# geloescht/mxnet-maintenance

Hardware: AMD Instinct MI355X
Metric: images/sec (whole node) ResNet-50 fp16 batch 256/GPU at 1/2/4/8 MI355X (higher is better)
Workload: dtype fp16; 1 GPU; model=ResNet-50 v1b, global_batch=256, per_gpu_batch=256, image_size=224, parallelism=dp1, layout=NHWC, optimizer=mp-SGD momentum 0.9, lr 0.1 (linear warm-up 40 steps), hip_graph=True, deterministic=True

## Files before the change

### mxnet_maintenance_amd/contrib/amp/lists.py

```python

LP16 = ['Convolution', 'Deconvolution', 'FullyConnected', 'RNN', 'dot', 'batch_dot', '_linalg_gemm', '_linalg_gemm2',
        'linalg_gemm', 'linalg_gemm2', '_contrib_interleaved_matmul_selfatt_qk',
        '_contrib_interleaved_matmul_selfatt_valatt', '_contrib_interleaved_matmul_encdec_qk',
        '_contrib_interleaved_matmul_encdec_valatt']

FP32 = ['exp', 'expm1', 'log', 'log10', 'log2', 'log1p', 'pow', '_power', 'power', 'broadcast_power', 'rsqrt',
        'rcbrt', 'reciprocal', 'square', 'sqrt', 'cbrt', 'arccos', 'arcsin', 'arctanh', 'arccosh', 'cosh', 'sinh',
        'tan', 'erfinv', 'gamma', 'gammaln', 'digamma',
        'softmax', 'log_softmax', 'softmin', 'SoftmaxActivation', 'softmax_cross_entropy', 'SoftmaxOutput',
        'LinearRegressionOutput', 'LogisticRegressionOutput', 'MAERegressionOutput', 'CTCLoss', 'ctc_loss',
        'MakeLoss', 'make_loss', 'SVMOutput',
        'norm', 'L2Normalization', 'LayerNorm', 'GroupNorm', 'InstanceNorm', 'LRN', 'moments',
        'sum', 'sum_axis', 'nansum', 'prod', 'nanprod', 'mean', 'topk', 'sort', 'argsort', 'cumsum',
        '_contrib_MultiBoxDetection', '_contrib_MultiBoxPrior', '_contrib_MultiBoxTarget', '_contrib_box_nms',
        '_contrib_ROIAlign', 'ROIPooling', 'Correlation', 'BilinearSampler', 'GridGenerator', 'SpatialTransformer']

WIDEST = ['elemwise_add', 'elemwise_sub', 'elemwise_mul', 'elemwise_div', '_plus', '_Plus', '_add', '_minus',
          '_Minus', '_sub', '_mul', '_Mul', '_div', '_Div', '_mod', '_Mod', '_maximum', '_minimum', '_hypot',
          '_equal', '_not_equal', '_greater', '_greater_equal', '_lesser', '_lesser_equal',
          'broadcast_add', 'broadcast_plus', 'broadcast_sub', 'broadcast_minus', 'broadcast_mul', 'broadcast_div',
          'broadcast_mod', 'broadcast_maximum', 'broadcast_minimum', 'broadcast_hypot', 'broadcast_equal',
          'broadcast_not_equal', 'broadcast_greater', 'broadcast_greater_equal', 'broadcast_lesser',
          'broadcast_lesser_equal', 'Concat', 'concat', 'stack', 'add_n', 'ElementWiseSum', 'where',
          '_contrib_BatchNormAddReLU', 'BatchNormAddReLU']

CONDITIONAL_FP32 = [('Activation', 'act_type', ['softrelu']), ('LeakyReLU', 'act_type', ['elu', 'selu'])]

LOSS_OUTPUT = ['SoftmaxOutput', 'LinearRegressionOutput', 'LogisticRegressionOutput', 'MAERegressionOutput']
```

### mxnet_maintenance_amd/gluon/model_zoo/vision/resnet.py

```python
from ... import nn
from ...block import HybridBlock
from ...nn.basic_layers import _BatchNorm
from ....context import cpu

__all__ = ['ResNetV1', 'ResNetV2', 'BasicBlockV1', 'BasicBlockV2', 'BottleneckV1', 'BottleneckV2',
           'BottleneckV1b', 'resnet18_v1', 'resnet34_v1', 'resnet50_v1', 'resnet101_v1', 'resnet152_v1',
           'resnet18_v2', 'resnet34_v2', 'resnet50_v2', 'resnet101_v2', 'resnet152_v2', 'resnet50_v1b',
           'resnet101_v1b', 'resnet152_v1b', 'resnet18_v1b', 'resnet34_v1b', 'get_resnet']


def _bn_axis(layout):
    return 3 if layout == 'NHWC' else 1


def _conv(channels, k, stride, pad, in_channels, layout, use_bias=False):
    return nn.Conv2D(channels, kernel_size=k, strides=stride, padding=pad, use_bias=use_bias,
                     in_channels=in_channels, layout=layout)


def _bn(layout, relu=False, fuse=False, **kw):
    if relu and fuse:
        return nn.BatchNormReLU(axis=_bn_axis(layout), **kw)
    return nn.BatchNorm(axis=_bn_axis(layout), **kw)


class _StemBNReLUPool(nn.BatchNormReLU):

    def hybrid_forward(self, F, x, gamma, beta, running_mean, running_var):
        return F.contrib.BatchNormReLUMaxPool(x, gamma, beta, running_mean, running_var, name='fwd',
                                              kernel=(3, 3), stride=(2, 2), pad=(1, 1), **self._kwargs)


def _stem_tail(features, layout, fuse):
    if fuse and layout == 'NHWC':
        features.add(_StemBNReLUPool(axis=_bn_axis(layout)))
        return
    features.add(_bn(layout, True, fuse))
    if not fuse:
        features.add(nn.Activation('relu'))
    features.add(nn.MaxPool2D(3, 2, 1, layout=layout))


class _ResidualTail(_BatchNorm):

    def __init__(self, layout, fuse, **kwargs):
        super().__init__(axis=_bn_axis(layout), **kwargs)
        self._fuse_add = fuse

    def _alias(self):
        return 'batchnorm'

    def hybrid_forward(self, F, x, shortcut, gamma, beta, running_mean, running_var):
        if self._fuse_add:
            return F.contrib.BatchNormAddReLU(x, shortcut, gamma, beta, running_mean, running_var, name='fwd',
                                              **self._kwargs)
        return F.BatchNorm(x, gamma, beta, running_mean, running_var, name='fwd', **self._kwargs)


def _finish(F, tail, out, shortcut):
    y = tail(out, shortcut)
    return y if tail._fuse_add else F.Activation(y + shortcut, act_type='relu')


class BasicBlockV1(HybridBlock):

    def __init__(self, channels, stride, downsample=False, in_channels=0, layout='NCHW', fuse=False, **kwargs):
        super().__init__(**kwargs)
        self.body = nn.HybridSequential(prefix='')
        self.body.add(_conv(channels, 3, stride, 1, in_channels, layout),
                      _bn(layout, True, fuse))
        if not fuse:
            self.body.add(nn.Activation('relu'))
        self.body.add(_conv(channels, 3, 1, 1, channels, layout))
        self.tail = _ResidualTail(layout, fuse)
        self.downsample = None
        if downsample:
            self.downsample = nn.HybridSequential(prefix='')
            self.downsample.add(_conv(channels, 1, stride, 0, in_channels, layout), _bn(layout))

    def hybrid_forward(self, F, x):
        shortcut = self.downsample(x) if self.downsample is not None else x
        return _finish(F, self.tail, self.body(x), shortcut)


class BottleneckV1(HybridBlock):

    def __init__(self, channels, stride, downsample=False, in_channels=0, layout='NCHW', fuse=False,
                 stride_on_3x3=False, **kwargs):
        super().__init__(**kwargs)
        mid = channels // 4
        s1, s3 = (1, stride) if stride_on_3x3 else (stride, 1)
        self.body = nn.HybridSequential(prefix='')
        self.body.add(_conv(mid, 1, s1, 0, in_channels, layout), _bn(layout, True, fuse))
        if not fuse:
            self.body.add(nn.Activation('relu'))
        self.body.add(_conv(mid, 3, s3, 1, mid, layout), _bn(layout, True, fuse))
        if not fuse:
            self.body.add(nn.Activation('relu'))
        self.body.add(_conv(channels, 1, 1, 0, mid, layout))
        self.tail = _ResidualTail(layout, fuse)
        self.downsample = None
        if downsample:
            self.downsample = nn.HybridSequential(prefix='')
            self.downsample.add(_conv(channels, 1, stride, 0, in_channels, layout), _bn(layout))
        self._tee = fuse and s1 == 1 and layout == 'NHWC'
        if self._tee:
            self.body[0]._tee = True

    def hybrid_forward(self, F, x):
        if self._tee:
            blocks = list(self.body._children.values())
            out, passthrough = blocks[0](x)
            for b in blocks[1:]:
                out = b(out)
            shortcut = self.downsample(passthrough) if self.downsample is not None else passthrough
            return _finish(F, self.tail, out, shortcut)
        shortcut = self.downsample(x) if self.downsample is not None else x
        return _finish(F, self.tail, self.body(x), shortcut)


class BottleneckV1b(BottleneckV1):
    def __init__(self, channels, stride, downsample=False, in_channels=0, layout='NCHW', fuse=False, **kwargs):
        super().__init__(channels, stride, downsample, in_channels, layout, fuse, stride_on_3x3=True, **kwargs)


class BasicBlockV2(HybridBlock):

    def __init__(self, channels, stride, downsample=False, in_channels=0, layout='NCHW', fuse=False, **kwargs):
        super().__init__(**kwargs)
        self.bn1 = _bn(layout, True, fuse)
        self.conv1 = _conv(channels, 3, stride, 1, in_channels, layout)
        self.bn2 = _bn(layout, True, fuse)
        self.conv2 = _conv(channels, 3, 1, 1, channels, layout)
        self._fused = fuse
        self.downsample = _conv(channels, 1, stride, 0, in_channels, layout) if downsample else None

    def _act(self, F, x, bn):
        x = bn(x)
        return x if self._fused else F.Activation(x, act_type='relu')

    def hybrid_forward(self, F, x):
        shortcut = x
        x = self._act(F, x, self.bn1)
        if self.downsample is not None:
            shortcut = self.downsample(x)
        x = self.conv1(x)
        x = self.conv2(self._act(F, x, self.bn2))
        return x + shortcut


class BottleneckV2(HybridBlock):

    def __init__(self, channels, stride, downsample=False, in_channels=0, layout='NCHW', fuse=False, **kwargs):
        super().__init__(**kwargs)
        mid = channels // 4
        self.bn1 = _bn(layout, True, fuse)
        self.conv1 = _conv(mid, 1, 1, 0, 0, layout)
        self.bn2 = _bn(layout, True, fuse)
        self.conv2 = _conv(mid, 3, stride, 1, mid, layout)
        self.bn3 = _bn(layout, True, fuse)
        self.conv3 = _conv(channels, 1, 1, 0, 0, layout)
        self._fused = fuse
        self.downsample = _conv(channels, 1, stride, 0, in_channels, layout) if downsample else None

    def _act(self, F, x, bn):
        x = bn(x)
        return x if self._fused else F.Activation(x, act_type='relu')

    def hybrid_forward(self, F, x):
        shortcut = x
        x = self._act(F, x, self.bn1)
        if self.downsample is not None:
            shortcut = self.downsample(x)
        x = self.conv1(x)
        x = self.conv2(self._act(F, x, self.bn2))
        x = self.conv3(self._act(F, x, self.bn3))
        return x + shortcut


class _ResNetBase(HybridBlock):
    def _stage(self, block, n, channels, stride, index, in_channels, layout, fuse):
        stage = nn.HybridSequential(prefix='stage%d_' % index)
        with stage.name_scope():
            stage.add(block(channels, stride, channels != in_channels, in_channels=in_channels, layout=layout,
                            fuse=fuse, prefix=''))
            for _ in range(n - 1):
                stage.add(block(channels, 1, False, in_channels=channels, layout=layout, fuse=fuse, prefix=''))
        return stage


class ResNetV1(_ResNetBase):

    def __init__(self, block, layers, channels, classes=1000, thumbnail=False, layout='NCHW', fuse=False,
                 **kwargs):
        super().__init__(**kwargs)
        assert len(layers) == len(channels) - 1
        self._layout = layout
        with self.name_scope():
            self.features = nn.HybridSequential(prefix='')
            if thumbnail:
                self.features.add(_conv(channels[0], 3, 1, 1, 0, layout))
            else:
                self.features.add(_conv(channels[0], 7, 2, 3, 0, layout))
                _stem_tail(self.features, layout, fuse)
            for i, n in enumerate(layers):
                self.features.add(self._stage(block, n, channels[i + 1], 1 if i == 0 else 2, i + 1,
                                              channels[i], layout, fuse))
            self.features.add(nn.GlobalAvgPool2D(layout=layout))
            self.output = nn.Dense(classes, in_units=channels[-1])

    def hybrid_forward(self, F, x):
        return self.output(self.features(x))


class ResNetV2(_ResNetBase):

    def __init__(self, block, layers, channels, classes=1000, thumbnail=False, layout='NCHW', fuse=False,
                 **kwargs):
        super().__init__(**kwargs)
        assert len(layers) == len(channels) - 1
        with self.name_scope():
            self.features = nn.HybridSequential(prefix='')
            self.features.add(nn.BatchNorm(scale=False, center=False, axis=_bn_axis(layout)))
            if thumbnail:
                self.features.add(_conv(channels[0], 3, 1, 1, 0, layout))
            else:
                self.features.add(_conv(channels[0], 7, 2, 3, 0, layout))
                _stem_tail(self.features, layout, fuse)
            in_channels = channels[0]
            for i, n in enumerate(layers):
                self.features.add(self._stage(block, n, channels[i + 1], 1 if i == 0 else 2, i + 1,
                                              in_channels, layout, fuse))
                in_channels = channels[i + 1]
            self.features.add(_bn(layout, True, fuse))
            if not fuse:
                self.features.add(nn.Activation('relu'))
            self.features.add(nn.GlobalAvgPool2D(layout=layout))
            self.features.add(nn.Flatten())
            self.output = nn.Dense(classes, in_units=in_channels)

    def hybrid_forward(self, F, x):
        return self.output(self.features(x))


resnet_spec = {18: ('basic_block', [2, 2, 2, 2], [64, 64, 128, 256, 512]),
               34: ('basic_block', [3, 4, 6, 3], [64, 64, 128, 256, 512]),
               50: ('bottle_neck', [3, 4, 6, 3], [64, 256, 512, 1024, 2048]),
               101: ('bottle_neck', [3, 4, 23, 3], [64, 256, 512, 1024, 2048]),
               152: ('bottle_neck', [3, 8, 36, 3], [64, 256, 512, 1024, 2048])}
resnet_net_versions = [ResNetV1, ResNetV2]
resnet_block_versions = [{'basic_block': BasicBlockV1, 'bottle_neck': BottleneckV1},
                         {'basic_block': BasicBlockV2, 'bottle_neck': BottleneckV2}]


def get_resnet(version, num_layers, pretrained=False, ctx=cpu(), root='~/.mxnet/models', v1b=False, **kwargs):
    assert num_layers in resnet_spec, 'Invalid number of layers: %d. Options are %s' % (
        num_layers, str(resnet_spec.keys()))
    block_type, layers, channels = resnet_spec[num_layers]
    assert 1 <= version <= 2, 'Invalid resnet version: %d. Options are 1 and 2.' % version
    resnet_class = resnet_net_versions[version - 1]
    block_class = resnet_block_versions[version - 1][block_type]
    if v1b and block_type == 'bottle_neck':
        block_class = BottleneckV1b
    net = resnet_class(block_class, layers, channels, **kwargs)
    if pretrained:
        from ..model_store import get_model_file
        net.load_parameters(get_model_file('resnet%d_v%d' % (num_layers, version), root=root), ctx=ctx)
    return net


# ... 59 lines not shown
```

### mxnet_maintenance_amd/ops/hip_ops.py

```python
import os

import torch
import torch.nn.functional as F

from ..base import MXNetError
from . import kernels as _K

_ALLOW_FALLBACK = os.environ.get('MXAMD_ALLOW_TORCH_FALLBACK', '0') == '1'


def _acc(t):
    return t if t.dtype == torch.float64 else t.float()


def _use_hip(t):
    if not t.is_cuda:
        return False
    if _K.available():
        return _K.enabled()
    if _ALLOW_FALLBACK:
        return False
    raise MXNetError('HIP kernel extension not loaded on a GPU device: %s' % _K.load_error())


def _nd_to_ncx(x):
    nd = x.dim()
    return x.permute(0, nd - 1, *range(1, nd - 1))


def _ncx_to_nd(x):
    nd = x.dim()
    return x.permute(0, *range(2, nd), 1)



def linear(data, weight, bias):
    if _use_hip(data) and _K.gemm_ok(data, weight):
        return _K.Linear.apply(data, weight, bias)
    if data.dim() == 2:
        return F.linear(data, weight, bias)
    return F.linear(data, weight, bias)


def embedding(data, weight):
    if _use_hip(weight) and _K.embedding_ok(data, weight):
        return _K.Embedding.apply(data, weight)
    return None


def _as_nhwc_view(t):
    v = t.permute(0, 2, 3, 1)
    return v if v.is_contiguous() else v.contiguous()


def _nchw_on_hip(data):
    return (data.dim() == 4 and data.dtype in (torch.float16, torch.bfloat16) and _use_hip(data)
            and _NCHW_VIA_NHWC)


_NCHW_VIA_NHWC = os.environ.get('MXAMD_NCHW_VIA_NHWC', '1') == '1'


def _nhwc_weight(w):
    if w.shape[2] == 1 and w.shape[3] == 1 and w.is_contiguous():
        return w.view(w.shape[0], 1, 1, w.shape[1])
    return w.permute(0, 2, 3, 1).contiguous()


def conv(data, weight, bias, stride, pad, dilate, groups, channel_last):
    nsp = data.dim() - 2
    if groups > 1 and nsp == 2 and _use_hip(data):
        from .conv_dw import dw_ok, ConvDwNHWC
        xl = data if channel_last else (_as_nhwc_view(data) if _nchw_on_hip(data) else None)
        if xl is not None and dw_ok(xl, weight, groups, dilate):
            rs = tuple(weight.shape[1:3]) if channel_last else tuple(weight.shape[2:4])
            y = ConvDwNHWC.apply(xl, weight, bias, rs, tuple(stride), tuple(pad), tuple(dilate))
            return y if channel_last else y.permute(0, 3, 1, 2)
    if not channel_last and nsp == 2 and _nchw_on_hip(data):
        xl = _as_nhwc_view(data)
        wl = _nhwc_weight(weight)
        if _K.conv_ok(xl, wl, stride, pad, dilate, groups):
            if _K.kpad_ok(xl, wl):
                return _K.conv_kpad(xl, wl, bias, stride, pad, dilate).permute(0, 3, 1, 2)
            return _K.ConvNHWC.apply(xl, wl, bias, tuple(stride), tuple(pad), tuple(dilate)).permute(0, 3, 1, 2)
    if channel_last and _use_hip(data) and _K.conv_ok(data, weight, stride, pad, dilate, groups):
        if _K.kpad_ok(data, weight):
            return _K.conv_kpad(data, weight, bias, stride, pad, dilate)
        return _K.ConvNHWC.apply(data, weight, bias, tuple(stride), tuple(pad), tuple(dilate))
    if nsp == 2 and groups == 1 and _use_hip(data) and tuple(dilate) != (1, 1):
        xl = data if channel_last else (_as_nhwc_view(data) if _nchw_on_hip(data) else None)
        if xl is not None:
            wl = weight if channel_last else _nhwc_weight(weight)
            if _K.dil_ok(xl, wl, dilate):
                y = _K.ConvDilNHWC.apply(xl, wl, bias, tuple(stride), tuple(pad), tuple(dilate))
                return y if channel_last else y.permute(0, 3, 1, 2)
    if _use_hip(data):
        from . import conv_gen
        y = conv_gen.conv(data, weight, bias, tuple(stride), tuple(pad), tuple(dilate), groups, channel_last)
        if y is not None:
            return y
    if channel_last:
        x = _nd_to_ncx(data)
        w = _nd_to_ncx(weight)
    else:
        x, w = data, weight
    fn = {1: F.conv1d, 2: F.conv2d, 3: F.conv3d}[nsp]
    y = fn(x, w, bias, stride=stride, padding=pad, dilation=dilate, groups=groups)
    return _ncx_to_nd(y) if channel_last else y


def conv_tee(data, weight, inplace_grad=False):
    if _use_hip(data) and hasattr(_K, 'ConvTeeNHWC') and _K.conv_tee_ok(data, weight):
        return _K.ConvTeeNHWC.apply(data, weight, bool(inplace_grad))
    return conv(data, weight, None, (1, 1), (0, 0), (1, 1), 1, True), data



def batch_norm_relu_maxpool(data, gamma, beta, moving_mean, moving_var, eps, momentum, fix_gamma, training,
                            axis, kernel, stride, pad, invstd_out=False):
    nd = data.dim()
    if (nd == 4 and axis % nd == 3 and _use_hip(data) and _K.bnrelu_pool_ok(data, kernel, stride, pad)):
        g = torch.ones_like(gamma) if fix_gamma else gamma
        return _K.BatchNormNHWC.apply(data, g, beta, None, eps, training, True, moving_mean, moving_var, momentum,
                                      invstd_out, (tuple(kernel), tuple(stride), tuple(pad)))
    out, m, v = batch_norm(data, gamma, beta, moving_mean, moving_var, eps, momentum, fix_gamma, training, axis,
                           'relu', invstd_out=invstd_out)
    return pool(out, 'max', tuple(kernel), tuple(stride), tuple(pad), 'valid', True, axis % nd == nd - 1), m, v


def batch_norm(data, gamma, beta, moving_mean, moving_var, eps, momentum, fix_gamma, training,
               axis, act_type, addend=None, invstd_out=False):
    nd = data.dim()
    axis = axis % nd
    channel_last = (axis == nd - 1) and nd > 2
    g = torch.ones_like(gamma) if fix_gamma else gamma
    if axis == 1 and _nchw_on_hip(data) and data.permute(0, 2, 3, 1).is_contiguous():
        xl = data.permute(0, 2, 3, 1)
        al = _as_nhwc_view(addend) if addend is not None else None
        if _K.bn_ok(xl):
            out, m, v = _K.BatchNormNHWC.apply(xl, g, beta, al, eps, training, act_type == 'relu',
                                                moving_mean, moving_var, momentum, invstd_out)
            return out.permute(0, 3, 1, 2), m, v
    if channel_last and _use_hip(data) and _K.bn_ok(data):
        return _K.BatchNormNHWC.apply(data, g, beta, addend, eps, training, act_type == 'relu',
                                      moving_mean, moving_var, momentum, invstd_out)
    if channel_last:
        x = _nd_to_ncx(data)
    elif axis != 1:
        others = [i for i in range(nd) if i != axis]
        perm = [others[0], axis] + others[1:]
        x = data.permute(*perm)
    else:
        x = data
    if training:
        out, smean, sinvstd = torch.ops.aten.native_batch_norm(x, g, beta, None, None, True, 0.0, eps)
        with torch.no_grad():
            var = (1.0 / (sinvstd.float() ** 2) - eps).clamp_(min=0.0) if sinvstd.numel() else sinvstd
            moving_mean.mul_(momentum).add_(smean.detach().to(moving_mean.dtype), alpha=1 - momentum)
            moving_var.mul_(momentum).add_(var.to(moving_var.dtype), alpha=1 - momentum)
        mean_out, var_out = smean, (sinvstd if invstd_out else var)
    else:
        out = F.batch_norm(x, moving_mean, moving_var, g, beta, False, 0.0, eps)
        mean_out, var_out = moving_mean, moving_var
    if channel_last:
        out = _ncx_to_nd(out)
    elif axis != 1:
        inv = [0] * nd
        others = [i for i in range(nd) if i != axis]
        perm = [others[0], axis] + others[1:]
        for i, p in enumerate(perm):
            inv[p] = i
        out = out.permute(*inv)
    if addend is not None:
        out = out + addend
    if act_type == 'relu':
        out = torch.relu(out)
    return out, mean_out, var_out



def global_pool(data, pool_type, channel_last):
    nsp = data.dim() - 2
    if not channel_last and pool_type == 'avg' and _nchw_on_hip(data) and data.permute(0, 2, 3, 1).is_contiguous():
        xl = data.permute(0, 2, 3, 1)
        if _K.gap_ok(xl):
            return _K.GlobalAvgPoolNHWC.apply(xl).permute(0, 3, 1, 2)
    if channel_last:
        if _use_hip(data) and nsp == 2 and pool_type == 'avg' and _K.gap_ok(data):
            return _K.GlobalAvgPoolNHWC.apply(data)
        dims = tuple(range(1, 1 + nsp))
    else:
        dims = tuple(range(2, 2 + nsp))
    if pool_type == 'max':
        return torch.amax(data, dim=dims, keepdim=True)
    if pool_type == 'sum':
        return torch.sum(data, dim=dims, keepdim=True)
    if pool_type == 'lp':
        return torch.sqrt(torch.sum(data * data, dim=dims, keepdim=True))
    return torch.mean(data, dim=dims, keepdim=True)


def _pool_out(n, k, s, p, conv):
    if conv == 'full':
        return int(-(-(n + 2 * p - k) // s)) + 1
    return (n + 2 * p - k) // s + 1


def pool(data, pool_type, kernel, stride, pad, convention, count_include_pad, channel_last, p_value=None):
    nsp = data.dim() - 2
    if not channel_last and nsp == 2 and pool_type in ('max', 'avg') and convention != 'same' \
            and _nchw_on_hip(data) and data.permute(0, 2, 3, 1).is_contiguous():
        xl = data.permute(0, 2, 3, 1)
        if _K.pool_ok(xl, kernel, stride, pad):
            return _K.PoolNHWC.apply(xl, pool_type, tuple(kernel), tuple(stride), tuple(pad),
                                     convention == 'full', bool(count_include_pad)).permute(0, 3, 1, 2)
    if channel_last and _use_hip(data) and nsp == 2 and pool_type in ('max', 'avg') \
            and _K.pool_ok(data, kernel, stride, pad):
        return _K.PoolNHWC.apply(data, pool_type, tuple(kernel), tuple(stride), tuple(pad),
                                 convention == 'full', bool(count_include_pad))
    x = _nd_to_ncx(data) if channel_last else data
    if channel_last and x.is_cuda and pool_type != 'max':
        x = x.contiguous()
    ceil = convention == 'full'
    pad_r = list(pad)
    if convention == 'same':
        ceil = False
        for i in range(nsp):
            n = x.shape[2 + i]
            out = -(-n // stride[i])
            tot = max((out - 1) * stride[i] + kernel[i] - n, 0)
            pad_r[i] = tot // 2
    if pool_type == 'max':
        fn = {1: F.max_pool1d, 2: F.max_pool2d, 3: F.max_pool3d}[nsp]
        y = fn(x, kernel, stride, pad_r, ceil_mode=ceil)
    elif pool_type == 'avg':
        fn = {1: F.avg_pool1d, 2: F.avg_pool2d, 3: F.avg_pool3d}[nsp]
        y = fn(x, kernel, stride, pad_r, ceil_mode=ceil, count_include_pad=count_include_pad)
    elif pool_type == 'sum':
        fn = {1: F.avg_pool1d, 2: F.avg_pool2d, 3: F.avg_pool3d}[nsp]
        y = fn(x, kernel, stride, pad_r, ceil_mode=ceil, count_include_pad=True) * float(torch.tensor(kernel).prod())
    elif pool_type == 'lp':
        pv = p_value or 2
        fn = {1: F.lp_pool1d, 2: F.lp_pool2d, 3: F.lp_pool3d}[nsp]
        if any(pad_r):
            x = F.pad(x, [q for pp in reversed(pad_r) for q in (pp, pp)])
        y = fn(x, pv, kernel, stride, ceil_mode=ceil)
    else:
        raise MXNetError('unknown pool_type %s' % pool_type)
    return _ncx_to_nd(y) if channel_last else y



_HIP_ELEMWISE = os.environ.get('MXAMD_HIP_ELEMWISE', '1') == '1'


def relu(x):
    if _HIP_ELEMWISE and _use_hip(x) and _K.relu_ok(x):
        return _K.ReluHip.apply(x)
    return torch.relu(x)


def binary(op, a, b):
    if (_HIP_ELEMWISE and isinstance(a, torch.Tensor) and isinstance(b, torch.Tensor) and _use_hip(a)
            and _K.binary_ok(a, b)):
        return _K.BinaryHip.apply(a, b, op)
    return None


def gelu(x):
    if _use_hip(x) and _K.ew_ok(x):
        return _K.GELU.apply(x)
    return F.gelu(x)


def layer_norm(data, gamma, beta, eps, want_stats=True):
    if _use_hip(data) and _K.ln_ok(data):
        return _K.LayerNorm.apply(data, gamma, beta, eps, bool(want_stats))
    x = _acc(data)
    mean = x.mean(-1, keepdim=True)
    var = x.var(-1, keepdim=True, unbiased=False)
    std = torch.sqrt(var + eps)
    y = (x - mean) / std * _acc(gamma) + _acc(beta)
    return y.to(data.dtype), mean.to(data.dtype), std.to(data.dtype)


def add_dropout_layer_norm(x, h, gamma, beta, eps, p, handoff=False):
    if (_use_hip(x) and x.dtype in (torch.float16, torch.bfloat16) and _K.ln_ok(x) and h.shape == x.shape
            and h.dtype == x.dtype and h.is_contiguous()
            and h.data_ptr() % 16 == 0 and 0.0 <= p < 1.0):
        return _K.AddDropoutLN.apply(x, h, gamma, beta, eps, p, bool(handoff))
    if p > 0:
        h = h * (torch.rand_like(h, dtype=torch.float32) >= p).to(h.dtype) / (1 - p)
    return layer_norm(x + h, gamma, beta, eps, False)[0]


def softmax(x, axis=-1, scale=1.0, log=False):
    if _use_hip(x) and hasattr(_K, 'Softmax') and _K.softmax_ok(x, axis):
        return _K.Softmax.apply(x, scale, log)
    return None


def dropout(x, p):
    if _use_hip(x) and hasattr(_K, 'Dropout') and _K.ew_ok(x) and 0.0 < p < 1.0:
        return _K.Dropout.apply(x, p)
    return None


def softmax_ce(logits, label, reduction='none'):
    if label.dim() > 1 and label.numel() == logits.shape[0]:
        label = label.reshape(-1)
    if _use_hip(logits) and _K.ce_ok(logits):
        loss = _K.SoftmaxCE.apply(logits, label)
    else:
        lg = logits.float() if logits.dtype in (torch.float16, torch.bfloat16) else logits
        loss = F.cross_entropy(lg, label.to(torch.int64), reduction='none')
    if reduction == 'sum':
        return loss.sum()
    if reduction == 'mean':
        return loss.mean()
    return loss
```

### mxnet_maintenance_amd/ops/kernel_fns.py

```python
import os

import torch

from . import kernels as _K
from .. import _state
from ..utils import env as _env

__all__ = ['BatchNormNHWC', 'SoftmaxCE', 'GlobalAvgPoolNHWC', 'flat_sgd']

_DT = {torch.float32: 0, torch.float16: 1, torch.bfloat16: 2}


def _stream():
    return torch.cuda.current_stream().cuda_stream


def _p(t):
    return 0 if t is None else t.data_ptr()


def _f32(t):
    if t.dtype == torch.float32 and t.is_contiguous():
        return t
    m = getattr(t, '_mxamd_master', None)
    if m is not None and m[1] == t._version and m[0].shape == t.shape:
        return m[0]
    return t.float().contiguous()



def bn_ok(x):
    C = x.shape[-1] if x.dim() else 0
    return (x.dtype in _DT and x.dim() >= 2 and x.is_contiguous() and C % 8 == 0
            and x.numel() > 0 and x.data_ptr() % 16 == 0)


def ce_ok(x):
    return x.dim() == 2 and x.dtype in _DT and x.is_contiguous()




def _leaf_grad(t, numel=None, dtype=torch.float32):
    if t is None or _state.DIRECT_GRAD[0] <= 0 or torch.is_grad_enabled() or not t.is_leaf or not t.requires_grad:
        return None
    gb = t.grad
    if gb is None or gb.dtype != dtype or not gb.is_contiguous() or gb.shape != t.shape:
        return None
    if numel is not None and gb.numel() != numel:
        return None
    return gb


_RELU_FROM_X = [True]
_BN_BWD_FUSE = [os.environ.get('MXAMD_BN_BWD_FUSE', '1') != '0']
_BN_TAIL_DS = [os.environ.get('MXAMD_BN_TAIL_DS', '1') != '0']
_BN_POOL_BWD = [True]
_ZEROS = {}


def _zeros_f32(n, dev):
    z = _ZEROS.get((n, dev))
    if z is None:
        z = _ZEROS[(n, dev)] = torch.zeros(n, dtype=torch.float32, device=dev)
    return z


class _BnToken:
    __slots__ = ('lazy',)

    def __init__(self):
        self.lazy = None


class BatchNormNHWC(torch.autograd.Function):

    @staticmethod
    def forward(ctx, x, gamma, beta, addend, eps, training, relu, moving_mean, moving_var, momentum=None,
                invstd_out=False, pool=None):
        lib = _K.lib()
        C = x.shape[-1]
        R = x.numel() // C
        dev = x.device
        g = _f32(gamma)
        b = _f32(beta)
        mm = _f32(moving_mean)
        assert pool is None or (relu and addend is None)
        y = torch.empty_like(x) if pool is None else None
        if addend is not None:
            assert addend.shape == x.shape and addend.dtype == x.dtype
            addend = addend.contiguous()
        ext_nblk = 0
        center = mm
        if training:
            ext = getattr(x, '_mxamd_bn_part', None)
            if ext is not None and ext[0].numel() == 2 * C * ext[1] and ext[0].device == dev:
                part, ext_nblk = ext
                center = _zeros_f32(C, dev)
            else:
                nblk = lib.bn_partials_rows(R, C)
                part = torch.empty(2 * nblk * C, dtype=torch.float32, device=dev)
            stats = torch.empty(5, C, dtype=torch.float32, device=dev)
            mean, invstd, var, scale, shift = stats.unbind(0)
        else:
            part = None
            mean = mm
            invstd = torch.rsqrt(_f32(moving_var) + eps)
            var = _f32(moving_var)
            scale = g * invstd
            shift = b - mean * scale
        upd = (training and momentum is not None and mm is moving_mean and moving_var.dtype == torch.float32
               and moving_var.is_contiguous())
        mask = (torch.empty(x.numel() // 8, dtype=torch.uint8, device=dev)
                if (addend is not None and relu and _RELU_FROM_X[0]) else None)
        lib.bn_nhwc_forward(_DT[x.dtype], x.data_ptr(), _p(addend), _p(y), _p(mask), g.data_ptr(),
                            b.data_ptr(),
                            center.data_ptr(), _p(part), mean.data_ptr(), invstd.data_ptr(), var.data_ptr(),
                            scale.data_ptr(), shift.data_ptr(), R, C, float(eps), int(bool(training)),
                            int(bool(relu)), 0, float(momentum or 0.0), moving_mean.data_ptr() if upd else 0,
                            moving_var.data_ptr() if upd else 0, int(ext_nblk), _stream())
        if training and momentum is not None and not upd:
            with torch.no_grad():
                moving_mean.mul_(momentum).add_(mean.to(moving_mean.dtype), alpha=1 - momentum)
                moving_var.mul_(momentum).add_(var.to(moving_var.dtype), alpha=1 - momentum)
        ctx.pool = None
        if pool is not None:
            (kh, kw), (sh, sw), (ph, pw) = pool
            N, H, W = x.shape[:3]
            Ho, Wo = _pool_out(H, kh, sh, ph, False), _pool_out(W, kw, sw, pw, False)
            y = torch.empty((N, Ho, Wo, C), dtype=x.dtype, device=dev)
            arg = torch.empty((N, Ho, Wo, C), dtype=torch.uint8, device=dev)
            ctx.pool = (N, H, W, C, Ho, Wo, kh, kw, sh, sw, ph, pw, 1)
            lib.pool_nhwc_forward_bnrelu(_DT[x.dtype], x.data_ptr(), y.data_ptr(), arg.data_ptr(), *ctx.pool,
                                         _stream(), scale.data_ptr(), shift.data_ptr())
            mask = arg
        relu_mode = 0 if not relu else (1 if not _RELU_FROM_X[0] else (3 if addend is not None else 2))
        if pool is not None:
            relu_mode = 2
        ctx.save_for_backward(x, y if relu_mode == 1 else mask, g, mean, invstd,
                              scale if relu_mode == 2 else None, shift if relu_mode == 2 else None)
        ctx.cfg = (relu_mode, bool(training), addend is not None, gamma.dtype, beta.dtype)
        ctx.tee_key = getattr(addend, '_mxamd_tee_key', None) if (addend is not None and relu_mode == 3) else None
        ctx.bn_token = None
        if training and relu_mode in (0, 2, 3) and _BN_BWD_FUSE[0] and pool is None:
            ctx.bn_token = _BnToken()
            y._mxamd_bn_src = (x, mean, scale if relu_mode == 2 else None, shift if relu_mode == 2 else None,
                               mask if relu_mode == 3 else None, relu_mode, ctx.bn_token)
        ctx.refs = (gamma, beta)
        ctx.add_src = None
        if relu_mode == 3 and training and _BN_BWD_FUSE[0] and _BN_TAIL_DS[0]:
            src = getattr(addend, '_mxamd_bn_src', None)
            if (src is not None and src[5] == 0 and tuple(src[0].shape) == tuple(x.shape)
                    and src[0].dtype == x.dtype and src[0].is_contiguous()):
                ctx.add_src = src
        third = invstd if (invstd_out and training) else var
        ctx.mark_non_differentiable(mean, third)
        ctx.set_materialize_grads(False)
        return y, mean, third

    @staticmethod
    def backward(ctx, gy, _gm, _gv):
        lib = _K.lib()
        x, y, g, mean, invstd, fscale, fshift = ctx.saved_tensors
        relu_mode, training, has_add, gdt, bdt = ctx.cfg
        gamma_ref, beta_ref = ctx.refs
        if gy is None:
            return (None,) * 12
        gy = gy.contiguous()
        C = x.shape[-1]
        R = x.numel() // C
        dev = x.device
        fused_pool = False
        if ctx.pool is not None:
            fused_pool = (x.dtype in (torch.float16, torch.bfloat16) and 256 % (C // 8) == 0
                          and hasattr(lib, 'bn_pool_backward') and _BN_POOL_BWD[0])
            if not fused_pool:
                gyd = torch.empty_like(x)
                lib.pool_nhwc_backward(_DT[x.dtype], 1, gy.data_ptr(), y.data_ptr(), gyd.data_ptr(), *ctx.pool,
                                       _stream())
                gy, y = gyd, None
        lazy_mask = None
        tok = ctx.bn_token
        if tok is not None and tok.lazy is not None:
            dy_l, mask_l, ver_l = tok.lazy
            tok.lazy = None
            if gy is dy_l and gy._version == ver_l and relu_mode == 0 and not has_add and ctx.pool is None:
                lazy_mask = mask_l
            else:
                gy = (gy - dy_l + _materialize_dz(dy_l, mask_l)).contiguous()
        dx = torch.empty_like(x)
        dz = torch.empty_like(x) if has_add else None
        ext = getattr(gy, '_mxamd_bn_bwd', None)
        ext_nblk = 0
        if (ext is not None and ctx.bn_token is not None and ext[2] is ctx.bn_token
                and ext[3] == gy._version):
            part, ext_nblk = ext[0], ext[1]
        else:
            nblk = lib.bn_partials_rows(R, C)
            part = torch.empty(2 * nblk * C, dtype=torch.float32, device=dev)
        out = torch.empty(5, C, dtype=torch.float32, device=dev)
        need_g, need_b = ctx.needs_input_grad[1], ctx.needs_input_grad[2]
        tg = _leaf_grad(gamma_ref, C) if need_g else None
        tb = _leaf_grad(beta_ref, C) if need_b else None
        direct = tb is not None and (tg is not None or not need_g) and (tg is not None or tb is not None)
        if direct:
            dg_buf = tg if tg is not None else torch.zeros(C, dtype=torch.float32, device=dev)
            dg_ptr, db_ptr, accum = dg_buf.data_ptr(), tb.data_ptr(), 1
        else:
            dg_ptr, db_ptr, accum = out[0].data_ptr(), out[1].data_ptr(), 0
        if fused_pool:
            N_, H_, W_, C_, Ho_, Wo_, kh, kw, sh, sw, ph, pw, _ = ctx.pool
            ppart = torch.empty(2 * lib.bn_pool_bwd_blocks() * C, dtype=torch.float32, device=dev)
            lib.bn_pool_backward(_DT[x.dtype], x.data_ptr(), gy.data_ptr(), y.data_ptr(), dx.data_ptr(), g.data_ptr(),
                                 mean.data_ptr(), invstd.data_ptr(), fscale.data_ptr(), fshift.data_ptr(),
                                 ppart.data_ptr(), dg_ptr, db_ptr, out[2].data_ptr(), N_, H_, W_, C_, Ho_, Wo_, kh, kw,
                                 sh, sw, ph, pw, 0, int(training), accum, _stream())
            if direct:
                return dx, None, None, None, None, None, None, None, None, None, None, None
            return (dx, out[0].to(gdt) if need_g else None, out[1].to(bdt) if need_b else None,
                    None, None, None, None, None, None, None, None, None)
        ymask = y if relu_mode == 3 else None
        y = y if relu_mode == 1 else None
        ds = ctx.add_src if dz is not None else None
        lazy = (dz is not None and ds is None and ymask is not None and ctx.tee_key is not None
                and lazy_shortcut_ok(ctx.tee_key))
        lazy_ds = (dz is not None and ds is not None and ymask is not None and _LAZY_DZ[0]
                   and isinstance(ds[6], _BnToken))
        if lazy or lazy_ds:
            dz = None
        kmode = relu_mode
        if lazy_mask is not None:
            kmode, ymask = 3, lazy_mask
        dkw = {}
        if ds is not None:
            ds_nblk = lib.bn_tail_ds_rows(R, C)
            ds_part = torch.empty(2 * ds_nblk * C, dtype=torch.float32, device=dev)
            dkw = dict(ds_z=ds[0].data_ptr(), ds_mean=ds[1].data_ptr(), ds_part=ds_part.data_ptr())
        lib.bn_nhwc_backward(_DT[x.dtype], x.data_ptr(), gy.data_ptr(), _p(y), _p(ymask), dx.data_ptr(), _p(dz),
                             g.data_ptr(),
                             mean.data_ptr(), invstd.data_ptr(), _p(fscale), _p(fshift), part.data_ptr(), dg_ptr,
                             db_ptr, out[2].data_ptr(), R, C, kmode, 0, int(training), accum, _stream(),
                             ext_nblk, **dkw)
        if ds is not None:
            if lazy_ds:
                gy._mxamd_bn_bwd = (ds_part, ds_nblk, ds[6], gy._version)
                ds[6].lazy = (gy, ymask, gy._version)
                dz = gy
            else:
                dz._mxamd_bn_bwd = (ds_part, ds_nblk, ds[6], dz._version)
        if lazy:
            gy._mxamd_lazy_mask = (ymask, gy._version)
            dz = gy
        if direct:
            dgamma = None
            dbeta = None
        else:
            dgamma = out[0].to(gdt) if need_g else None
            dbeta = out[1].to(bdt) if need_b else None
        return dx, dgamma, dbeta, dz, None, None, None, None, None, None, None, None


def bnrelu_pool_ok(x, kernel, stride, pad):
    return (bn_ok(x) and tuple(kernel) == (3, 3) and pool_ok(x, kernel, stride, pad)
            and x.numel() + 256 * 32 * 256 * 8 < 2 ** 31 and hasattr(_K.lib(), 'pool_nhwc_forward_bnrelu'))


class SoftmaxCE(torch.autograd.Function):

    @staticmethod
    def forward(ctx, logits, label):
        lib = _K.lib()
        N, K = logits.shape
        lab = label.reshape(-1)
        is_int = not lab.is_floating_point()
        lab = lab.to(torch.int64).contiguous() if is_int else lab.float().contiguous()
        loss = torch.empty(N, dtype=torch.float32, device=logits.device)
        lse = torch.empty(N, dtype=torch.float32, device=logits.device)
        lib.softmax_ce_forward(_DT[logits.dtype], int(is_int), logits.data_ptr(), lab.data_ptr(), loss.data_ptr(),
                               lse.data_ptr(), N, K, _stream())
        ctx.save_for_backward(logits, lab, lse)
        ctx.is_int = is_int
        return loss

    @staticmethod
    def backward(ctx, gout):
        lib = _K.lib()
        logits, lab, lse = ctx.saved_tensors
        N, K = logits.shape
        g = gout.float().contiguous()
        dl = torch.empty_like(logits)
        lib.softmax_ce_backward(_DT[logits.dtype], int(ctx.is_int), logits.data_ptr(), lab.data_ptr(),
                                lse.data_ptr(), g.data_ptr(), dl.data_ptr(), N, K, _stream())
        return dl, None


class GlobalAvgPoolNHWC(torch.autograd.Function):
    @staticmethod
    def forward(ctx, x):
        lib = _K.lib()
        x = x.contiguous()
        N, C = x.shape[0], x.shape[-1]
        HW = x.numel() // (N * C)
        y = torch.empty((N,) + (1,) * (x.dim() - 2) + (C,), dtype=x.dtype, device=x.device)
        lib.gap_nhwc_forward(_DT[x.dtype], x.data_ptr(), y.data_ptr(), N, HW, C, _stream())
        ctx.shape = x.shape
        return y

    @staticmethod
    def backward(ctx, gy):
        lib = _K.lib()
        shape = ctx.shape
        N, C = shape[0], shape[-1]
        HW = int(torch.tensor(shape[1:-1]).prod())
        gy = gy.contiguous()
        dx = torch.empty(shape, dtype=gy.dtype, device=gy.device)
        lib.gap_nhwc_backward(_DT[gy.dtype], gy.data_ptr(), dx.data_ptr(), N, HW, C, _stream())
        return dx


def gap_ok(x):
    return x.dtype in _DT and x.is_contiguous() and x.shape[-1] % 8 == 0


class ReluHip(torch.autograd.Function):

    @staticmethod
    def forward(ctx, x):
        x = x.contiguous()
        y = torch.empty_like(x)
        _K.lib().relu_forward(_DT[x.dtype], x.data_ptr(), y.data_ptr(), x.numel(), _stream())
        ctx.save_for_backward(y)
        return y

    @staticmethod
    def backward(ctx, gy):
        y, = ctx.saved_tensors
        gy = gy.contiguous()
        dx = torch.empty_like(y)
        _K.lib().relu_backward(_DT[y.dtype], y.data_ptr(), gy.data_ptr(), dx.data_ptr(), y.numel(), _stream())
        return dx


def relu_ok(x):
    return x.dtype in _DT and x.is_cuda and x.numel() > 0 and x.data_ptr() % 16 == 0 and x.is_contiguous()


_PW_OPS = {'add': 0, 'sub': 1, 'mul': 2, 'div': 3, 'maximum': 4, 'minimum': 5}


def _bcast_strides(t, shape):
    lead = len(shape) - t.dim()
    st = [0] * lead + list(t.stride())
    sz = [1] * lead + list(t.shape)
    return [0 if sz[d] == 1 and shape[d] != 1 else st[d] for d in range(len(shape))]


def _collapse(shape, sa, sb):
    dims = [(n, a, b) for n, a, b in zip(shape, sa, sb) if n != 1] or [(1, 0, 0)]
    out = [list(dims[-1])]
    for n, a, b in reversed(dims[:-1]):
        pn, pa, pb = out[0]
        if a == pa * pn and b == pb * pn:
            out[0] = [n * pn, pa, pb]
        else:
            out.insert(0, [n, a, b])
    return [d[0] for d in out], [d[1] for d in out], [d[2] for d in out]


def _is_row(t, full):
    ts = tuple(t.shape)
    while ts and ts[0] == 1:
        ts = ts[1:]
    return len(ts) <= len(full) and ts == full[len(full) - len(ts):]


def binary_hip(op, a, b):
    shape = torch.broadcast_shapes(a.shape, b.shape)
    out = torch.empty(shape, dtype=a.dtype, device=a.device)
    n = out.numel()
    if n == 0:
        return out
    vec = 4 if a.dtype == torch.float32 else 8
    aligned = a.data_ptr() % 16 == 0 and b.data_ptr() % 16 == 0
    mode, row = 3, 0
    full = tuple(shape)
    if aligned and a.is_contiguous() and b.is_contiguous():
        if tuple(a.shape) == full and tuple(b.shape) == full:
            mode = 0
        elif tuple(a.shape) == full and _is_row(b, full) and b.numel() % vec == 0:
            mode, row = 1, b.numel()
        elif tuple(b.shape) == full and _is_row(a, full) and a.numel() % vec == 0:
            mode, row = 2, a.numel()
    if mode == 3:
        shp, sa, sb = _collapse(list(shape), _bcast_strides(a, shape), _bcast_strides(b, shape))
        if len(shp) > 6:
            return {'add': torch.add, 'sub': torch.sub, 'mul': torch.mul, 'div': torch.div,
                    'maximum': torch.maximum, 'minimum': torch.minimum}[op](a, b)
    else:
        shp, sa, sb = [], [], []
    _K.lib().pointwise_binary(_DT[a.dtype], _PW_OPS[op], a.data_ptr(), b.data_ptr(), out.data_ptr(), n, mode, row,
                              shp, sa, sb, _stream())
    return out


def _sum_to(g, shape):
    if tuple(g.shape) == tuple(shape):
        return g
    return g.sum_to_size(shape) if len(shape) else g.sum()


class BinaryHip(torch.autograd.Function):

    @staticmethod
    def forward(ctx, a, b, op):
# ... 1279 lines not shown
```

### mxnet_maintenance_amd/ops/nn.py

```python
import math
import os

import torch
import torch.nn.functional as F

from .. import _state
from ..base import torch_dtype, MXNetError
from .registry import register
from . import hip_ops



def _acc(t):
    return t if t.dtype == torch.float64 else t.float()


def _is_channel_last(layout):
    return layout is not None and layout.endswith('C') and len(layout) > 2


def _to_ncx(x, layout):
    if _is_channel_last(layout):
        nd = x.dim()
        return x.permute(0, nd - 1, *range(1, nd - 1))
# ... 71 lines not shown

_CONV_PARAMS = {'kernel': ('shape', ()), 'stride': ('shape', ()), 'dilate': ('shape', ()),
                'pad': ('shape', ()), 'num_filter': ('int', 0), 'num_group': ('int', 1),
                'workspace': ('int', 1024), 'no_bias': ('bool', False), 'cudnn_tune': ('str?', None),
                'cudnn_off': ('bool', False), 'layout': ('str?', None)}


@register('Convolution', aliases=('Convolution_v1',), arg_names=_conv_args, infer_params=_conv_infer,
          params=_CONV_PARAMS)
def convolution(data, weight, bias=None, kernel=(), stride=(), dilate=(), pad=(), num_filter=0,
                num_group=1, workspace=1024, no_bias=False, cudnn_tune=None, cudnn_off=False, layout=None):
    nsp = len(kernel)
    stride = _tup(stride, nsp, 1)
    dilate = _tup(dilate, nsp, 1)
    pad = _tup(pad, nsp, 0)
    return hip_ops.conv(data, weight, bias, stride, pad, dilate, num_group,
                        _is_channel_last(layout))


@register('_contrib_ConvolutionTee', aliases=('ConvolutionTee',), arg_names=('data', 'weight'),
          infer_params=_conv_infer, num_outputs=2,
          params=dict(_CONV_PARAMS, no_bias=('bool', True), inplace_shortcut_grad=('bool', False)))
def convolution_tee(data, weight, kernel=(1, 1), stride=(), dilate=(), pad=(), num_filter=0, num_group=1,
                    workspace=1024, no_bias=True, cudnn_tune=None, cudnn_off=False, layout=None,
                    inplace_shortcut_grad=False):
    if tuple(kernel) != (1, 1) or tuple(stride or (1, 1)) != (1, 1) or tuple(pad or (0, 0)) != (0, 0) \
            or not _is_channel_last(layout) or num_group != 1:
        raise ValueError('ConvolutionTee: only channel-last 1x1 stride-1 convolutions')
    return hip_ops.conv_tee(data, weight, inplace_shortcut_grad)


def _deconv_infer(in_shapes, a):
    d = in_shapes[0]
    if d is None:
        return {}
    k = tuple(a['kernel'])
    layout = a.get('layout') or {1: 'NCW', 2: 'NCHW', 3: 'NCDHW'}[len(k)]
    g = a.get('num_group', 1) or 1
    c = d[-1] if _is_channel_last(layout) else d[1]
    if _is_channel_last(layout):
        w = (c,) + k + (a['num_filter'] // g,)
    else:
        w = (c, a['num_filter'] // g) + k
    res = {1: w}
    if not a.get('no_bias', True):
        res[2] = (a['num_filter'],)
    return res


def _deconv_args(a):
    nb = a.get('no_bias', True)
    nb = nb if isinstance(nb, bool) else str(nb) in ('True', 'true', '1')
    return ['data', 'weight'] if nb else ['data', 'weight', 'bias']


@register('Deconvolution', arg_names=_deconv_args, infer_params=_deconv_infer,
          params=dict(_CONV_PARAMS, adj=('shape', ()), target_shape=('shape', ()), no_bias=('bool', True)))
def deconvolution(data, weight, bias=None, kernel=(), stride=(), dilate=(), pad=(), adj=(), target_shape=(),
                  num_filter=0, num_group=1, workspace=1024, no_bias=True, cudnn_tune=None,
                  cudnn_off=False, layout=None):
    nsp = len(kernel)
    stride = _tup(stride, nsp, 1)
    dilate = _tup(dilate, nsp, 1)
    pad = list(_tup(pad, nsp, 0))
    adj = list(_tup(adj, nsp, 0))
    x = _to_ncx(data, layout)
    w = _to_ncx(weight, layout)
    if target_shape:
        for i in range(nsp):
            full = (x.shape[2 + i] - 1) * stride[i] + dilate[i] * (kernel[i] - 1) + 1
            tot = full - target_shape[i]
            pad[i] = (tot + 1) // 2
            adj[i] = tot % 2
    if data.is_cuda and hip_ops._use_hip(data):
        from . import conv_gen
        y = conv_gen.deconv(data, weight, bias, stride, pad, dilate, adj, num_group, _is_channel_last(layout))
        if y is not None:
            return y
    fn = {1: F.conv_transpose1d, 2: F.conv_transpose2d, 3: F.conv_transpose3d}[nsp]
    y = fn(x, w, bias, stride=stride, padding=pad, output_padding=adj, groups=num_group, dilation=dilate)
    return _from_ncx(y, layout)



def _bn_infer(in_shapes, a):
    d = in_shapes[0]
    if d is None:
        return {}
    c = d[a.get('axis', 1) % len(d)]
    return {1: (c,), 2: (c,), 3: (c,), 4: (c,)}


_BN_PARAMS = {'eps': ('float', 1e-3), 'momentum': ('float', 0.9), 'fix_gamma': ('bool', True),
              'use_global_stats': ('bool', False), 'output_mean_var': ('bool', False),
              'axis': ('int', 1), 'cudnn_off': ('bool', False), 'act_type': ('str?', None),
              'min_calib_range': ('float?', None), 'max_calib_range': ('float?', None)}


def _bn_nvis(a):
    o = a.get('output_mean_var', False)
    o = o if isinstance(o, bool) else str(o) in ('True', 'true', '1')
    return 3 if o else 1


@register('BatchNorm', aliases=('BatchNorm_v1', 'CuDNNBatchNorm'),
          arg_names=('data', 'gamma', 'beta'), aux_names=('moving_mean', 'moving_var'),
          num_outputs=3, num_visible_outputs=_bn_nvis, infer_params=_bn_infer, params=_BN_PARAMS,
          output_names=('output', 'mean', 'var'))
def batch_norm(data, gamma, beta, moving_mean, moving_var, eps=1e-3, momentum=0.9, fix_gamma=True,
               use_global_stats=False, output_mean_var=False, axis=1, cudnn_off=False, act_type=None,
               min_calib_range=None, max_calib_range=None):
    training = _state.STATE.training and not use_global_stats
    return hip_ops.batch_norm(data, gamma, beta, moving_mean, moving_var, eps, momentum, fix_gamma,
                              training, axis, act_type, invstd_out=True)


@register('_contrib_BatchNormWithReLU', aliases=('BatchNormWithReLU',),
          arg_names=('data', 'gamma', 'beta'), aux_names=('moving_mean', 'moving_var'),
          num_outputs=3, num_visible_outputs=_bn_nvis, infer_params=_bn_infer, params=_BN_PARAMS)
def batch_norm_relu(data, gamma, beta, moving_mean, moving_var, eps=1e-3, momentum=0.9, fix_gamma=True,
                    use_global_stats=False, output_mean_var=False, axis=1, cudnn_off=False, act_type=None,
                    min_calib_range=None, max_calib_range=None):
    training = _state.STATE.training and not use_global_stats
    return hip_ops.batch_norm(data, gamma, beta, moving_mean, moving_var, eps, momentum, fix_gamma,
                              training, axis, 'relu', invstd_out=True)


_BNPOOL_PARAMS = dict(_BN_PARAMS, kernel=('shape', (3, 3)), stride=('shape', (2, 2)), pad=('shape', (1, 1)))


@register('_contrib_BatchNormReLUMaxPool', aliases=('BatchNormReLUMaxPool',),
          arg_names=('data', 'gamma', 'beta'), aux_names=('moving_mean', 'moving_var'),
          num_outputs=3, num_visible_outputs=_bn_nvis, infer_params=_bn_infer, params=_BNPOOL_PARAMS)
def batch_norm_relu_maxpool(data, gamma, beta, moving_mean, moving_var, eps=1e-3, momentum=0.9, fix_gamma=True,
                            use_global_stats=False, output_mean_var=False, axis=1, cudnn_off=False, act_type=None,
                            min_calib_range=None, max_calib_range=None, kernel=(3, 3), stride=(2, 2), pad=(1, 1)):
    training = _state.STATE.training and not use_global_stats
    return hip_ops.batch_norm_relu_maxpool(data, gamma, beta, moving_mean, moving_var, eps, momentum, fix_gamma,
                                           training, axis, _tup(kernel, 2, 1), _tup(stride, 2, 1), _tup(pad, 2, 0),
                                           invstd_out=True)


@register('_contrib_BatchNormAddReLU', aliases=('BatchNormAddReLU',),
          arg_names=('data', 'addend', 'gamma', 'beta'), aux_names=('moving_mean', 'moving_var'),
          num_outputs=3, num_visible_outputs=_bn_nvis,
          infer_params=lambda s, a: {k + 1: v for k, v in _bn_infer(s, a).items() if k + 1 <= 5 and k > 0},
          params=_BN_PARAMS)
def batch_norm_add_relu(data, addend, gamma, beta, moving_mean, moving_var, eps=1e-3, momentum=0.9,
                        fix_gamma=True, use_global_stats=False, output_mean_var=False, axis=1,
                        cudnn_off=False, act_type=None, min_calib_range=None, max_calib_range=None):
    training = _state.STATE.training and not use_global_stats
    return hip_ops.batch_norm(data, gamma, beta, moving_mean, moving_var, eps, momentum, fix_gamma,
                              training, axis, 'relu', addend=addend)



_POOL_PARAMS = {'kernel': ('shape', ()), 'pool_type': ('str', 'max'), 'global_pool': ('bool', False),
                'cudnn_off': ('bool', False), 'pooling_convention': ('str', 'valid'),
                'stride': ('shape', ()), 'pad': ('shape', ()), 'p_value': ('int?', None),
                'count_include_pad': ('bool?', None), 'layout': ('str?', None)}


@register('Pooling', aliases=('Pooling_v1',), params=_POOL_PARAMS)
def pooling(data, kernel=(), pool_type='max', global_pool=False, cudnn_off=False,
            pooling_convention='valid', stride=(), pad=(), p_value=None, count_include_pad=None,
            layout=None):
    nsp = data.dim() - 2
    if count_include_pad is None:
        count_include_pad = True
    if global_pool:
        return hip_ops.global_pool(data, pool_type, _is_channel_last(layout))
    kernel = _tup(kernel, nsp, 1)
    stride = _tup(stride, nsp, 1)
    if pooling_convention == 'same':
        if any(int(p) != 0 for p in (pad or ())):
            raise MXNetError('Pooling: pad must be 0 with pooling_convention=same, got %s' % (tuple(pad),))
        pad = (0,) * nsp
    pad = _tup(pad, nsp, 0)
    return hip_ops.pool(data, pool_type, kernel, stride, pad, pooling_convention,
                        count_include_pad, _is_channel_last(layout), p_value)


@register('_contrib_AdaptiveAvgPooling2D', aliases=('AdaptiveAvgPooling2D',), params={'output_size': ('shape', ())})
def adaptive_avg_pool2d(data, output_size=()):
    os_ = tuple(output_size) if output_size else (1, 1)
    if len(os_) == 1:
        os_ = os_ * 2
    return F.adaptive_avg_pool2d(data, os_)


@register('_contrib_BilinearResize2D', aliases=('BilinearResize2D',), arg_names=lambda a: ['data'] if a.get('mode', 'size') != 'like' else ['data', 'like'],
          params={'height': ('int', 1), 'width': ('int', 1), 'scale_height': ('float?', None),
                  'scale_width': ('float?', None), 'mode': ('str', 'size'), 'align_corners': ('bool', True)})
def bilinear_resize2d(data, like=None, height=1, width=1, scale_height=None, scale_width=None, mode='size',
                      align_corners=True):
    if mode == 'like' and like is not None:
        height, width = like.shape[2], like.shape[3]
    elif scale_height is not None:
        height, width = int(data.shape[2] * scale_height), int(data.shape[3] * (scale_width or scale_height))
    elif mode == 'odd_scale':
        pass
    return F.interpolate(data, size=(height, width), mode='bilinear', align_corners=align_corners)



_ACTS = {
    'relu': torch.relu, 'sigmoid': torch.sigmoid, 'tanh': torch.tanh,
    'softrelu': F.softplus, 'softsign': F.softsign, 'log_sigmoid': F.logsigmoid,
    'mish': F.mish,
}


@register('Activation', params={'act_type': ('str', 'relu')})
def activation(data, act_type='relu'):
    if act_type == 'relu':
        return hip_ops.relu(data)
    return _ACTS[act_type](data)


def _lrelu_args(a):
    return ['data', 'gamma'] if a.get('act_type', 'leaky') == 'prelu' else ['data']


def _lrelu_infer(in_shapes, a):
    if a.get('act_type') != 'prelu' or in_shapes[0] is None:
        return {}
    d = in_shapes[0]
    return {1: (d[1] if len(d) > 1 else 1,)}


@register('LeakyReLU', arg_names=_lrelu_args, infer_params=_lrelu_infer, num_outputs=1,
          params={'act_type': ('str', 'leaky'), 'slope': ('float', 0.25), 'lower_bound': ('float', 0.125),
                  'upper_bound': ('float', 0.334)})
def leaky_relu(data, gamma=None, act_type='leaky', slope=0.25, lower_bound=0.125, upper_bound=0.334):
    if act_type == 'leaky':
        return F.leaky_relu(data, slope)
    if act_type == 'prelu':
        if gamma.dim() > 1:
            g = gamma.reshape(tuple(gamma.shape) + (1,) * (data.dim() - gamma.dim()))
        else:
            g = gamma.reshape((1, -1) + (1,) * (data.dim() - 2)) if data.dim() > 1 else gamma
        return torch.where(data >= 0, data, data * g)
    if act_type == 'elu':
        return F.elu(data, slope)
    if act_type == 'selu':
        return F.selu(data)
    if act_type == 'gelu':
        return hip_ops.gelu(data)
    if act_type == 'rrelu':
        if _state.STATE.training:
            a = torch.empty_like(data).uniform_(lower_bound, upper_bound)
            return torch.where(data >= 0, data, data * a)
        return F.leaky_relu(data, (lower_bound + upper_bound) / 2)
    raise MXNetError('unknown act_type %s' % act_type)



def _softmax_args(a):
    ul = a.get('use_length', False)
    ul = ul if isinstance(ul, bool) else str(ul) in ('True', 'true', '1')
    return ['data', 'length'] if ul else ['data']


def _length_mask(data, length, axis):
    n = data.shape[axis]
    ar = torch.arange(n, device=data.device)
    shape = [1] * data.dim()
    shape[axis] = n
    ar = ar.reshape(shape)
    lshape = list(data.shape)
    lshape[axis] = 1
    return ar < length.reshape(lshape).to(ar.dtype)


_SM_PARAMS = {'axis': ('int', -1), 'temperature': ('float?', None), 'dtype': ('str?', None),
              'use_length': ('bool', False)}


@register('softmax', arg_names=_softmax_args, params=_SM_PARAMS)
def softmax(data, length=None, axis=-1, temperature=None, dtype=None, use_length=False):
    if not (length is not None and use_length) and (dtype is None or torch_dtype(dtype) == data.dtype):
        r = hip_ops.softmax(data, axis, 1.0 / temperature if temperature else 1.0)
        if r is not None:
            return r
    x = data if temperature is None or temperature == 1.0 else data / temperature
    if length is not None and use_length:
        m = _length_mask(x, length, axis % x.dim())
        x = x.masked_fill(~m, float('-inf'))
        r = torch.softmax(_acc(x), dim=axis)
        r = torch.nan_to_num(r, nan=0.0).masked_fill(~m, 0.0)
    else:
        r = torch.softmax(x, dim=axis, dtype=torch.float32) if x.dtype in (torch.float16, torch.bfloat16) else torch.softmax(x, dim=axis)
    return r.to(torch_dtype(dtype) if dtype else data.dtype)


@register('log_softmax', arg_names=_softmax_args, params=_SM_PARAMS)
def log_softmax(data, length=None, axis=-1, temperature=None, dtype=None, use_length=False):
    if dtype is None or torch_dtype(dtype) == data.dtype:
        r = hip_ops.softmax(data, axis, 1.0 / temperature if temperature else 1.0, log=True)
        if r is not None:
            return r
    x = data if temperature is None or temperature == 1.0 else data / temperature
    r = torch.log_softmax(x.float() if x.dtype in (torch.float16, torch.bfloat16) else x, dim=axis)
    return r.to(torch_dtype(dtype) if dtype else data.dtype)


# ... 777 lines not shown
```

### src/kernels/bindings.cc

```cpp
#include <hip/hip_runtime.h>
#include <pybind11/pybind11.h>
#include <pybind11/stl.h>

#include <cstdint>
#include <stdexcept>
#include <vector>

namespace py = pybind11;

namespace mxamd {
void bn_nhwc_forward(int dtype, const void* x, const void* addend, void* y, uint8_t* mask, const float* gamma,
                     const float* beta,
                     const float* center, float* part, float* mean, float* invstd, float* var, float* scale,
                     float* shift, int64_t R, int C, float eps, int training, int relu, int fix_gamma,
                     float momentum, float* mm_upd, float* mv_upd, int ext_nblk, hipStream_t s);
void bn_nhwc_backward(int dtype, const void* x, const void* dy, const void* y, const uint8_t* mask, void* dx,
                      void* dz,
                      const float* gamma, const float* mean, const float* invstd, const float* fscale,
                      const float* fshift, float* part, float* dgamma, float* dbeta, float* coef, int64_t R, int C,
                      int relu_mode, int fix_gamma, int training, int accum, hipStream_t s, int ext_nblk, const void* ds_z, const float* ds_mean, float* ds_part);
int bn_partials_rows(int64_t R, int C);
int bn_tail_ds_rows(int64_t R, int C);
void gemm_nt(int dtype, const void* a, const void* b, const void* bias, const void* addend, void* c, int out_f32,
             int M, int N, int K, int lda, int ldb, int ldc, int act, int cfg, int splits, float* ws, hipStream_t s,
             int bias_lowp);
int gemm_nt_tile_n(int cfg);
int gemm_nt_tile_m(int cfg);
void int8_gemm(const int8_t* A, const int8_t* B, int32_t* C, int M, int N, int K, hipStream_t s);
void csr_dot_dense(int dtype, const int64_t* indptr, const int64_t* indices, const void* vals, const void* rhs,
                   void* out, int64_t M, int64_t K, int N, hipStream_t s);
void csrT_dot_dense(int dtype, const int64_t* indptr, const int64_t* indices, const void* vals, const void* rhs,
                    const int64_t* slot, float* out32, int64_t M, int64_t K, int N, hipStream_t s);
void embedding_forward(int dtype, int itype, const void* idx, const void* w, void* y, int64_t n, int V, int C,
                       hipStream_t s);
void embedding_backward(int dtype, int itype, const void* idx, const void* dy, float* acc, uint8_t* touched,
                        int out_dtype, void* grad, int accum, int64_t n, int V, int C, hipStream_t s);
int bn_nhwc_stats(int dtype, const void* x, const float* center, float* part, int64_t R, int C, hipStream_t s,
                  int total_blocks);
int64_t colsum_partials(int64_t R, int C);
void colsum_rows(int dtype, const void* x, const float* zeros, float* part, int64_t R, int C, int out_dtype,
                 void* out, int accum, hipStream_t s);
void softmax_ce_forward(int dtype, int label_is_int, const void* logits, const void* label, float* loss, float* lse,
                        int N, int K, hipStream_t s);
void softmax_ce_backward(int dtype, int label_is_int, const void* logits, const void* label, const float* lse,
                         const float* gout, void* dlogits, int N, int K, hipStream_t s);
void gap_nhwc_forward(int dtype, const void* x, void* y, int N, int HW, int C, hipStream_t s);
void relu_forward(int dtype, const void* x, void* y, int64_t n, hipStream_t s);
void relu_backward(int dtype, const void* y, const void* dy, void* dx, int64_t n, hipStream_t s);
void pointwise_binary(int dtype, int op, const void* a, const void* b, void* out, int64_t n, int mode, int64_t row,
                      int ndim, const int64_t* shape, const int64_t* astride, const int64_t* bstride, hipStream_t s);
void gap_nhwc_backward(int dtype, const void* dy, void* dx, int N, int HW, int C, hipStream_t s);
void flat_sgd(int dtype, void* w, const void* g, float* mom, float* w32, int64_t n, float lr, float wd,
              float momentum, float rescale, float clip, const float* hp, hipStream_t s);
void conv_nhwc_fwd(int dtype, const void* x, const void* w, const float* bias, void* y, int N, int H, int W, int C,
                   int K, int R, int S, int sh, int sw, int ph, int pw, int variant, hipStream_t s);
int conv_nhwc_fwd_big_nparts(int N, int H, int W, int R, int S, int sh, int sw, int ph, int pw, int variant);
void conv_nhwc_fwd_big(int dtype, const void* x, const void* w, const float* bias, void* y, const void* zero, int N,
                       int H, int W, int C, int K, int R, int S, int sh, int sw, int ph, int pw, int variant,
                       float* part, int nparts, const void* addend, hipStream_t s, const void* bn_z,
                       const float* bn_mean, const float* bn_scale, const float* bn_shift, const uint8_t* bn_mask,
                       int bn_mode, float* bn_part, int bn_nparts, int up, int dh, int dw);
int conv_nhwc_fwd_big_bwd_nparts(int N, int H, int W, int R, int S, int sh, int sw, int ph, int pw, int variant);
void conv_nhwc_fwd_glds(int dtype, const void* x, const void* w, const float* bias, void* y, const void* zero, int N,
                        int H, int W, int C, int K, int R, int S, int sh, int sw, int ph, int pw, int bco,
                        hipStream_t s, const void* bn_z, const float* bn_mean, const float* bn_scale,
                        const float* bn_shift, float* bn_part, int bn_nparts);
int conv_glds_bwd_nparts(int M, int bco);
void conv_nhwc_dgrad_phases_glds(int dtype, const void* dy, const void* w, void* dx, const void* zero, int N, int Hi,
                                 int Wi, int Cin, int Cout, int Ho, int Wo, int stride, int nph, const int* ph,
                                 const int* pw, const int* R, const int* S, const int* pad_h, const int* pad_w,
                                 const int64_t* w_off, int nzero, const int* zph, const int* zpw, int bco,
                                 hipStream_t s, const void* bn_z, const float* bn_mean, const float* bn_scale,
                                 const float* bn_shift, float* bn_part, int bn_nparts);
int conv_nhwc_fwd_ring_nparts(int N, int H, int W, int R, int S, int sh, int sw, int ph, int pw, int variant);
void conv_nhwc_fwd_ring(int dtype, const void* x, const void* w, void* y, const void* zero, int N, int H, int W, int C,
                        int K, int R, int S, int sh, int sw, int ph, int pw, int variant, float* part, int nparts,
                        hipStream_t s);
bool conv3x3_halo_ok(int C, int K, int R, int S, int sh, int sw, int ph, int pw, int W);
int conv3x3_halo_nparts(int N, int H);
void conv3x3_halo(int dtype, const void* x, const void* w, void* y, const void* zero, int N, int H, int W, int C, int K,
                  float* part, int nparts, const void* bn_z, const float* bn_mean, const float* bn_scale,
                  const float* bn_shift, int bn_mode, float* bn_part, hipStream_t s);
int conv_nhwc_wgrad_ring_ok(int C, int K, int R, int S, int variant);
int64_t conv_nhwc_wgrad_ring_workspace(int N, int H, int W, int C, int K, int R, int S, int sh, int sw, int ph, int pw,
                                       int variant, int dh, int dw);
void conv_nhwc_wgrad_ring(int dtype, const void* x, const void* dy, float* slab, int out_dtype, void* out, int accum,
                          int N, int H, int W, int C, int K, int R, int S, int sh, int sw, int ph, int pw,
                          const void* zero, int variant, hipStream_t s, int dh, int dw);
int64_t conv_nhwc_wgrad_workspace(int N, int H, int W, int C, int K, int R, int S, int sh, int sw, int ph, int pw,
                                  int dh, int dw);
void conv_nhwc_wgrad(int dtype, const void* x, const void* dy, float* slab, int out_dtype, void* out, int accum, int N,
                     int H, int W, int C, int K, int R, int S, int sh, int sw, int ph, int pw, const void* zero,
                     hipStream_t s, int dh, int dw);
int conv_stem_grid(int N, int H, int W, int R, int S, int ph, int pw);
void conv_stem_fwd(int dtype, const void* x, const void* w, void* y, int N, int H, int W, int C, int K, int R, int S,
                   int sh, int sw, int ph, int pw, float* part, int nparts, hipStream_t s);
int64_t conv_stem_wgrad_workspace(int N, int H, int W, int R, int S, int ph, int pw);
void conv_stem_wgrad(int dtype, const void* x, const void* dy, float* slab, int out_dtype, void* out, int accum, int N,
                     int H, int W, int C, int K, int R, int S, int sh, int sw, int ph, int pw, hipStream_t s);
int layernorm_bwd_partials(int M);
void layernorm_forward(int dtype, const void* x, const void* gamma, const void* beta, int pt, void* y, float* mean,
                       float* rstd, int M, int D, float eps, hipStream_t s);
void layernorm_backward(int dtype, const void* x, const void* dy, const void* gamma, int pt, const float* mean,
                        const float* rstd, void* dx, float* part, void* dgamma, void* dbeta, int gdtype, int accum,
                        int M, int D, hipStream_t s);
void add_dropout_ln_forward(int dtype, const void* x, const void* h, const void* gamma, const void* beta, int pt,
                            void* y, void* s_out, uint8_t* mask, float* mean, float* rstd, int M, int D, float eps,
                            float p, uint64_t seed, const uint64_t* seed_base, hipStream_t s);
void add_dropout_ln_backward(int dtype, const void* s_in, const void* dy, const void* gamma, int pt, const float* mean,
                             const float* rstd, const uint8_t* mask, float p, void* ds, void* dh, float* part,
                             float* hpart, void* dgamma, void* dbeta, int gdtype, int accum, int M, int D,
                             hipStream_t s);
void column_sum_partials(int gdtype, const float* part, int nb, int ncol, void* out, int accum, hipStream_t s);
void gelu_forward(int dtype, const void* x, void* y, int64_t n, hipStream_t s);
void gelu_backward(int dtype, const void* x, const void* dy, void* dx, int64_t n, hipStream_t s);
void gelu_backward_colpart(int dtype, const void* x, const void* dy, void* dx, float* part, int M, int N,
                           hipStream_t s);
int gelu_colpart_blocks(int M, int N);
void softmax_forward(int dtype, int log, const void* x, void* y, int M, int L, float scale, hipStream_t s);
void softmax_backward(int dtype, int log, const void* y, const void* dy, void* dx, int M, int L, float scale,
                      hipStream_t s);
void dropout_forward(int dtype, const void* x, void* y, uint8_t* mask, int64_t n, float p, uint64_t seed,
                     const uint64_t* seed_base, hipStream_t s);
void dropout_backward(int dtype, const void* dy, const uint8_t* mask, void* dx, int64_t n, float p, hipStream_t s);
int attention_max_seq();
void attention_forward(int dtype, const void* qkv, const float* kmask, void* out, float* lse, int S, int B, int H,
                       int D, float scale, float p, uint64_t seed, const uint64_t* seed_base, hipStream_t s);
void attention_backward(int dtype, const void* qkv, const float* kmask, const void* out, const void* dout,
                        const float* lse, float* delta, void* dqkv, int S, int B, int H, int D, float scale, float p,
                        uint64_t seed, const uint64_t* seed_base, hipStream_t s);
void flat_adam(int dtype, int mode, void* w, const void* g, float* mean, float* var, float* w32, int64_t n, float lr,
               float beta1, float beta2, float eps, float wd, float eta, float rescale, float clip, const float* hp,
               hipStream_t s);
void lamb_update(int dtype, void* w, const void* g, float* mean, float* var, float* w32, float* upd,
                 const void* chunks, int nchunks, float* nrm, int nseg, float lr, float beta1, float beta2, float eps,
                 float bc1, float bc2, float wd, float rescale, float clip, float lb, float ub, const float* hp,
                 hipStream_t s);
void seg_sumsq(int dtype, const void* x, const void* chunks, int nchunks, float* out, int nseg, hipStream_t s);
void all_finite(int dtype, const void* x, int64_t n, float scale, int* flag, int init, hipStream_t s);
void pool_nhwc_forward(int dtype, int is_max, const void* x, void* y, uint8_t* arg, int N, int H, int W, int C,
                       int Ho, int Wo, int kh, int kw, int sh, int sw, int ph, int pw, int cip, hipStream_t s,
                       const float* scale, const float* shift);
int bn_pool_bwd_blocks();
void bn_pool_backward(int dtype, const void* x, const void* dy, const uint8_t* arg, void* dx, const float* gamma,
                      const float* mean, const float* invstd, const float* fscale, const float* fshift, float* part,
                      float* dgamma, float* dbeta, float* coef, int N, int H, int W, int C, int Ho, int Wo, int kh,
                      int kw, int sh, int sw, int ph, int pw, int fix_gamma, int training, int accum,
                      hipStream_t s);
void pool_nhwc_backward(int dtype, int is_max, const void* dy, const uint8_t* arg, void* dx, int N, int H, int W,
                        int C, int Ho, int Wo, int kh, int kw, int sh, int sw, int ph, int pw, int cip,
                        hipStream_t s);
void deform_im2col(int dtype, const void* x, const void* off, const void* msk, void* cols, int N, int C, int H, int W,
                   int Ho, int Wo, int kh, int kw, int sh, int sw, int ph, int pw, int dh, int dw, int dg,
                   int rows, hipStream_t s);
void deform_col2im(int dtype, const void* off, const void* msk, const void* gcols, float* gx, int N, int C, int H,
                   int W, int Ho, int Wo, int kh, int kw, int sh, int sw, int ph, int pw, int dh, int dw, int dg,
                   int rows, hipStream_t s);
void deform_col2im_coord(int dtype, const void* x, const void* off, const void* msk, const void* gcols, void* goff,
                         void* gmsk, int N, int C, int H, int W, int Ho, int Wo, int kh, int kw, int sh, int sw,
                         int ph, int pw, int dh, int dw, int dg, int rows, hipStream_t s);
void deform_im2col_nhwc(int dtype, const void* x, const void* off, const void* msk, void* cols, const int* g,
                        int ld_off, int ld_msk, hipStream_t s);
void deform_bwd_nhwc(int dtype, const void* x, const void* off, const void* msk, const void* gcols, float* gx,
                     void* goff, void* gmsk, const int* g, int ld_off, int ld_msk, hipStream_t s);
void conv_dw_fwd(int dtype, const void* x, const void* wt, const float* bias, void* y, const int* gm, hipStream_t s);
void conv_dw_dgrad(int dtype, const void* dy, const void* wt, void* dx, const int* gm, hipStream_t s);
void conv_dw_wgrad(int dtype, const void* x, const void* dy, float* slab, int nslice, int out_dtype, void* out,
                   int accum, const int* gm, hipStream_t s);
// ... 99 lines not shown
                                    uintptr_t out, uintptr_t s) {
    twobit_dequantize_sum(P<void>(packed), row_bytes, nrows, n, thr, P<float>(out), S(s));
    check_launch("twobit_dequantize_sum");
  });
  m.def("gemm_nt", [](int dt, uintptr_t a, uintptr_t b, uintptr_t bias, uintptr_t addend, uintptr_t c, int out_f32,
                      int M, int N, int K, int lda, int ldb, int ldc, int act, int cfg, int splits, uintptr_t ws,
                      uintptr_t s, int bias_lowp) {
    gemm_nt(dt, P<void>(a), P<void>(b), P<void>(bias), P<void>(addend), P<void>(c), out_f32, M, N, K, lda, ldb, ldc,
            act, cfg, splits, P<float>(ws), S(s), bias_lowp);
    check_launch("gemm_nt");
  }, py::arg("dt"), py::arg("a"), py::arg("b"), py::arg("bias"), py::arg("addend"), py::arg("c"), py::arg("out_f32"),
     py::arg("M"), py::arg("N"), py::arg("K"), py::arg("lda"), py::arg("ldb"), py::arg("ldc"), py::arg("act"),
     py::arg("cfg"), py::arg("splits"), py::arg("ws"), py::arg("s"), py::arg("bias_lowp") = 0);
  m.def("weight_taps_t", [](int eb, uintptr_t w, uintptr_t out, int K, int RS, int C, std::vector<int> src,
                            std::vector<int64_t> base, std::vector<int64_t> rstride, uintptr_t s) {
    if (src.size() != base.size() || src.size() != rstride.size()) throw std::runtime_error("weight_taps_t: table sizes");
    weight_taps_t(eb, P<const void>(w), P<void>(out), K, RS, C, static_cast<int>(src.size()), src.data(), base.data(),
                  rstride.data(), S(s));
    check_launch("weight_taps_t");
  });
  m.def("conv_pw_stream_ok", &conv_pw_stream_ok);
  m.def("conv_pw_stream_slices", &conv_pw_stream_slices);
  m.def("conv_pw_stream_grid", [](int M, int kin, int nout, int ncu, int add) {
    return conv_pw_stream_grid(M, kin, nout, ncu, add);
  }, pybind11::arg("M"), pybind11::arg("kin"), pybind11::arg("nout"), pybind11::arg("ncu"), pybind11::arg("add") = 0);
  m.def("conv_pw_stream", [](int dt, uintptr_t x, uintptr_t w, uintptr_t y, uintptr_t zero, int M, int kin, int nout,
                             uintptr_t part, int grid, uintptr_t s, uintptr_t addend, int wt, uintptr_t bn_z,
                             uintptr_t bn_mask, uintptr_t bn_mean, uintptr_t bn_scale, uintptr_t bn_shift, int bn_mode,
                             uintptr_t addend_mask) {
    conv_pw_stream(dt, P<const void>(x), P<const void>(w), P<void>(y), P<const void>(zero), M, kin, nout,
                   P<float>(part), grid, S(s), P<const void>(addend), wt, P<const void>(bn_z), P<const uint8_t>(bn_mask),
                   P<const float>(bn_mean), P<const float>(bn_scale), P<const float>(bn_shift), bn_mode,
                   P<const uint8_t>(addend_mask));
    check_launch("conv_pw_stream");
  }, pybind11::arg("dt"), pybind11::arg("x"), pybind11::arg("w"), pybind11::arg("y"), pybind11::arg("zero"),
     pybind11::arg("M"), pybind11::arg("kin"), pybind11::arg("nout"), pybind11::arg("part"), pybind11::arg("grid"),
     pybind11::arg("s"), pybind11::arg("addend"), pybind11::arg("wt") = 0, pybind11::arg("bn_z") = 0,
     pybind11::arg("bn_mask") = 0, pybind11::arg("bn_mean") = 0, pybind11::arg("bn_scale") = 0,
     pybind11::arg("bn_shift") = 0, pybind11::arg("bn_mode") = 0, pybind11::arg("addend_mask") = 0);
  m.def("conv_pw_stream_bnb_ok", &conv_pw_stream_bnb_ok);
  m.def("conv_gen", [](int dt, int mode, uintptr_t src, uintptr_t wsrc, uintptr_t bias, uintptr_t dst,
                       std::vector<int> geom, int splits, uintptr_t s) {
    if (geom.size() != 22) throw std::runtime_error("conv_gen: geometry needs 22 ints");
    conv_gen(dt, mode, P<const void>(src), P<const void>(wsrc), P<const float>(bias), P<void>(dst), geom.data(),
             splits, S(s));
    check_launch("conv_gen");
  });
  m.def("rnn_fwd_seq", [](int dt, int mode, uintptr_t gx, uintptr_t h0, uintptr_t c0, uintptr_t whh, uintptr_t bhh,
                          uintptr_t out, int ldo, uintptr_t cseq, uintptr_t save, int T, int N, int H, int reverse,
                          uintptr_t s) {
    rnn_fwd_seq(dt, mode, P<const float>(gx), P<const void>(h0), P<const float>(c0), P<const void>(whh),
                P<const float>(bhh), P<void>(out), ldo, P<float>(cseq), P<float>(save), T, N, H, reverse, S(s));
    check_launch("rnn_fwd_seq");
  });
  m.def("rnn_bwd_seq", [](int dt, int mode, uintptr_t whhT, uintptr_t dy, int ldy, uintptr_t dhT, uintptr_t save,
                          uintptr_t cseq, uintptr_t c0, uintptr_t h0, uintptr_t out, int ldo, uintptr_t dgh,
                          uintptr_t dgx, uintptr_t dc, uintptr_t dhd, uintptr_t dh0, int T, int N, int H, int reverse,
                          uintptr_t s) {
    rnn_bwd_seq(dt, mode, P<const void>(whhT), P<const void>(dy), ldy, P<const float>(dhT), P<const float>(save),
                P<const float>(cseq), P<const float>(c0), P<const void>(h0), P<const void>(out), ldo, P<void>(dgh),
                P<void>(dgx), P<float>(dc), P<float>(dhd), P<float>(dh0), T, N, H, reverse, S(s));
    check_launch("rnn_bwd_seq");
  });
  m.def("gemm_nt_tile_n", &gemm_nt_tile_n);
  m.def("gemm_nt_tile_m", &gemm_nt_tile_m);
  m.def("slab_reduce", [](int odt, uintptr_t slab, int splits, int64_t n, uintptr_t out, int accum, uintptr_t s) {
    slab_reduce(odt, P<float>(slab), splits, n, P<void>(out), accum, S(s));
    check_launch("slab_reduce");
  });
  m.def("deform_im2col", [](int dt, uintptr_t x, uintptr_t off, uintptr_t msk, uintptr_t cols, std::vector<int> g,
                            uintptr_t s) {
    if (g.size() != 15 && g.size() != 16) throw std::runtime_error("deform_im2col: geometry needs 15 or 16 ints");
    const int rows = g.size() == 16 ? g[15] : 0;
    deform_im2col(dt, P<void>(x), P<void>(off), P<void>(msk), P<void>(cols), g[0], g[1], g[2], g[3], g[4], g[5], g[6],
                  g[7], g[8], g[9], g[10], g[11], g[12], g[13], g[14], rows, S(s));
    check_launch("deform_im2col");
  });
  m.def("deform_col2im", [](int dt, uintptr_t off, uintptr_t msk, uintptr_t gcols, uintptr_t gx, std::vector<int> g,
                            uintptr_t s) {
    if (g.size() != 15 && g.size() != 16) throw std::runtime_error("deform_col2im: geometry needs 15 or 16 ints");
    const int rows = g.size() == 16 ? g[15] : 0;
    deform_col2im(dt, P<void>(off), P<void>(msk), P<void>(gcols), P<float>(gx), g[0], g[1], g[2], g[3], g[4], g[5],
                  g[6], g[7], g[8], g[9], g[10], g[11], g[12], g[13], g[14], rows, S(s));
    check_launch("deform_col2im");
  });
  m.def("deform_col2im_coord", [](int dt, uintptr_t x, uintptr_t off, uintptr_t msk, uintptr_t gcols, uintptr_t goff,
                                  uintptr_t gmsk, std::vector<int> g, uintptr_t s) {
    if (g.size() != 15 && g.size() != 16) throw std::runtime_error("deform_col2im_coord: geometry needs 15 or 16 ints");
    const int rows = g.size() == 16 ? g[15] : 0;
    deform_col2im_coord(dt, P<void>(x), P<void>(off), P<void>(msk), P<void>(gcols), P<void>(goff), P<void>(gmsk),
                        g[0], g[1], g[2], g[3], g[4], g[5], g[6], g[7], g[8], g[9], g[10], g[11], g[12], g[13], g[14],
                        rows, S(s));
    check_launch("deform_col2im_coord");
  });
  m.def("deform_im2col_nhwc", [](int dt, uintptr_t x, uintptr_t off, uintptr_t msk, uintptr_t cols, std::vector<int> g,
                                 int ld_off, int ld_msk, uintptr_t s) {
    if (g.size() != 15) throw std::runtime_error("deform_im2col_nhwc: geometry needs 15 ints");
    deform_im2col_nhwc(dt, P<void>(x), P<void>(off), P<void>(msk), P<void>(cols), g.data(), ld_off, ld_msk, S(s));
    check_launch("deform_im2col_nhwc");
  });
  m.def("deform_bwd_nhwc", [](int dt, uintptr_t x, uintptr_t off, uintptr_t msk, uintptr_t gcols, uintptr_t gx,
                              uintptr_t goff, uintptr_t gmsk, std::vector<int> g, int ld_off, int ld_msk, uintptr_t s) {
    if (g.size() != 15) throw std::runtime_error("deform_bwd_nhwc: geometry needs 15 ints");
    deform_bwd_nhwc(dt, P<void>(x), P<void>(off), P<void>(msk), P<void>(gcols), P<float>(gx), P<void>(goff),
                    P<void>(gmsk), g.data(), ld_off, ld_msk, S(s));
    check_launch("deform_bwd_nhwc");
  });
  m.def("conv_dw_fwd", [](int dt, uintptr_t x, uintptr_t wt, uintptr_t bias, uintptr_t y, std::vector<int> g,
                          uintptr_t s) {
    if (g.size() != 14) throw std::runtime_error("conv_dw_fwd: geometry needs 14 ints");
    conv_dw_fwd(dt, P<void>(x), P<void>(wt), P<float>(bias), P<void>(y), g.data(), S(s));
    check_launch("conv_dw_fwd");
  });
  m.def("conv_dw_dgrad", [](int dt, uintptr_t dy, uintptr_t wt, uintptr_t dx, std::vector<int> g, uintptr_t s) {
    if (g.size() != 14) throw std::runtime_error("conv_dw_dgrad: geometry needs 14 ints");
    conv_dw_dgrad(dt, P<void>(dy), P<void>(wt), P<void>(dx), g.data(), S(s));
    check_launch("conv_dw_dgrad");
  });
  m.def("conv_dw_wgrad", [](int dt, uintptr_t x, uintptr_t dy, uintptr_t slab, int nslice, int out_dt, uintptr_t out,
                            int accum, std::vector<int> g, uintptr_t s) {
    if (g.size() != 14) throw std::runtime_error("conv_dw_wgrad: geometry needs 14 ints");
    conv_dw_wgrad(dt, P<void>(x), P<void>(dy), P<float>(slab), nslice, out_dt, P<void>(out), accum, g.data(), S(s));
    check_launch("conv_dw_wgrad");
  });
  m.def("ssd_loss_blocks", &ssd_loss_blocks);
  m.def("ssd_loss_fwd", [](int dt, uintptr_t cls, uintptr_t loc, uintptr_t ct, uintptr_t lt, uintptr_t lm, int rows,
                           int C1, float lambd, uintptr_t part, uintptr_t out, uintptr_t s) {
    ssd_loss_fwd(dt, P<void>(cls), P<void>(loc), P<float>(ct), P<float>(lt), P<float>(lm), rows, C1, lambd,
                 P<float>(part), P<float>(out), S(s));
    check_launch("ssd_loss_fwd");
  });
  m.def("ssd_loss_bwd", [](int dt, uintptr_t cls, uintptr_t loc, uintptr_t ct, uintptr_t lt, uintptr_t lm,
                           uintptr_t stats, uintptr_t gout, int rows, int C1, float lambd, uintptr_t dcls, uintptr_t dloc,
                           uintptr_t s) {
    ssd_loss_bwd(dt, P<void>(cls), P<void>(loc), P<float>(ct), P<float>(lt), P<float>(lm), P<float>(stats),
                 P<float>(gout), rows, C1, lambd, P<void>(dcls), P<void>(dloc), S(s));
    check_launch("ssd_loss_bwd");
  });
  m.def("multibox_target", [](int dt, uintptr_t anchors, uintptr_t labels, uintptr_t cls_pred, uintptr_t loc_target,
                              uintptr_t loc_mask, uintptr_t cls_target, uintptr_t match_iou, uintptr_t match_gt,
                              uintptr_t key, int B, int A, int L, int W, int C, float thr, float ignore_label,
                              float neg_ratio, float neg_thresh, int min_neg, float v0, float v1, float v2, float v3,
                              uintptr_t s) {
    multibox_target(dt, P<float>(anchors), P<float>(labels), P<void>(cls_pred), P<float>(loc_target),
                    P<float>(loc_mask), P<float>(cls_target), P<float>(match_iou), P<int>(match_gt),
                    P<uint32_t>(key), B, A, L, W, C, thr, ignore_label, neg_ratio, neg_thresh, min_neg, v0, v1, v2,
                    v3, S(s));
    check_launch("multibox_target");
  });
  m.def("bn_nhwc_forward", [](int dt, uintptr_t x, uintptr_t add, uintptr_t y, uintptr_t mask, uintptr_t g, uintptr_t b,
                              uintptr_t center, uintptr_t part, uintptr_t mean, uintptr_t inv, uintptr_t var,
                              uintptr_t scale, uintptr_t shift, int64_t R, int C, float eps, int training, int relu,
                              int fix_gamma, float momentum, uintptr_t mm_upd, uintptr_t mv_upd, int ext_nblk,
                              uintptr_t s) {
    bn_nhwc_forward(dt, P<void>(x), P<void>(add), P<void>(y), P<uint8_t>(mask), P<float>(g), P<float>(b), P<float>(center),
                    P<float>(part), P<float>(mean), P<float>(inv), P<float>(var), P<float>(scale), P<float>(shift), R,
                    C, eps, training, relu, fix_gamma, momentum, P<float>(mm_upd), P<float>(mv_upd), ext_nblk, S(s));
    check_launch("bn_nhwc_forward");
  });
  m.def("bn_nhwc_backward", [](int dt, uintptr_t x, uintptr_t dy, uintptr_t y, uintptr_t mask, uintptr_t dx,
                               uintptr_t dz,
                               uintptr_t g, uintptr_t mean, uintptr_t inv, uintptr_t fscale, uintptr_t fshift,
                               uintptr_t part, uintptr_t dgamma, uintptr_t dbeta, uintptr_t coef, int64_t R, int C,
                               int relu_mode, int fix_gamma, int training, int accum, uintptr_t s, int ext_nblk,
                               uintptr_t ds_z, uintptr_t ds_mean, uintptr_t ds_part) {
    bn_nhwc_backward(dt, P<void>(x), P<void>(dy), P<void>(y), P<uint8_t>(mask), P<void>(dx), P<void>(dz), P<float>(g), P<float>(mean),
                     P<float>(inv), P<float>(fscale), P<float>(fshift), P<float>(part), P<float>(dgamma),
                     P<float>(dbeta), P<float>(coef), R, C, relu_mode, fix_gamma, training, accum, S(s), ext_nblk,
                     P<const void>(ds_z), P<const float>(ds_mean), P<float>(ds_part));
    check_launch("bn_nhwc_backward");
  }, py::arg("dt"), py::arg("x"), py::arg("dy"), py::arg("y"), py::arg("mask"), py::arg("dx"), py::arg("dz"),
     py::arg("g"), py::arg("mean"), py::arg("inv"), py::arg("fscale"), py::arg("fshift"), py::arg("part"),
     py::arg("dgamma"), py::arg("dbeta"), py::arg("coef"), py::arg("R"), py::arg("C"), py::arg("relu_mode"),
     py::arg("fix_gamma"), py::arg("training"), py::arg("accum"), py::arg("stream"), py::arg("ext_nblk") = 0,
     py::arg("ds_z") = 0, py::arg("ds_mean") = 0, py::arg("ds_part") = 0);
  m.def("softmax_ce_forward", [](int dt, int li, uintptr_t logits, uintptr_t label, uintptr_t loss, uintptr_t lse,
                                 int N, int K, uintptr_t s) {
    softmax_ce_forward(dt, li, P<void>(logits), P<void>(label), P<float>(loss), P<float>(lse), N, K, S(s));
    check_launch("softmax_ce_forward");
  });
  m.def("softmax_ce_backward", [](int dt, int li, uintptr_t logits, uintptr_t label, uintptr_t lse, uintptr_t gout,
                                  uintptr_t dlogits, int N, int K, uintptr_t s) {
    softmax_ce_backward(dt, li, P<void>(logits), P<void>(label), P<float>(lse), P<float>(gout), P<void>(dlogits), N,
                        K, S(s));
    check_launch("softmax_ce_backward");
  });
  m.def("relu_forward", [](int dt, uintptr_t x, uintptr_t y, int64_t n, uintptr_t s) {
    relu_forward(dt, P<void>(x), P<void>(y), n, S(s));
    check_launch("relu_forward");
  });
  m.def("relu_backward", [](int dt, uintptr_t y, uintptr_t dy, uintptr_t dx, int64_t n, uintptr_t s) {
    relu_backward(dt, P<void>(y), P<void>(dy), P<void>(dx), n, S(s));
    check_launch("relu_backward");
  });
  m.def("pointwise_binary", [](int dt, int op, uintptr_t a, uintptr_t b, uintptr_t out, int64_t n, int mode,
                               int64_t row, std::vector<int64_t> shape, std::vector<int64_t> sa,
                               std::vector<int64_t> sb, uintptr_t s) {
    if (shape.size() != sa.size() || shape.size() != sb.size()) throw std::runtime_error("pointwise_binary: rank");
    pointwise_binary(dt, op, P<void>(a), P<void>(b), P<void>(out), n, mode, row, static_cast<int>(shape.size()),
                     shape.data(), sa.data(), sb.data(), S(s));
    check_launch("pointwise_binary");
  });
  m.def("gap_nhwc_forward", [](int dt, uintptr_t x, uintptr_t y, int N, int HW, int C, uintptr_t s) {
    gap_nhwc_forward(dt, P<void>(x), P<void>(y), N, HW, C, S(s));
    check_launch("gap_nhwc_forward");
  });
  m.def("gap_nhwc_backward", [](int dt, uintptr_t dy, uintptr_t dx, int N, int HW, int C, uintptr_t s) {
    gap_nhwc_backward(dt, P<void>(dy), P<void>(dx), N, HW, C, S(s));
    check_launch("gap_nhwc_backward");
  });
  m.def("flat_sgd", [](int dt, uintptr_t w, uintptr_t g, uintptr_t mom, uintptr_t w32, int64_t n, float lr,
                       float wd, float momentum, float rescale, float clip, uintptr_t s) {
    flat_sgd(dt, P<void>(w), P<void>(g), P<float>(mom), P<float>(w32), n, lr, wd, momentum, rescale, clip, nullptr,
             S(s));
    check_launch("flat_sgd");
  });
  m.def("flat_sgd", [](int dt, uintptr_t w, uintptr_t g, uintptr_t mom, uintptr_t w32, int64_t n, float lr,
                       float wd, float momentum, float rescale, float clip, uintptr_t s, uintptr_t hp) {
    flat_sgd(dt, P<void>(w), P<void>(g), P<float>(mom), P<float>(w32), n, lr, wd, momentum, rescale, clip,
             P<float>(hp), S(s));
    check_launch("flat_sgd");
  });
  m.def("conv_nhwc_fwd", [](int dt, uintptr_t x, uintptr_t w, uintptr_t bias, uintptr_t y, int N, int H, int W,
                            int C, int K, int R, int Sf, int sh, int sw, int ph, int pw, int variant, uintptr_t s) {
    conv_nhwc_fwd(dt, P<void>(x), P<void>(w), P<float>(bias), P<void>(y), N, H, W, C, K, R, Sf, sh, sw, ph, pw,
                  variant, S(s));
    check_launch("conv_nhwc_fwd");
  });
  m.def("conv_nhwc_fwd_glds", [](int dt, uintptr_t x, uintptr_t w, uintptr_t bias, uintptr_t y, uintptr_t zero, int N,
                                 int H, int W, int C, int K, int R, int Sf, int sh, int sw, int ph, int pw, int bco,
                                 uintptr_t s, uintptr_t bn_z, uintptr_t bn_mean, uintptr_t bn_scale,
                                 uintptr_t bn_shift, uintptr_t bn_part, int bn_nparts) {
    conv_nhwc_fwd_glds(dt, P<void>(x), P<void>(w), P<float>(bias), P<void>(y), P<void>(zero), N, H, W, C, K, R, Sf,
                       sh, sw, ph, pw, bco, S(s), P<void>(bn_z), P<float>(bn_mean), P<float>(bn_scale),
                       P<float>(bn_shift), P<float>(bn_part), bn_nparts);
    check_launch("conv_nhwc_fwd_glds");
  }, py::arg("dtype"), py::arg("x"), py::arg("w"), py::arg("bias"), py::arg("y"), py::arg("zero"), py::arg("N"),
     py::arg("H"), py::arg("W"), py::arg("C"), py::arg("K"), py::arg("R"), py::arg("S"), py::arg("sh"),
     py::arg("sw"), py::arg("ph"), py::arg("pw"), py::arg("bco"), py::arg("stream"), py::arg("bn_z") = 0,
     py::arg("bn_mean") = 0, py::arg("bn_scale") = 0, py::arg("bn_shift") = 0, py::arg("bn_part") = 0,
     py::arg("bn_nparts") = 0);
  m.def("conv_glds_bwd_nparts", &conv_glds_bwd_nparts);
  m.def("conv_nhwc_dgrad_phases_glds",
        [](int dt, uintptr_t dy, uintptr_t w, uintptr_t dx, uintptr_t zero, int N, int Hi, int Wi, int Cin, int Cout,
           int Ho, int Wo, int stride, std::vector<int> ph, std::vector<int> pw, std::vector<int> R,
           std::vector<int> Sf, std::vector<int> pad_h, std::vector<int> pad_w, std::vector<int64_t> w_off,
           std::vector<int> zph, std::vector<int> zpw, int bco, uintptr_t s, uintptr_t bn_z, uintptr_t bn_mean,
           uintptr_t bn_scale, uintptr_t bn_shift, uintptr_t bn_part, int bn_nparts) {
          const size_t n = ph.size();
          if (pw.size() != n || R.size() != n || Sf.size() != n || pad_h.size() != n || pad_w.size() != n ||
              w_off.size() != n || zph.size() != zpw.size())
            throw std::runtime_error("conv_nhwc_dgrad_phases_glds: per-phase lists differ in length");
          conv_nhwc_dgrad_phases_glds(dt, P<void>(dy), P<void>(w), P<void>(dx), P<void>(zero), N, Hi, Wi, Cin, Cout,
                                      Ho, Wo, stride, (int)n, ph.data(), pw.data(), R.data(), Sf.data(),
                                      pad_h.data(), pad_w.data(), w_off.data(), (int)zph.size(), zph.data(),
                                      zpw.data(), bco, S(s), P<void>(bn_z), P<float>(bn_mean), P<float>(bn_scale),
                                      P<float>(bn_shift), P<float>(bn_part), bn_nparts);
          check_launch("conv_nhwc_dgrad_phases_glds");
        },
        py::arg("dtype"), py::arg("dy"), py::arg("w"), py::arg("dx"), py::arg("zero"), py::arg("N"), py::arg("Hi"),
        py::arg("Wi"), py::arg("Cin"), py::arg("Cout"), py::arg("Ho"), py::arg("Wo"), py::arg("stride"),
        py::arg("ph"), py::arg("pw"), py::arg("R"), py::arg("S"), py::arg("pad_h"), py::arg("pad_w"),
        py::arg("w_off"), py::arg("zph"), py::arg("zpw"), py::arg("bco"), py::arg("stream"), py::arg("bn_z") = 0,
        py::arg("bn_mean") = 0, py::arg("bn_scale") = 0, py::arg("bn_shift") = 0, py::arg("bn_part") = 0,
        py::arg("bn_nparts") = 0);
  m.def("conv_stem_grid", &conv_stem_grid);
  m.def("conv_stem_wgrad_workspace", &conv_stem_wgrad_workspace);
  m.def("conv_stem_fwd", [](int dt, uintptr_t x, uintptr_t w, uintptr_t y, int N, int H, int W, int C, int K, int R,
                            int Sf, int sh, int sw, int ph, int pw, uintptr_t part, int nparts, uintptr_t s) {
    conv_stem_fwd(dt, P<void>(x), P<void>(w), P<void>(y), N, H, W, C, K, R, Sf, sh, sw, ph, pw, P<float>(part),
                  nparts, S(s));
    check_launch("conv_stem_fwd");
  });
  m.def("conv_stem_wgrad", [](int dt, uintptr_t x, uintptr_t dy, uintptr_t slab, int odt, uintptr_t out, int accum,
                              int N, int H, int W, int C, int K, int R, int Sf, int sh, int sw, int ph, int pw,
                              uintptr_t s) {
    conv_stem_wgrad(dt, P<void>(x), P<void>(dy), P<float>(slab), odt, P<void>(out), accum, N, H, W, C, K, R, Sf, sh,
                    sw, ph, pw, S(s));
    check_launch("conv_stem_wgrad");
  });
  m.def("conv_nhwc_fwd_big_nparts", &conv_nhwc_fwd_big_nparts);
  m.def("conv_nhwc_fwd_big_bwd_nparts", &conv_nhwc_fwd_big_bwd_nparts);
  m.def("conv_nhwc_fwd_big", [](int dt, uintptr_t x, uintptr_t w, uintptr_t bias, uintptr_t y, uintptr_t zero, int N,
                                int H, int W, int C, int K, int R, int Sf, int sh, int sw, int ph, int pw, int variant,
                                uintptr_t part, int nparts, uintptr_t addend, uintptr_t s, uintptr_t bz,
                                uintptr_t bmean, uintptr_t bscale, uintptr_t bshift, uintptr_t bmask, int bmode,
                                uintptr_t bpart, int bnparts, int up, int dh, int dw) {
    conv_nhwc_fwd_big(dt, P<void>(x), P<void>(w), P<float>(bias), P<void>(y), P<void>(zero), N, H, W, C, K, R, Sf, sh,
                      sw, ph, pw, variant, P<float>(part), nparts, P<void>(addend), S(s), P<void>(bz), P<float>(bmean),
                      P<float>(bscale), P<float>(bshift), P<uint8_t>(bmask), bmode, P<float>(bpart), bnparts, up, dh,
                      dw);
    check_launch("conv_nhwc_fwd_big");
  }, py::arg("dt"), py::arg("x"), py::arg("w"), py::arg("bias"), py::arg("y"), py::arg("zero"), py::arg("N"),
     py::arg("H"), py::arg("W"), py::arg("C"), py::arg("K"), py::arg("R"), py::arg("S"), py::arg("sh"),
     py::arg("sw"), py::arg("ph"), py::arg("pw"), py::arg("variant"), py::arg("part"), py::arg("nparts"),
     py::arg("addend"), py::arg("stream"), py::arg("bn_z") = 0, py::arg("bn_mean") = 0, py::arg("bn_scale") = 0,
     py::arg("bn_shift") = 0, py::arg("bn_mask") = 0, py::arg("bn_mode") = 0, py::arg("bn_part") = 0,
     py::arg("bn_nparts") = 0, py::arg("up") = 0, py::arg("dh") = 1, py::arg("dw") = 1);
  m.def("conv_nhwc_fwd_ring_nparts", &conv_nhwc_fwd_ring_nparts);
  m.def("conv_nhwc_fwd_ring", [](int dt, uintptr_t x, uintptr_t w, uintptr_t y, uintptr_t zero, int N, int H, int W,
                                 int C, int K, int R, int Sf, int sh, int sw, int ph, int pw, int variant, uintptr_t part,
                                 int nparts, uintptr_t s) {
    conv_nhwc_fwd_ring(dt, P<void>(x), P<void>(w), P<void>(y), P<void>(zero), N, H, W, C, K, R, Sf, sh, sw, ph, pw,
                       variant, P<float>(part), nparts, S(s));
    check_launch("conv_nhwc_fwd_ring");
  });
  m.def("conv3x3_halo_ok", &conv3x3_halo_ok);
  m.def("conv3x3_halo_nparts", &conv3x3_halo_nparts);
  m.def("conv3x3_halo", [](int dt, uintptr_t x, uintptr_t w, uintptr_t y, uintptr_t zero, int N, int H, int W, int C,
                           int K, uintptr_t part, int nparts, uintptr_t bn_z, uintptr_t bn_mean, uintptr_t bn_scale,
                           uintptr_t bn_shift, int bn_mode, uintptr_t bn_part, uintptr_t s) {
    conv3x3_halo(dt, P<void>(x), P<void>(w), P<void>(y), P<void>(zero), N, H, W, C, K, P<float>(part), nparts,
// ... 199 lines not shown
```

### src/kernels/bn_nhwc.hip

```cpp
#include <cstdlib>
#include <stdexcept>

#include <algorithm>

#include "common.h"

namespace mxamd {

constexpr int kBnThreads = 256;

struct BnGeom {
  int tpr;
  int cb;
  int rpi;
};

static inline BnGeom bn_geom(int C) {
  BnGeom g;
  int v = C / 8;
  g.tpr = v;
  if (v > kBnThreads)
    for (g.tpr = kBnThreads; v % g.tpr != 0; --g.tpr) {
    }
  g.cb = g.tpr * 8;
// ... 49 lines not shown
        s1[i] += dz;
        s2[i] += dz * (xi - k[i]);
      }
    }
  };
  int64_t r = r0 + lane_r;
  for (; r + (UNR - 1) * rpi < r1; r += UNR * rpi) {
    Vec8<T> vx[UNR], vdy[UNR], vy[UNR];
    uint32_t vm[UNR];
#pragma unroll
    for (int u = 0; u < UNR; ++u) {
      const int64_t off = (r + u * rpi) * C + cbase;
      vx[u].load(x + off);
      if (MODE == 1) vdy[u].load(dy + off);
      if (MODE == 1 && RELU == kReluFromY) vy[u].load(y + off);
      vm[u] = (MODE == 1 && RELU == kReluFromMask) ? mask[off >> 3] : 0u;
    }
#pragma unroll
    for (int u = 0; u < UNR; ++u) accum(vx[u], vdy[u], vy[u], vm[u]);
  }
  for (; r < r1; r += rpi) {
    const int64_t off = r * C + cbase;
    Vec8<T> vx, vdy, vy;
    vx.load(x + off);
    if (MODE == 1) vdy.load(dy + off);
    if (MODE == 1 && RELU == kReluFromY) vy.load(y + off);
    accum(vx, vdy, vy, (MODE == 1 && RELU == kReluFromMask) ? mask[off >> 3] : 0u);
  }
  __shared__ float sh1[kBnThreads * 8];
  __shared__ float sh2[kBnThreads * 8];
  const int cb = tpr * 8;
  if (!spare) {
#pragma unroll
    for (int i = 0; i < 8; ++i) {
      sh1[lane_r * cb + lane_c * 8 + i] = s1[i];
      sh2[lane_r * cb + lane_c * 8 + i] = s2[i];
    }
  }
  __syncthreads();
  for (int c = tid; c < cb; c += kBnThreads) {
    float a = 0.f, b = 0.f;
    for (int rr = 0; rr < rpi; ++rr) {
      a += sh1[rr * cb + c];
      b += sh2[rr * cb + c];
    }
    const int64_t o = static_cast<int64_t>(blockIdx.y * cb + c) * gridDim.x + blockIdx.x;
    part1[o] = a;
    part2[o] = b;
  }
}

constexpr int kFinThreads = 256;
constexpr int kFinPerBlock = kFinThreads / 64;
template <int MODE>
__global__ void __launch_bounds__(kFinThreads) bn_finalize_kernel(
    const float* __restrict__ part1, const float* __restrict__ part2, int nblk, int C, int64_t R,
    const float* __restrict__ center, const float* __restrict__ gamma, const float* __restrict__ beta,
    const float* __restrict__ invstd_in, float eps, float* __restrict__ o0, float* __restrict__ o1,
    float* __restrict__ o2, float* __restrict__ o3, float* __restrict__ o4, float* __restrict__ o5,
    int fix_gamma, int training, float momentum, float* __restrict__ mm_upd, float* __restrict__ mv_upd,
    int accum) {
  const int lane = threadIdx.x & 63;
  const int c = blockIdx.x * kFinPerBlock + (threadIdx.x >> 6);
  if (c >= C) return;
  const float* p1 = part1 + static_cast<int64_t>(c) * nblk;
  const float* p2 = part2 + static_cast<int64_t>(c) * nblk;
  double a = 0.0, b = 0.0;
  const int nv = ((reinterpret_cast<uintptr_t>(p1) | reinterpret_cast<uintptr_t>(p2)) & 15) == 0 ? nblk / 4 : 0;
  for (int i = lane; i < nv; i += 64) {
    const float4 x = reinterpret_cast<const float4*>(p1)[i];
    const float4 y = reinterpret_cast<const float4*>(p2)[i];
    a += static_cast<double>(x.x) + static_cast<double>(x.y) + static_cast<double>(x.z) + static_cast<double>(x.w);
    b += static_cast<double>(y.x) + static_cast<double>(y.y) + static_cast<double>(y.z) + static_cast<double>(y.w);
  }
  for (int i = nv * 4 + lane; i < nblk; i += 64) {
    a += p1[i];
    b += p2[i];
  }
#pragma unroll
  for (int o = 32; o > 0; o >>= 1) {
    a += __shfl_xor(a, o, 64);
    b += __shfl_xor(b, o, 64);
  }
  if (lane != 0) return;
  const double n = static_cast<double>(R);
  const float g = fix_gamma ? 1.f : gamma[c];
  if (MODE == 0) {
    double m1 = a / n;
    double var = b / n - m1 * m1;
    if (var < 0) var = 0;
    double mean = center[c] + m1;
    float inv = static_cast<float>(1.0 / sqrt(var + eps));
    o0[c] = static_cast<float>(mean);
    o1[c] = inv;
    o2[c] = static_cast<float>(var);
    float sc = g * inv;
    o3[c] = sc;
    o4[c] = beta[c] - static_cast<float>(mean) * sc;
    if (mm_upd) mm_upd[c] = mm_upd[c] * momentum + static_cast<float>(mean) * (1.f - momentum);
    if (mv_upd) mv_upd[c] = mv_upd[c] * momentum + static_cast<float>(var) * (1.f - momentum);
  } else {
    const float inv = invstd_in[c];
    const double dbeta = a;
    const double dgamma = b * inv;
    if (accum) {
      o0[c] += static_cast<float>(dgamma);
      o1[c] += static_cast<float>(dbeta);
    } else {
      o0[c] = static_cast<float>(dgamma);
      o1[c] = static_cast<float>(dbeta);
    }
    const double A = static_cast<double>(g) * inv;
    const double B = training ? -A * inv * dgamma / n : 0.0;
    const double Cc = training ? A * (static_cast<double>(center[c]) * inv * dgamma / n - dbeta / n) : 0.0;
    o2[c] = static_cast<float>(A);
    o3[c] = static_cast<float>(B);
    o4[c] = static_cast<float>(Cc);
  }
}

typedef unsigned int bn_u32x4 __attribute__((ext_vector_type(4)));

template <typename T>
__device__ __forceinline__ void vload(Vec8<T>& v, const T* p, int nt) {
  if constexpr (sizeof(T) == 2) {
    if (nt) {
      const bn_u32x4 r = __builtin_nontemporal_load(reinterpret_cast<const bn_u32x4*>(p));
      v.raw = make_uint4(r.x, r.y, r.z, r.w);
      return;
    }
  }
  v.load(p);
}

template <typename T>
__device__ __forceinline__ void vstore(const Vec8<T>& v, T* p, int nt) {
  if constexpr (sizeof(T) == 2) {
    if (nt > 1) {
      const bn_u32x4 r = {v.raw.x, v.raw.y, v.raw.z, v.raw.w};
      __builtin_nontemporal_store(r, reinterpret_cast<bn_u32x4*>(p));
      return;
    }
  }
  v.store(p);
}

__device__ __forceinline__ void load8f(const float* __restrict__ p, float* o) {
  const float4 a = *reinterpret_cast<const float4*>(p);
  const float4 b = *reinterpret_cast<const float4*>(p + 4);
  o[0] = a.x; o[1] = a.y; o[2] = a.z; o[3] = a.w; o[4] = b.x; o[5] = b.y; o[6] = b.z; o[7] = b.w;
}


template <typename T, bool ADD, bool RELU, bool MASK>
__global__ void __launch_bounds__(kBnThreads) bn_apply_kernel(
    const T* __restrict__ x, const T* __restrict__ addend, const float* __restrict__ scale,
    const float* __restrict__ shift, T* __restrict__ y, uint8_t* __restrict__ mask, int64_t nvec, int C, int nt) {
  const int64_t stride = static_cast<int64_t>(gridDim.x) * blockDim.x;
  int64_t v = static_cast<int64_t>(blockIdx.x) * blockDim.x + threadIdx.x;
  int c = static_cast<int>((v * 8) % C);
  const int cstep = static_cast<int>((stride * 8) % C);
  float sc[8], sh[8];
  auto compute = [&](const Vec8<T>& vx, const Vec8<T>& va, int64_t vv) {
    Vec8<T> out;
    uint32_t bits = 0;
#pragma unroll
    for (int i = 0; i < 8; ++i) {
      float r = vx.get(i) * sc[i] + sh[i];
      if (ADD) r += va.get(i);
      if (MASK) bits |= (r > 0.f ? 1u : 0u) << i;
      if (RELU) r = r > 0.f ? r : 0.f;
      out.set(i, r);
    }
    vstore(out, y + vv * 8, nt == 2 ? 2 : 0);
    if (MASK) mask[vv] = static_cast<uint8_t>(bits);
  };
  if (cstep == 0) {
    load8f(scale + c, sc);
    load8f(shift + c, sh);
    for (; v + stride < nvec; v += 2 * stride) {
      Vec8<T> vx0, vx1, va0, va1;
      vload(vx0, x + v * 8, nt);
      vload(vx1, x + (v + stride) * 8, nt);
      if (ADD) {
        vload(va0, addend + v * 8, nt);
        vload(va1, addend + (v + stride) * 8, nt);
      }
      compute(vx0, va0, v);
      compute(vx1, va1, v + stride);
    }
    if (v < nvec) {
      Vec8<T> vx, va;
      vload(vx, x + v * 8, nt);
      if (ADD) vload(va, addend + v * 8, nt);
      compute(vx, va, v);
    }
    return;
  }
  for (; v < nvec; v += stride, c = (c + cstep >= C) ? c + cstep - C : c + cstep) {
    Vec8<T> vx, va;
    vload(vx, x + v * 8, nt);
    if (ADD) vload(va, addend + v * 8, nt);
    load8f(scale + c, sc);
    load8f(shift + c, sh);
    compute(vx, va, v);
  }
}

template <typename T, int RELU, bool WRITE_DZ>
__global__ void __launch_bounds__(kBnThreads) bn_bwd_apply_kernel(
    const T* __restrict__ x, const T* __restrict__ dy, const T* __restrict__ y, const uint8_t* __restrict__ mask,
    const float* __restrict__ A, const float* __restrict__ B, const float* __restrict__ Cc,
    const float* __restrict__ fscale, const float* __restrict__ fshift,
    T* __restrict__ dx, T* __restrict__ dz_out, int64_t nvec, int C, int nt) {
  const int64_t stride = static_cast<int64_t>(gridDim.x) * blockDim.x;
  int64_t v = static_cast<int64_t>(blockIdx.x) * blockDim.x + threadIdx.x;
  int c = static_cast<int>((v * 8) % C);
  const int cstep = static_cast<int>((stride * 8) % C);
  float fs[8], fh[8], ka[8], kb[8], kc[8];
  auto coef = [&](int cc) {
    if (RELU == kReluFromX) {
      load8f(fscale + cc, fs);
      load8f(fshift + cc, fh);
    }
    load8f(A + cc, ka);
    load8f(B + cc, kb);
    load8f(Cc + cc, kc);
  };
  struct In {
    Vec8<T> x, dy, y;
    uint32_t mb;
  };
  auto load = [&](In& in, int64_t vv) {
    vload(in.x, x + vv * 8, nt);
    vload(in.dy, dy + vv * 8, nt);
    if (RELU == kReluFromY) vload(in.y, y + vv * 8, nt);
    in.mb = RELU == kReluFromMask ? mask[vv] : 0u;
  };
  auto compute = [&](const In& in, int64_t vv) {
    Vec8<T> out, dz;
#pragma unroll
    for (int i = 0; i < 8; ++i) {
      float d = in.dy.get(i);
      if (RELU == kReluFromY) d = in.y.get(i) > 0.f ? d : 0.f;
      if (RELU == kReluFromX) d = fmaf(in.x.get(i), fs[i], fh[i]) > 0.f ? d : 0.f;
      if (RELU == kReluFromMask) d = ((in.mb >> i) & 1u) ? d : 0.f;
      if (WRITE_DZ) dz.set(i, d);
      out.set(i, ka[i] * d + kb[i] * in.x.get(i) + kc[i]);
    }
    vstore(out, dx + vv * 8, nt == 2 ? 2 : 0);
    if (WRITE_DZ) vstore(dz, dz_out + vv * 8, nt >= 2 ? 2 : 0);
  };
  if (cstep == 0) {
    coef(c);
    for (; v + stride < nvec; v += 2 * stride) {
      In i0, i1;
      load(i0, v);
      load(i1, v + stride);
      compute(i0, v);
      compute(i1, v + stride);
    }
    if (v < nvec) {
      In i0;
      load(i0, v);
      compute(i0, v);
    }
    return;
  }
  for (; v < nvec; v += stride, c = (c + cstep >= C) ? c + cstep - C : c + cstep) {
    In i0;
    load(i0, v);
    coef(c);
    compute(i0, v);
  }
}

template <typename T>
__global__ void __launch_bounds__(kBnThreads) bn_tail_bwd_ds_kernel(
    const T* __restrict__ x, const T* __restrict__ dy, const uint8_t* __restrict__ mask,
    const float* __restrict__ A, const float* __restrict__ B, const float* __restrict__ Cc, T* __restrict__ dx,
    T* __restrict__ dz_out, const T* __restrict__ zds, const float* __restrict__ mean_ds, float* __restrict__ part1,
    float* __restrict__ part2, int64_t R, int C, int tpr, int rpi, int64_t rows_per_block, int nt) {
  const int tid = threadIdx.x;
  const int lane_c = tid % tpr;
  const int lane_r = tid / tpr;
  const int cbase = blockIdx.y * tpr * 8 + lane_c * 8;
  float s1[8], s2[8], ka[8], kb[8], kc[8], km[8];
#pragma unroll
  for (int i = 0; i < 8; ++i) {
    s1[i] = 0.f;
    s2[i] = 0.f;
    ka[i] = A[cbase + i];
    kb[i] = B[cbase + i];
    kc[i] = Cc[cbase + i];
    km[i] = mean_ds[cbase + i];
  }
  const int64_t r0 = static_cast<int64_t>(blockIdx.x) * rows_per_block;
  int64_t r1 = r0 + rows_per_block;
  if (r1 > R) r1 = R;
  const bool spare = lane_r >= rpi;
  if (spare) r1 = r0;
  constexpr int UNR = 2;
  auto body = [&](const Vec8<T>& vx, const Vec8<T>& vdy, const Vec8<T>& vz, uint32_t mb, int64_t off) {
    Vec8<T> out, dz;
#pragma unroll
    for (int i = 0; i < 8; ++i) {
      const float d = ((mb >> i) & 1u) ? vdy.get(i) : 0.f;
      dz.set(i, d);
      out.set(i, ka[i] * d + kb[i] * vx.get(i) + kc[i]);
      s1[i] += d;
      s2[i] += d * (vz.get(i) - km[i]);
    }
    out.store(dx + off);
    if (dz_out != nullptr) vstore(dz, dz_out + off, nt >= 2 ? 2 : 0);
  };
  int64_t r = r0 + lane_r;
  for (; r + (UNR - 1) * rpi < r1; r += UNR * rpi) {
    Vec8<T> vx[UNR], vdy[UNR], vz[UNR];
    uint32_t vm[UNR];
#pragma unroll
    for (int u = 0; u < UNR; ++u) {
      const int64_t off = (r + u * rpi) * C + cbase;
      vload(vx[u], x + off, nt);
      vload(vdy[u], dy + off, nt);
      vload(vz[u], zds + off, nt);
      vm[u] = mask[off >> 3];
    }
#pragma unroll
    for (int u = 0; u < UNR; ++u) body(vx[u], vdy[u], vz[u], vm[u], (r + u * rpi) * C + cbase);
  }
  for (; r < r1; r += rpi) {
    const int64_t off = r * C + cbase;
    Vec8<T> vx, vdy, vz;
    vload(vx, x + off, nt);
    vload(vdy, dy + off, nt);
    vload(vz, zds + off, nt);
    body(vx, vdy, vz, mask[off >> 3], off);
  }
  __shared__ float sh1[kBnThreads * 8];
  __shared__ float sh2[kBnThreads * 8];
  const int cb = tpr * 8;
  if (!spare) {
#pragma unroll
    for (int i = 0; i < 8; ++i) {
      sh1[lane_r * cb + lane_c * 8 + i] = s1[i];
      sh2[lane_r * cb + lane_c * 8 + i] = s2[i];
    }
  }
  __syncthreads();
  for (int c = tid; c < cb; c += kBnThreads) {
    float a = 0.f, b = 0.f;
    for (int rr = 0; rr < rpi; ++rr) {
      a += sh1[rr * cb + c];
      b += sh2[rr * cb + c];
    }
    const int64_t o = static_cast<int64_t>(blockIdx.y * cb + c) * gridDim.x + blockIdx.x;
    part1[o] = a;
    part2[o] = b;
  }
}


static int bn_nt() { return 1; }

static int bn_total_blocks() { return 512; }

static inline int64_t bn_rows_per_block(int64_t R, int C, const BnGeom& g, int* nblk,
                                        int total_blocks = bn_total_blocks(), int min_rows = 0) {
  const int cblocks = C / g.cb;
  int64_t target = total_blocks / cblocks;
  if (target < 8) target = 8;
  int64_t rpb = (R + target - 1) / target;
  rpb = (rpb + g.rpi - 1) / g.rpi * g.rpi;
  if (rpb < g.rpi * 4) rpb = g.rpi * 4;
  if (rpb < min_rows) rpb = (min_rows + g.rpi - 1) / g.rpi * g.rpi;
  *nblk = static_cast<int>((R + rpb - 1) / rpb);
  return rpb;
}

static int bn_tail_blocks() { return 1024; }

int bn_tail_ds_rows(int64_t R, int C) {
  BnGeom g = bn_geom(C);
  int nblk;
  bn_rows_per_block(R, C, g, &nblk, bn_tail_blocks(), 64);
  return nblk;
}

int bn_partials_rows(int64_t R, int C) {
  BnGeom g = bn_geom(C);
  int nblk;
  bn_rows_per_block(R, C, g, &nblk);
  return nblk;
}

template <typename T>
static void bn_forward_impl(const void* x, const void* addend, void* y, uint8_t* mask, const float* gamma,
                            const float* beta, const float* center, float* part, float* mean, float* invstd,
                            float* var, float* scale, float* shift, int64_t R, int C, float eps, int training,
                            int relu, int fix_gamma, float momentum, float* mm_upd, float* mv_upd, int ext_nblk,
                            hipStream_t s) {
  MXAMD_HOST_CHECK(C % 8 == 0, "bn_nhwc: channels must be a multiple of 8");
  BnGeom g = bn_geom(C);
  MXAMD_HOST_CHECK(C % g.cb == 0, "bn_nhwc: unsupported channel count");
  if (training) {
    int nblk;
    float* p1 = part;
    if (ext_nblk > 0) {
      nblk = ext_nblk;
    } else {
      int64_t rpb = bn_rows_per_block(R, C, g, &nblk);
      dim3 grid(nblk, C / g.cb);
      float* p2r = part + static_cast<int64_t>(nblk) * C;
      hipLaunchKernelGGL((bn_reduce_kernel<T, 0, kReluNone>), grid, dim3(kBnThreads), 0, s,
                         static_cast<const T*>(x), nullptr, nullptr, nullptr, center, nullptr, nullptr, p1, p2r, R, C,
                         g.tpr, g.rpi, rpb);
    }
    float* p2 = part + static_cast<int64_t>(nblk) * C;
    hipLaunchKernelGGL((bn_finalize_kernel<0>), dim3((C + kFinPerBlock - 1) / kFinPerBlock), dim3(kFinThreads), 0, s, p1, p2, nblk, C, R, center, gamma,
                       beta, nullptr, eps, mean, invstd, var, scale, shift, nullptr, fix_gamma, 1, momentum, mm_upd,
                       mv_upd, 0);
  }
  if (y == nullptr) return;
  const int64_t nvec = R * C / 8;
  int blocks = static_cast<int>((nvec + kBnThreads - 1) / kBnThreads);
  if (blocks > 256 * 16) blocks = 256 * 16;
  const T* xa = static_cast<const T*>(x);
  const T* aa = static_cast<const T*>(addend);
  T* ya = static_cast<T*>(y);
#define APPLY(ADD, RELU, MASK)                                                                              \
  hipLaunchKernelGGL((bn_apply_kernel<T, ADD, RELU, MASK>), dim3(blocks), dim3(kBnThreads), 0, s, xa, aa, scale, \
                     shift, ya, mask, nvec, C, bn_nt())
  MXAMD_HOST_CHECK(mask == nullptr || (addend && relu), "bn_nhwc_forward: mask output only for add+relu");
  if (addend) {
    if (relu) {
      if (mask) APPLY(true, true, true); else APPLY(true, true, false);
    } else {
      APPLY(true, false, false);
    }
  } else {
    if (relu) APPLY(false, true, false); else APPLY(false, false, false);
  }
#undef APPLY
}

template <typename T>
static void bn_backward_impl(const void* x, const void* dy, const void* y, const uint8_t* mask, void* dx, void* dz,
                             const float* gamma, const float* mean, const float* invstd, const float* fscale,
                             const float* fshift, float* part, float* dgamma, float* dbeta, float* coef, int64_t R,
                             int C, int relu_mode, int fix_gamma, int training, int accum, hipStream_t s,
                             int ext_nblk, const void* ds_z, const float* ds_mean, float* ds_part) {
  BnGeom g = bn_geom(C);
  int nblk;
  int64_t rpb = bn_rows_per_block(R, C, g, &nblk);
  if (ext_nblk > 0) nblk = ext_nblk;
  dim3 grid(nblk, C / g.cb);
  float* p1 = part;
  float* p2 = part + static_cast<int64_t>(nblk) * C;
  const T* xa = static_cast<const T*>(x);
  const T* dya = static_cast<const T*>(dy);
  const T* ya = static_cast<const T*>(y);
  MXAMD_HOST_CHECK(relu_mode != kReluFromY || y != nullptr, "bn_nhwc_backward: relu mask from y needs y");
  MXAMD_HOST_CHECK(relu_mode != kReluFromX || (fscale && fshift), "bn_nhwc_backward: relu-from-x needs scale/shift");
  MXAMD_HOST_CHECK(relu_mode != kReluFromMask || mask != nullptr, "bn_nhwc_backward: relu-from-mask needs the mask");
#define RED(RL)                                                                                                \
  hipLaunchKernelGGL((bn_reduce_kernel<T, 1, RL>), grid, dim3(kBnThreads), 0, s, xa, dya, ya, mask, mean, fscale, \
                     fshift,                                                                                         \
                     p1, p2, R, C, g.tpr, g.rpi, rpb)
  if (ext_nblk > 0) {
  } else if (relu_mode == kReluFromY) RED(kReluFromY);
  else if (relu_mode == kReluFromX) RED(kReluFromX);
  else if (relu_mode == kReluFromMask) RED(kReluFromMask);
  else RED(kReluNone);
#undef RED
  float* A = coef;
  float* B = coef + C;
  float* Cc = coef + 2 * C;
  hipLaunchKernelGGL((bn_finalize_kernel<1>), dim3((C + kFinPerBlock - 1) / kFinPerBlock), dim3(kFinThreads), 0, s, p1, p2, nblk, C, R, mean, gamma, nullptr,
                     invstd, 0.f, dgamma, dbeta, A, B, Cc, nullptr, fix_gamma, training, 0.f, nullptr,
                     nullptr, accum);
  const int64_t nvec = R * C / 8;
  int blocks = static_cast<int>((nvec + kBnThreads - 1) / kBnThreads);
  if (blocks > 256 * 16) blocks = 256 * 16;
  T* dxa = static_cast<T*>(dx);
  T* dza = static_cast<T*>(dz);
  if (ds_z) {
    MXAMD_HOST_CHECK(relu_mode == kReluFromMask && ds_mean && ds_part,
                     "bn_nhwc_backward: shortcut statistics need the tail's mask mode and the BN's mean");
    int dnblk;
    const int64_t drpb = bn_rows_per_block(R, C, g, &dnblk, bn_tail_blocks(), 64);
    hipLaunchKernelGGL((bn_tail_bwd_ds_kernel<T>), dim3(dnblk, C / g.cb), dim3(kBnThreads), 0, s, xa, dya, mask, A, B,
                       Cc, dxa, dza, static_cast<const T*>(ds_z), ds_mean, ds_part,
                       ds_part + static_cast<int64_t>(dnblk) * C, R, C, g.tpr, g.rpi, drpb, bn_nt());
    return;
  }
#define BWD(RL, WD)                                                                                      \
  hipLaunchKernelGGL((bn_bwd_apply_kernel<T, RL, WD>), dim3(blocks), dim3(kBnThreads), 0, s, xa, dya, ya, mask, A, B, \
                     Cc, fscale, fshift, dxa, dza, nvec, C, bn_nt())
  if (relu_mode == kReluFromY) {
    if (dz) BWD(kReluFromY, true); else BWD(kReluFromY, false);
  } else if (relu_mode == kReluFromX) {
    if (dz) BWD(kReluFromX, true); else BWD(kReluFromX, false);
  } else if (relu_mode == kReluFromMask) {
    if (dz) BWD(kReluFromMask, true); else BWD(kReluFromMask, false);
  } else {
    if (dz) BWD(kReluNone, true); else BWD(kReluNone, false);
  }
#undef BWD
}

int bn_nhwc_stats(int dtype, const void* x, const float* center, float* part, int64_t R, int C, hipStream_t s,
                  int total_blocks) {
  MXAMD_HOST_CHECK(C % 8 == 0, "bn_nhwc: channels must be a multiple of 8");
  BnGeom g = bn_geom(C);
  MXAMD_HOST_CHECK(C % g.cb == 0, "bn_nhwc: unsupported channel count");
  int nblk;
  int64_t rpb = bn_rows_per_block(R, C, g, &nblk, total_blocks);
  dim3 grid(nblk, C / g.cb);
  float* p2 = part + static_cast<int64_t>(nblk) * C;
#define STATS(T)                                                                                              \
  hipLaunchKernelGGL((bn_reduce_kernel<T, 0, kReluNone>), grid, dim3(kBnThreads), 0, s, static_cast<const T*>(x), \
                     nullptr, nullptr, nullptr, center, nullptr, nullptr, part, p2, R, C, g.tpr, g.rpi, rpb)
  if (dtype == kF16) STATS(__half); else if (dtype == kBF16) STATS(__hip_bfloat16); else STATS(float);
#undef STATS
  return nblk;
}

namespace {
constexpr int kColsumTargetBlocks = 768;

inline void colsum_geom(int64_t R, int C, int* nchunk, int* rows_per) {
  const int strips = (C + 63) / 64;
  int64_t n = (kColsumTargetBlocks + strips - 1) / strips;
  n = std::max<int64_t>(1, std::min<int64_t>(n, (R + 31) / 32));
  int64_t rp = (R + n - 1) / n;
  rp = (rp + 31) / 32 * 32;
  *rows_per = static_cast<int>(rp);
  *nchunk = static_cast<int>((R + rp - 1) / rp);
}

template <typename T>
__global__ void __launch_bounds__(256) colsum_part_kernel(const T* __restrict__ x, int64_t R, int C, int rows_per,
                                                          float* __restrict__ part) {
  __shared__ float red[32][64 + 1];
  const int cv = threadIdx.x & 7, ty = threadIdx.x >> 3;
  const int c0 = (blockIdx.x * 8 + cv) * 8;
  const int64_t r0 = static_cast<int64_t>(blockIdx.y) * rows_per;
  const int64_t r1 = r0 + rows_per < R ? r0 + rows_per : R;
  float a[8] = {0.f, 0.f, 0.f, 0.f, 0.f, 0.f, 0.f, 0.f};
  if (c0 < C) {
    for (int64_t r = r0 + ty; r < r1; r += 32) {
      Vec8<T> v;
      v.load(x + r * C + c0);
#pragma unroll
      for (int i = 0; i < 8; ++i) a[i] += v.get(i);
    }
  }
#pragma unroll
  for (int i = 0; i < 8; ++i) red[ty][cv * 8 + i] = a[i];
  __syncthreads();
  if (threadIdx.x < 64) {
    const int col = threadIdx.x;
    float t = 0.f;
#pragma unroll 8
    for (int j = 0; j < 32; ++j) t += red[j][col];
    const int c = blockIdx.x * 64 + col;
    if (c < C) part[static_cast<int64_t>(blockIdx.y) * C + c] = t;
  }
}

template <typename TO>
__global__ void __launch_bounds__(256) colsum_fin_kernel(const float* __restrict__ part, int nchunk, int C,
                                                         TO* __restrict__ out, int accum) {
  __shared__ float red[16][17];
  const int col = threadIdx.x & 15, l16 = threadIdx.x >> 4;
  const int c = blockIdx.x * 16 + col;
  float t0 = 0.f, t1 = 0.f, t2 = 0.f, t3 = 0.f;
  if (c < C) {
    int i = l16;
    for (; i + 48 < nchunk; i += 64) {
      t0 += part[static_cast<int64_t>(i) * C + c];
      t1 += part[static_cast<int64_t>(i + 16) * C + c];
      t2 += part[static_cast<int64_t>(i + 32) * C + c];
      t3 += part[static_cast<int64_t>(i + 48) * C + c];
    }
    for (; i < nchunk; i += 16) t0 += part[static_cast<int64_t>(i) * C + c];
  }
  red[l16][col] = (t0 + t1) + (t2 + t3);
  __syncthreads();
  if (l16 == 0 && c < C) {
    float t = 0.f;
#pragma unroll
    for (int j = 0; j < 16; ++j) t += red[j][col];
    if (accum) t += static_cast<float>(out[c]);
    out[c] = static_cast<TO>(t);
  }
}
}

int64_t colsum_partials(int64_t R, int C) {
  int nchunk, rows_per;
  colsum_geom(R, C, &nchunk, &rows_per);
  return static_cast<int64_t>(nchunk) * C;
}

void colsum_rows(int dtype, const void* x, const float* zeros, float* part, int64_t R, int C, int out_dtype,
                 void* out, int accum, hipStream_t s) {
  (void)zeros;
  MXAMD_HOST_CHECK(C % 8 == 0, "colsum_rows: columns must be a multiple of 8");
  int nchunk, rows_per;
  colsum_geom(R, C, &nchunk, &rows_per);
  const dim3 grid((C + 63) / 64, nchunk);
  if (dtype == kF16)
    hipLaunchKernelGGL(colsum_part_kernel<__half>, grid, dim3(256), 0, s, static_cast<const __half*>(x), R, C,
                       rows_per, part);
  else if (dtype == kBF16)
    hipLaunchKernelGGL(colsum_part_kernel<__hip_bfloat16>, grid, dim3(256), 0, s,
                       static_cast<const __hip_bfloat16*>(x), R, C, rows_per, part);
  else
    hipLaunchKernelGGL(colsum_part_kernel<float>, grid, dim3(256), 0, s, static_cast<const float*>(x), R, C,
                       rows_per, part);
  const dim3 g2((C + 15) / 16);
  if (out_dtype == kF16)
    hipLaunchKernelGGL(colsum_fin_kernel<__half>, g2, dim3(256), 0, s, part, nchunk, C, static_cast<__half*>(out),
                       accum);
  else if (out_dtype == kBF16)
    hipLaunchKernelGGL(colsum_fin_kernel<__hip_bfloat16>, g2, dim3(256), 0, s, part, nchunk, C,
                       static_cast<__hip_bfloat16*>(out), accum);
  else
    hipLaunchKernelGGL(colsum_fin_kernel<float>, g2, dim3(256), 0, s, part, nchunk, C, static_cast<float*>(out),
                       accum);
}

void bn_nhwc_forward(int dtype, const void* x, const void* addend, void* y, uint8_t* mask, const float* gamma,
                     const float* beta,
                     const float* center, float* part, float* mean, float* invstd, float* var, float* scale,
                     float* shift, int64_t R, int C, float eps, int training, int relu, int fix_gamma,
                     float momentum, float* mm_upd, float* mv_upd, int ext_nblk, hipStream_t s) {
  switch (dtype) {
    case kF16:
      bn_forward_impl<__half>(x, addend, y, mask, gamma, beta, center, part, mean, invstd, var, scale, shift, R, C, eps,
                              training, relu, fix_gamma, momentum, mm_upd, mv_upd, ext_nblk, s);
      break;
    case kBF16:
      bn_forward_impl<__hip_bfloat16>(x, addend, y, mask, gamma, beta, center, part, mean, invstd, var, scale, shift, R,
                                      C, eps, training, relu, fix_gamma, momentum, mm_upd, mv_upd, ext_nblk, s);
      break;
    default:
      bn_forward_impl<float>(x, addend, y, mask, gamma, beta, center, part, mean, invstd, var, scale, shift, R, C, eps,
                             training, relu, fix_gamma, momentum, mm_upd, mv_upd, ext_nblk, s);
  }
}

void bn_finalize_backward(const float* part, int nblk, int C, int64_t R, const float* mean, const float* gamma,
                          const float* invstd, float* dgamma, float* dbeta, float* coef, int fix_gamma, int training,
                          int accum, hipStream_t s) {
  hipLaunchKernelGGL((bn_finalize_kernel<1>), dim3((C + kFinPerBlock - 1) / kFinPerBlock), dim3(kFinThreads), 0, s, part,
                     part + static_cast<int64_t>(nblk) * C, nblk, C, R, mean, gamma, nullptr, invstd, 0.f, dgamma,
                     dbeta, coef, coef + C, coef + 2 * C, nullptr, fix_gamma, training, 0.f, nullptr, nullptr, accum);
}

void bn_nhwc_backward(int dtype, const void* x, const void* dy, const void* y, const uint8_t* mask, void* dx,
                      void* dz,
                      const float* gamma, const float* mean, const float* invstd, const float* fscale,
                      const float* fshift, float* part, float* dgamma, float* dbeta, float* coef, int64_t R, int C,
                      int relu_mode, int fix_gamma, int training, int accum, hipStream_t s, int ext_nblk,
                      const void* ds_z, const float* ds_mean, float* ds_part) {
  switch (dtype) {
    case kF16:
      bn_backward_impl<__half>(x, dy, y, mask, dx, dz, gamma, mean, invstd, fscale, fshift, part, dgamma, dbeta, coef, R,
                               C, relu_mode, fix_gamma, training, accum, s, ext_nblk, ds_z, ds_mean, ds_part);
      break;
    case kBF16:
      bn_backward_impl<__hip_bfloat16>(x, dy, y, mask, dx, dz, gamma, mean, invstd, fscale, fshift, part, dgamma, dbeta,
                                       coef, R, C, relu_mode, fix_gamma, training, accum, s, ext_nblk, ds_z, ds_mean,
                                       ds_part);
      break;
    default:
      bn_backward_impl<float>(x, dy, y, mask, dx, dz, gamma, mean, invstd, fscale, fshift, part, dgamma, dbeta, coef, R,
                              C, relu_mode, fix_gamma, training, accum, s, ext_nblk, ds_z, ds_mean, ds_part);
  }
}

}
```

### src/kernels/conv_wgrad.hip

```cpp
#include <algorithm>
#include <stdexcept>

#include "common.h"
#include "mfma.h"

namespace mxamd {

namespace {

typedef short v4s __attribute__((ext_vector_type(4)));
typedef short v8s __attribute__((ext_vector_type(8)));
typedef _Float16 half8_t __attribute__((ext_vector_type(8)));
typedef __bf16 bf16x8_t __attribute__((ext_vector_type(8)));
typedef float f4_t __attribute__((ext_vector_type(4)));
typedef uint32_t u32x4 __attribute__((ext_vector_type(4)));
typedef __attribute__((address_space(3))) v4s lds_v4s;

struct FastDiv {
  uint32_t d, m, s;
};

inline FastDiv make_fastdiv(uint32_t d) {
  FastDiv f;
  f.d = d;
// ... 373 lines not shown
#pragma unroll
  for (int i = 0; i < IPW; ++i) {
    const int ins = wid + i * NW;
    d_on[i] = ins < NINS;
    lpt += d_on[i] ? 1 : 0;
    const int sub = d_on[i] ? ins >> 3 : 0;
    const int row = (ins & 7) * 8 + t;
    const int gch = (lane & 7) ^ swz(row);
    d_row[i] = row;
    d_lds[i] = sub * SUB * (int)sizeof(T) + (ins & 7) * 1024;
    d_isx[i] = sub < XSUB;
    if (d_isx[i]) {
      const int n = m0 + sub * 64;
      const int rs = n / g.C;
      d_col[i] = n - rs * g.C + gch * 8;
      d_r[i] = (rs / g.S) * g.dh;
      d_s[i] = (rs - (rs / g.S) * g.S) * g.dw;
    } else {
      d_col[i] = n0 + (sub - XSUB) * 64 + gch * 8;
      d_r[i] = d_s[i] = 0;
    }
  }
  const T* zsrc = zero + ((lane & 7) << 3);

  int i_kt = 0, i_stage = 0;
  auto issue = [&]() {
    char* sbase = wsm + i_stage * STAGE_B;
#pragma unroll
    for (int i = 0; i < IPW; ++i) {
      if (!d_on[i]) continue;
      const int p = pbeg + i_kt * 64 + d_row[i];
      bool ok = p < pend;
      const T* src;
      if (!d_isx[i]) {
        src = dy + (int64_t)p * g.K + d_col[i];
      } else if (IDENT) {
        src = x + (int64_t)p * g.C + d_col[i];
      } else {
        const int nimg = (int)fdiv((uint32_t)p, g.fHoWo);
        const int rem = p - nimg * (g.Ho * g.Wo);
        const int ho = (int)fdiv((uint32_t)rem, g.fWo);
        const int wo = rem - ho * g.Wo;
        const int hi = ho * g.sh - g.ph + d_r[i];
        const int wi = wo * g.sw - g.pw + d_s[i];
        ok = ok && (unsigned)hi < (unsigned)g.H && (unsigned)wi < (unsigned)g.W;
        src = x + ((int64_t)(nimg * g.H + hi) * g.W + wi) * g.C + d_col[i];
      }
      __builtin_amdgcn_global_load_lds((gbl_void_t*)(ok ? src : zsrc), (lds_void_t*)(sbase + d_lds[i]), 16, 0,
                                       0);
    }
    ++i_kt;
    i_stage = (i_stage + 1 == NST) ? 0 : i_stage + 1;
  };

  const int fg = lane >> 4, fq = (lane >> 2) & 3, fp = lane & 3;
  const int frow = 8 * fg + fq;
  int foff[4];
#pragma unroll
  for (int f = 0; f < 4; ++f) foff[f] = frow * 128 + ((((2 * f) + (fp >> 1)) ^ swz(frow)) << 4) + ((fp & 1) << 3);

  f4_t acc[FM][4];
#pragma unroll
  for (int i = 0; i < FM; ++i)
#pragma unroll
    for (int j = 0; j < 4; ++j) acc[i][j] = f4_t{0.f, 0.f, 0.f, 0.f};

  const int npro = KT < D ? KT : D;
  for (int p = 0; p < npro; ++p) issue();
  int c_stage = 0;
  for (int kt = 0; kt < KT; ++kt) {
    const int ahead = (KT - 1 - kt) < (D - 1) ? (KT - 1 - kt) : (D - 1);
    wg_vm_wait_le(ahead * lpt);
    asm volatile("s_waitcnt lgkmcnt(0)\n\ts_barrier" ::: "memory");
    if (kt + D < KT) issue();
    const T* sx = reinterpret_cast<const T*>(wsm + c_stage * STAGE_B) + wm * MS * SUB;
    const T* sd = reinterpret_cast<const T*>(wsm + c_stage * STAGE_B) + (XSUB + wn) * SUB;
#pragma unroll
    for (int kk = 0; kk < 64; kk += 32) {
      v8s a[FM], b[4];
#pragma unroll
      for (int f = 0; f < 4; ++f) b[f] = tr_frag(sd, kk * 128 + foff[f]);
#pragma unroll
      for (int f = 0; f < FM; ++f) a[f] = tr_frag(sx + (f >> 2) * SUB, kk * 128 + foff[f & 3]);
#pragma unroll
      for (int i = 0; i < FM; ++i)
#pragma unroll
        for (int j = 0; j < 4; ++j) acc[i][j] = Mfma16<T>::run(a[i], b[j], acc[i][j]);
    }
    c_stage = (c_stage + 1 == NST) ? 0 : c_stage + 1;
  }

  float* out = slab + (size_t)split * g.K * g.RSC;
  const int rsc_l = (lane >> 4) * 4;
  const int k_l = lane & 15;
#pragma unroll
  for (int i = 0; i < FM; ++i) {
    const int rsc = m0 + wm * MS * 64 + i * 16 + rsc_l;
#pragma unroll
    for (int j = 0; j < 4; ++j) {
      const int k = n0 + wn * 64 + j * 16 + k_l;
      *reinterpret_cast<f4_t*>(out + (size_t)k * g.RSC + rsc) = acc[i][j];
    }
  }
}

template <typename OutT>
__device__ __forceinline__ void store4(OutT* p, f4_t v);
template <>
__device__ __forceinline__ void store4<float>(float* p, f4_t v) {
  *reinterpret_cast<f4_t*>(p) = v;
}
template <>
__device__ __forceinline__ void store4<__half>(__half* p, f4_t v) {
  __half2 a = __floats2half2_rn(v[0], v[1]), b = __floats2half2_rn(v[2], v[3]);
  uint2 r;
  r.x = *reinterpret_cast<uint32_t*>(&a);
  r.y = *reinterpret_cast<uint32_t*>(&b);
  *reinterpret_cast<uint2*>(p) = r;
}
template <>
__device__ __forceinline__ void store4<__hip_bfloat16>(__hip_bfloat16* p, f4_t v) {
  uint32_t u[4];
#pragma unroll
  for (int i = 0; i < 4; ++i) {
    uint32_t b = __float_as_uint(v[i]);
    u[i] = (b + 0x7fffu + ((b >> 16) & 1u)) >> 16;
  }
  uint2 r;
  r.x = u[0] | (u[1] << 16);
  r.y = u[2] | (u[3] << 16);
  *reinterpret_cast<uint2*>(p) = r;
}

template <typename OutT>
__device__ __forceinline__ f4_t load4(const OutT* p);
template <>
__device__ __forceinline__ f4_t load4<float>(const float* p) {
  return *reinterpret_cast<const f4_t*>(p);
}
template <>
__device__ __forceinline__ f4_t load4<__half>(const __half* p) {
  uint2 r = *reinterpret_cast<const uint2*>(p);
  __half2 a = *reinterpret_cast<__half2*>(&r.x), b = *reinterpret_cast<__half2*>(&r.y);
  float2 fa = __half22float2(a), fb = __half22float2(b);
  return f4_t{fa.x, fa.y, fb.x, fb.y};
}
template <>
__device__ __forceinline__ f4_t load4<__hip_bfloat16>(const __hip_bfloat16* p) {
  uint2 r = *reinterpret_cast<const uint2*>(p);
  return f4_t{__uint_as_float(r.x << 16), __uint_as_float(r.x & 0xffff0000u), __uint_as_float(r.y << 16),
              __uint_as_float(r.y & 0xffff0000u)};
}

template <typename OutT, bool FINAL>
__global__ void __launch_bounds__(256) wgrad_reduce_kernel(float* __restrict__ slab, int nrows, int64_t row_stride,
                                                           int rows_per_group, int64_t n, OutT* __restrict__ out,
                                                           int accum) {
  const int64_t i4 = ((int64_t)blockIdx.x * 256 + threadIdx.x) * 4;
  if (i4 >= n) return;
  const int r0 = blockIdx.y * rows_per_group;
  const int r1 = min(nrows, r0 + rows_per_group);
  float* base = slab + i4;
  f4_t s0 = f4_t{0.f, 0.f, 0.f, 0.f}, s1 = s0, s2 = s0, s3 = s0;
  int r = r0;
  for (; r + 3 < r1; r += 4) {
    s0 += *reinterpret_cast<const f4_t*>(base + (int64_t)r * row_stride);
    s1 += *reinterpret_cast<const f4_t*>(base + (int64_t)(r + 1) * row_stride);
    s2 += *reinterpret_cast<const f4_t*>(base + (int64_t)(r + 2) * row_stride);
    s3 += *reinterpret_cast<const f4_t*>(base + (int64_t)(r + 3) * row_stride);
  }
  for (; r < r1; ++r) s0 += *reinterpret_cast<const f4_t*>(base + (int64_t)r * row_stride);
  s0 += s1 + s2 + s3;
  if (FINAL) {
    if (accum) s0 += load4<OutT>(out + i4);
    store4<OutT>(out + i4, s0);
  } else {
    *reinterpret_cast<f4_t*>(base + (int64_t)r0 * row_stride) = s0;
  }
}

template <typename OutT>
void launch_reduce(float* slab, int splits, int64_t n, OutT* out, int accum, hipStream_t s) {
  const int64_t cols4 = n / 4;
  const unsigned gx = (unsigned)((cols4 + 255) / 256);
  int groups = (int)std::min<int64_t>(splits, std::max<int64_t>(1, (256 * 256 * 2) / std::max<int64_t>(cols4, 1)));
  const int rpg = (splits + groups - 1) / groups;
  groups = (splits + rpg - 1) / rpg;
  if (groups > 1) {
    hipLaunchKernelGGL((wgrad_reduce_kernel<OutT, false>), dim3(gx, groups), dim3(256), 0, s, slab, splits, n, rpg, n,
                       out, accum);
    hipLaunchKernelGGL((wgrad_reduce_kernel<OutT, true>), dim3(gx, 1), dim3(256), 0, s, slab, groups,
                       (int64_t)rpg * n, groups, n, out, accum);
  } else {
    hipLaunchKernelGGL((wgrad_reduce_kernel<OutT, true>), dim3(gx, 1), dim3(256), 0, s, slab, splits, n, splits, n,
                       out, accum);
  }
}

struct WgradPlan {
  int wm, wn, fm, splits, plen;
};

WgradPlan plan_wgrad(int N, int H, int W, int C, int K, int R, int S, int sh, int sw, int ph, int pw, int dh = 1,
                     int dw = 1) {
  WgradPlan pl;
  const int Ho = (H + 2 * ph - dh * (R - 1) - 1) / sh + 1, Wo = (W + 2 * pw - dw * (S - 1) - 1) / sw + 1;
  const int RSC = R * S * C;
  const int64_t P = (int64_t)N * Ho * Wo;
  pl.fm = 4;
  if (RSC % 128 == 0 && K % 128 == 0) { pl.wm = 2; pl.wn = 2; }
  else if (RSC % 192 == 0) { pl.wm = 3; pl.wn = 1; }
  else if (RSC % 128 == 0) { pl.wm = 2; pl.wn = 1; }
  else if (K % 128 == 0) { pl.wm = 1; pl.wn = 2; }
  else { pl.wm = 1; pl.wn = 1; }
  const int64_t tiles = (int64_t)(RSC / (16 * pl.fm * pl.wm)) * (K / (64 * pl.wn));
  const int waves = pl.wm * pl.wn;
  int64_t splits = 4096 / (tiles * waves);
  const int64_t max_by_len = P / 512;
  const int64_t max_by_mem = (int64_t)(24 << 20) / ((int64_t)K * RSC);
  splits = std::min(splits, std::min(max_by_len, max_by_mem));
  if (splits < 1) splits = 1;
  int64_t plen = (P + splits - 1) / splits;
  plen = (plen + 63) / 64 * 64;
  pl.plen = (int)plen;
  pl.splits = (int)((P + plen - 1) / plen);
  return pl;
}

template <typename T, int WM, int WN, int FM>
void launch_wgrad(const void* x, const void* dy, float* slab, const WgradGeom& g, int splits, bool ident,
                  const void* zero, hipStream_t s) {
  dim3 grid(g.tiles * splits);
  if (zero && FM == 4) {
    if (ident)
      hipLaunchKernelGGL((conv_wgrad_glds_kernel<T, WM, WN, true>), grid, dim3(64 * WM * WN), 0, s,
                         static_cast<const T*>(x), static_cast<const T*>(dy), slab, static_cast<const T*>(zero), g);
    else
      hipLaunchKernelGGL((conv_wgrad_glds_kernel<T, WM, WN, false>), grid, dim3(64 * WM * WN), 0, s,
                         static_cast<const T*>(x), static_cast<const T*>(dy), slab, static_cast<const T*>(zero), g);
    return;
  }
  if (ident)
    hipLaunchKernelGGL((conv_wgrad_kernel<T, WM, WN, FM, true>), grid, dim3(64 * WM * WN), 0, s,
                       static_cast<const T*>(x), static_cast<const T*>(dy), slab, g);
  else
    hipLaunchKernelGGL((conv_wgrad_kernel<T, WM, WN, FM, false>), grid, dim3(64 * WM * WN), 0, s,
                       static_cast<const T*>(x), static_cast<const T*>(dy), slab, g);
}

template <typename T>
void dispatch_wgrad(const void* x, const void* dy, float* slab, const WgradGeom& g, const WgradPlan& pl, bool ident,
                    const void* zero, hipStream_t s) {
  if (pl.wm == 2 && pl.wn == 2 && pl.fm == 8) launch_wgrad<T, 2, 2, 8>(x, dy, slab, g, pl.splits, ident, zero, s);
  else if (pl.wm == 2 && pl.wn == 2) launch_wgrad<T, 2, 2, 4>(x, dy, slab, g, pl.splits, ident, zero, s);
  else if (pl.wm == 3) launch_wgrad<T, 3, 1, 4>(x, dy, slab, g, pl.splits, ident, zero, s);
  else if (pl.wm == 2) launch_wgrad<T, 2, 1, 4>(x, dy, slab, g, pl.splits, ident, zero, s);
  else if (pl.wn == 2) launch_wgrad<T, 1, 2, 4>(x, dy, slab, g, pl.splits, ident, zero, s);
  else launch_wgrad<T, 1, 1, 4>(x, dy, slab, g, pl.splits, ident, zero, s);
}

struct RingW {
  int wm, wn, nst, fm;
};
static bool ring_wgrad_cfg(int variant, RingW* c) {
  switch (variant) {
    case 1: *c = {4, 2, 3, 4}; return true;
    case 2: *c = {2, 4, 3, 4}; return true;
    case 3: *c = {3, 1, 4, 4}; return true;
    case 4: *c = {4, 1, 4, 4}; return true;
    case 5: *c = {2, 2, 4, 4}; return true;
    case 6: *c = {2, 4, 2, 8}; return true;
    case 7: *c = {4, 2, 2, 8}; return true;
    case 8: *c = {9, 1, 2, 4}; return true;
    case 9: *c = {1, 4, 4, 4}; return true;
    default: return false;
  }
}

static WgradPlan plan_wgrad_ring(const RingW& c, int N, int H, int W, int C, int K, int R, int S, int sh, int sw,
                                 int ph, int pw, int dh = 1, int dw = 1) {
  WgradPlan pl;
  const int Ho = (H + 2 * ph - dh * (R - 1) - 1) / sh + 1, Wo = (W + 2 * pw - dw * (S - 1) - 1) / sw + 1;
  const int RSC = R * S * C;
  const int64_t P = (int64_t)N * Ho * Wo;
  pl.fm = 4;
  pl.wm = c.wm;
  pl.wn = c.wn;
  const int64_t tiles = (int64_t)(RSC / (16 * c.fm * c.wm)) * (K / (64 * c.wn));
  int64_t splits = std::max<int64_t>(1, 256 / tiles);
  splits = std::min<int64_t>(splits, std::max<int64_t>(1, P / 256));
  int64_t plen = (P + splits - 1) / splits;
  plen = (plen + 63) / 64 * 64;
  pl.plen = (int)plen;
  pl.splits = (int)((P + plen - 1) / plen);
  return pl;
}

template <typename T, int WM, int WN, int NST, int FM = 4>
static void launch_wgrad_ring(const void* x, const void* dy, float* slab, const WgradGeom& g, int splits, bool ident,
                              const void* zero, hipStream_t s) {
  constexpr int SMEM = NST * (WM * FM / 4 + WN) * 64 * 64 * (int)sizeof(T);
  static_assert(SMEM <= 160 * 1024, "wgrad ring LDS budget");
  static bool attr[2] = {false, false};
  const void* fn = ident ? reinterpret_cast<const void*>(&conv_wgrad_ring_kernel<T, WM, WN, NST, FM, true>)
                         : reinterpret_cast<const void*>(&conv_wgrad_ring_kernel<T, WM, WN, NST, FM, false>);
  if (!attr[ident]) {
    hipFuncSetAttribute(fn, hipFuncAttributeMaxDynamicSharedMemorySize, SMEM);
    attr[ident] = true;
  }
  dim3 grid(g.tiles * splits);
  if (ident)
    hipLaunchKernelGGL((conv_wgrad_ring_kernel<T, WM, WN, NST, FM, true>), grid, dim3(64 * WM * WN), SMEM, s,
                       static_cast<const T*>(x), static_cast<const T*>(dy), slab, static_cast<const T*>(zero), g);
  else
    hipLaunchKernelGGL((conv_wgrad_ring_kernel<T, WM, WN, NST, FM, false>), grid, dim3(64 * WM * WN), SMEM, s,
                       static_cast<const T*>(x), static_cast<const T*>(dy), slab, static_cast<const T*>(zero), g);
}

template <typename T>
static void dispatch_wgrad_ring(int variant, const void* x, const void* dy, float* slab, const WgradGeom& g,
                                int splits, bool ident, const void* zero, hipStream_t s) {
  switch (variant) {
    case 1: launch_wgrad_ring<T, 4, 2, 3>(x, dy, slab, g, splits, ident, zero, s); break;
    case 2: launch_wgrad_ring<T, 2, 4, 3>(x, dy, slab, g, splits, ident, zero, s); break;
    case 3: launch_wgrad_ring<T, 3, 1, 4>(x, dy, slab, g, splits, ident, zero, s); break;
    case 4: launch_wgrad_ring<T, 4, 1, 4>(x, dy, slab, g, splits, ident, zero, s); break;
    case 5: launch_wgrad_ring<T, 2, 2, 4>(x, dy, slab, g, splits, ident, zero, s); break;
    case 6: launch_wgrad_ring<T, 2, 4, 2, 8>(x, dy, slab, g, splits, ident, zero, s); break;
    case 7: launch_wgrad_ring<T, 4, 2, 2, 8>(x, dy, slab, g, splits, ident, zero, s); break;
    case 8: launch_wgrad_ring<T, 9, 1, 2, 4>(x, dy, slab, g, splits, ident, zero, s); break;
    case 9: launch_wgrad_ring<T, 1, 4, 4, 4>(x, dy, slab, g, splits, ident, zero, s); break;
  }
}

}

int conv_nhwc_wgrad_ring_ok(int C, int K, int R, int S, int variant) {
  RingW c;
  if (!ring_wgrad_cfg(variant, &c)) return 0;
  return (C % 64 == 0 && K % (64 * c.wn) == 0 && (R * S * C) % (16 * c.fm * c.wm) == 0) ? 1 : 0;
}

int64_t conv_nhwc_wgrad_ring_workspace(int N, int H, int W, int C, int K, int R, int S, int sh, int sw, int ph, int pw,
                                       int variant, int dh, int dw) {
  RingW c;
  MXAMD_HOST_CHECK(ring_wgrad_cfg(variant, &c), "conv_nhwc_wgrad_ring: unknown variant");
  WgradPlan pl = plan_wgrad_ring(c, N, H, W, C, K, R, S, sh, sw, ph, pw, dh, dw);
  return (int64_t)pl.splits * K * R * S * C;
// ... 85 lines not shown
```

Measured before the change: 12360 images/sec.

## Fold projection-shortcut BN into dual BN-add-ReLU tail; single-pass LDS wgrad reduce

The projection shortcut's BatchNorm is folded into the residual tail. A new dual BN+add+ReLU op computes the shortcut BN statistics, then applies both affine transforms, the add and the ReLU in one apply kernel, so the shortcut BN output is never written and read back. Separately, the split-K wgrad reduction goes from two launches to one, with groups reduced through LDS inside a block. The cost is more complex autograd plumbing with two backward launches, plus different reduction ordering and occupancy behaviour.

```diff
diff --git a/mxnet_maintenance_amd/contrib/amp/lists.py b/mxnet_maintenance_amd/contrib/amp/lists.py
--- a/mxnet_maintenance_amd/contrib/amp/lists.py
+++ b/mxnet_maintenance_amd/contrib/amp/lists.py
@@ -22,7 +22,8 @@
           'broadcast_mod', 'broadcast_maximum', 'broadcast_minimum', 'broadcast_hypot', 'broadcast_equal',
           'broadcast_not_equal', 'broadcast_greater', 'broadcast_greater_equal', 'broadcast_lesser',
           'broadcast_lesser_equal', 'Concat', 'concat', 'stack', 'add_n', 'ElementWiseSum', 'where',
-          '_contrib_BatchNormAddReLU', 'BatchNormAddReLU']
+          '_contrib_BatchNormAddReLU', 'BatchNormAddReLU',
+          '_contrib_BatchNormBatchNormAddReLU', 'BatchNormBatchNormAddReLU']
 
 CONDITIONAL_FP32 = [('Activation', 'act_type', ['softrelu']), ('LeakyReLU', 'act_type', ['elu', 'selu'])]
 
diff --git a/mxnet_maintenance_amd/gluon/model_zoo/vision/resnet.py b/mxnet_maintenance_amd/gluon/model_zoo/vision/resnet.py
--- a/mxnet_maintenance_amd/gluon/model_zoo/vision/resnet.py
+++ b/mxnet_maintenance_amd/gluon/model_zoo/vision/resnet.py
@@ -1,6 +1,8 @@
 from ... import nn
 from ...block import HybridBlock
 from ...nn.basic_layers import _BatchNorm
+from ...parameter import DeferredInitializationError
+from .... import symbol as _symbol
 from ....context import cpu
 
 __all__ = ['ResNetV1', 'ResNetV2', 'BasicBlockV1', 'BasicBlockV2', 'BottleneckV1', 'BottleneckV2',
@@ -46,11 +48,32 @@
     def __init__(self, layout, fuse, **kwargs):
         super().__init__(axis=_bn_axis(layout), **kwargs)
         self._fuse_add = fuse
+        self._shortcut_bn_params = None
 
     def _alias(self):
         return 'batchnorm'
 
+    def fold_shortcut_bn(self, bn):
+        assert bn._kwargs == self._kwargs
+        self._shortcut_bn_params = [bn.gamma, bn.beta, bn.running_mean, bn.running_var]
+
+    def _shortcut_bn_values(self, F, shortcut):
+        if F is _symbol:
+            return [p.var() for p in self._shortcut_bn_params]
+        ctx = shortcut.context
+        try:
+            return [p.data(ctx) for p in self._shortcut_bn_params]
+        except DeferredInitializationError:
+            for p in self._shortcut_bn_params:
+                p.shape = (shortcut.shape[self._kwargs['axis']],)
+                p._finish_deferred_init()
+            return [p.data(ctx) for p in self._shortcut_bn_params]
+
     def hybrid_forward(self, F, x, shortcut, gamma, beta, running_mean, running_var):
+        if self._fuse_add and self._shortcut_bn_params is not None:
+            sg, sb, sm, sv = self._shortcut_bn_values(F, shortcut)
+            return F.contrib.BatchNormBatchNormAddReLU(x, shortcut, gamma, beta, sg, sb, running_mean, running_var,
+                                                       sm, sv, name='fwd', **self._kwargs)
         if self._fuse_add:
             return F.contrib.BatchNormAddReLU(x, shortcut, gamma, beta, running_mean, running_var, name='fwd',
                                               **self._kwargs)
@@ -60,6 +83,18 @@
 def _finish(F, tail, out, shortcut):
     y = tail(out, shortcut)
     return y if tail._fuse_add else F.Activation(y + shortcut, act_type='relu')
+
+
+def _fold_projection_bn(block, layout, fuse):
+    block._fold_ds = block.downsample is not None and fuse and layout == 'NHWC'
+    if block._fold_ds:
+        block.tail.fold_shortcut_bn(block.downsample[1])
+
+
+def _shortcut(block, x):
+    if block.downsample is None:
+        return x
+    return block.downsample[0](x) if block._fold_ds else block.downsample(x)
 
 
 class BasicBlockV1(HybridBlock):
@@ -77,9 +112,10 @@
         if downsample:
             self.downsample = nn.HybridSequential(prefix='')
             self.downsample.add(_conv(channels, 1, stride, 0, in_channels, layout), _bn(layout))
-
-    def hybrid_forward(self, F, x):
-        shortcut = self.downsample(x) if self.downsample is not None else x
+        _fold_projection_bn(self, layout, fuse)
+
+    def hybrid_forward(self, F, x):
+        shortcut = _shortcut(self, x)
         return _finish(F, self.tail, self.body(x), shortcut)
 
 
@@ -103,6 +139,7 @@
         if downsample:
             self.downsample = nn.HybridSequential(prefix='')
             self.downsample.add(_conv(channels, 1, stride, 0, in_channels, layout), _bn(layout))
+        _fold_projection_bn(self, layout, fuse)
         self._tee = fuse and s1 == 1 and layout == 'NHWC'
         if self._tee:
             self.body[0]._tee = True
@@ -113,9 +150,8 @@
             out, passthrough = blocks[0](x)
             for b in blocks[1:]:
                 out = b(out)
-            shortcut = self.downsample(passthrough) if self.downsample is not None else passthrough
-            return _finish(F, self.tail, out, shortcut)
-        shortcut = self.downsample(x) if self.downsample is not None else x
+            return _finish(F, self.tail, out, _shortcut(self, passthrough))
+        shortcut = _shortcut(self, x)
         return _finish(F, self.tail, self.body(x), shortcut)
 
 
diff --git a/mxnet_maintenance_amd/ops/hip_ops.py b/mxnet_maintenance_amd/ops/hip_ops.py
--- a/mxnet_maintenance_amd/ops/hip_ops.py
+++ b/mxnet_maintenance_amd/ops/hip_ops.py
@@ -176,6 +176,24 @@
     if act_type == 'relu':
         out = torch.relu(out)
     return out, mean_out, var_out
+
+
+def batch_norm_dual_add_relu(data, shortcut_data, gamma, beta, shortcut_gamma, shortcut_beta, moving_mean,
+                             moving_var, shortcut_moving_mean, shortcut_moving_var, eps, momentum, fix_gamma,
+                             training, axis):
+    nd = data.dim()
+    if (axis % nd == nd - 1 and nd > 2 and _use_hip(data) and _K.bn_ok(data) and _K.bn_ok(shortcut_data)
+            and shortcut_data.shape == data.shape and shortcut_data.dtype == data.dtype
+            and shortcut_data.device == data.device):
+        g = torch.ones_like(gamma) if fix_gamma else gamma
+        sg = torch.ones_like(shortcut_gamma) if fix_gamma else shortcut_gamma
+        return _K.BatchNormDualTailNHWC.apply(data, shortcut_data, g, beta, sg, shortcut_beta, eps, training,
+                                              moving_mean, moving_var, shortcut_moving_mean, shortcut_moving_var,
+                                              momentum)
+    sc = batch_norm(shortcut_data, shortcut_gamma, shortcut_beta, shortcut_moving_mean, shortcut_moving_var, eps,
+                    momentum, fix_gamma, training, axis, None)[0]
+    return batch_norm(data, gamma, beta, moving_mean, moving_var, eps, momentum, fix_gamma, training, axis, 'relu',
+                      addend=sc)
 
 
 
diff --git a/mxnet_maintenance_amd/ops/kernel_fns.py b/mxnet_maintenance_amd/ops/kernel_fns.py
--- a/mxnet_maintenance_amd/ops/kernel_fns.py
+++ b/mxnet_maintenance_amd/ops/kernel_fns.py
@@ -6,7 +6,7 @@
 from .. import _state
 from ..utils import env as _env
 
-__all__ = ['BatchNormNHWC', 'SoftmaxCE', 'GlobalAvgPoolNHWC', 'flat_sgd']
+__all__ = ['BatchNormNHWC', 'BatchNormDualTailNHWC', 'SoftmaxCE', 'GlobalAvgPoolNHWC', 'flat_sgd']
 
 _DT = {torch.float32: 0, torch.float16: 1, torch.bfloat16: 2}
 
@@ -73,6 +73,43 @@
         self.lazy = None
 
 
+def _bn_fwd_stats(lib, x, gamma, beta, moving_mean, moving_var, eps, training, momentum):
+    C = x.shape[-1]
+    R = x.numel() // C
+    dev = x.device
+    g, b, mm = _f32(gamma), _f32(beta), _f32(moving_mean)
+    ext_nblk, center, part = 0, mm, None
+    if training:
+        ext = getattr(x, '_mxamd_bn_part', None)
+        if ext is not None and ext[0].numel() == 2 * C * ext[1] and ext[0].device == dev:
+            part, ext_nblk = ext
+            center = _zeros_f32(C, dev)
+        else:
+            part = torch.empty(2 * lib.bn_partials_rows(R, C) * C, dtype=torch.float32, device=dev)
+        mean, invstd, var, scale, shift = torch.empty(5, C, dtype=torch.float32, device=dev).unbind(0)
+    else:
+        mean, var = mm, _f32(moving_var)
+        invstd = torch.rsqrt(var + eps)
+        scale = g * invstd
+        shift = b - mean * scale
+    upd = (training and momentum is not None and mm is moving_mean and moving_var.dtype == torch.float32
+           and moving_var.is_contiguous())
+
+    def args(relu):
+        return (g.data_ptr(), b.data_ptr(), center.data_ptr(), _p(part), mean.data_ptr(), invstd.data_ptr(),
+                var.data_ptr(), scale.data_ptr(), shift.data_ptr(), R, C, float(eps), int(bool(training)), int(bool(relu)),
+                0, float(momentum or 0.0), moving_mean.data_ptr() if upd else 0, moving_var.data_ptr() if upd else 0,
+                int(ext_nblk), _stream())
+    if training and momentum is not None and not upd:
+        def host_update():
+            with torch.no_grad():
+                moving_mean.mul_(momentum).add_(mean.to(moving_mean.dtype), alpha=1 - momentum)
+                moving_var.mul_(momentum).add_(var.to(moving_var.dtype), alpha=1 - momentum)
+    else:
+        host_update = None
+    return g, mean, invstd, var, scale, shift, args, host_update
+
+
 class BatchNormNHWC(torch.autograd.Function):
 
     @staticmethod
@@ -82,47 +119,18 @@
         C = x.shape[-1]
         R = x.numel() // C
         dev = x.device
-        g = _f32(gamma)
-        b = _f32(beta)
-        mm = _f32(moving_mean)
         assert pool is None or (relu and addend is None)
         y = torch.empty_like(x) if pool is None else None
         if addend is not None:
             assert addend.shape == x.shape and addend.dtype == x.dtype
             addend = addend.contiguous()
-        ext_nblk = 0
-        center = mm
-        if training:
-            ext = getattr(x, '_mxamd_bn_part', None)
-            if ext is not None and ext[0].numel() == 2 * C * ext[1] and ext[0].device == dev:
-                part, ext_nblk = ext
-                center = _zeros_f32(C, dev)
-            else:
-                nblk = lib.bn_partials_rows(R, C)
-                part = torch.empty(2 * nblk * C, dtype=torch.float32, device=dev)
-            stats = torch.empty(5, C, dtype=torch.float32, device=dev)
-            mean, invstd, var, scale, shift = stats.unbind(0)
-        else:
-            part = None
-            mean = mm
-            invstd = torch.rsqrt(_f32(moving_var) + eps)
-            var = _f32(moving_var)
-            scale = g * invstd
-            shift = b - mean * scale
-        upd = (training and momentum is not None and mm is moving_mean and moving_var.dtype == torch.float32
-               and moving_var.is_contiguous())
+        g, mean, invstd, var, scale, shift, args, host_update = _bn_fwd_stats(
+            lib, x, gamma, beta, moving_mean, moving_var, eps, training, momentum)
         mask = (torch.empty(x.numel() // 8, dtype=torch.uint8, device=dev)
                 if (addend is not None and relu and _RELU_FROM_X[0]) else None)
-        lib.bn_nhwc_forward(_DT[x.dtype], x.data_ptr(), _p(addend), _p(y), _p(mask), g.data_ptr(),
-                            b.data_ptr(),
-                            center.data_ptr(), _p(part), mean.data_ptr(), invstd.data_ptr(), var.data_ptr(),
-                            scale.data_ptr(), shift.data_ptr(), R, C, float(eps), int(bool(training)),
-                            int(bool(relu)), 0, float(momentum or 0.0), moving_mean.data_ptr() if upd else 0,
-                            moving_var.data_ptr() if upd else 0, int(ext_nblk), _stream())
-        if training and momentum is not None and not upd:
-            with torch.no_grad():
-                moving_mean.mul_(momentum).add_(mean.to(moving_mean.dtype), alpha=1 - momentum)
-                moving_var.mul_(momentum).add_(var.to(moving_var.dtype), alpha=1 - momentum)
+        lib.bn_nhwc_forward(_DT[x.dtype], x.data_ptr(), _p(addend), _p(y), _p(mask), *args(relu))
+        if host_update is not None:
+            host_update()
         ctx.pool = None
         if pool is not None:
             (kh, kw), (sh, sw), (ph, pw) = pool
@@ -260,6 +268,100 @@
         return dx, dgamma, dbeta, dz, None, None, None, None, None, None, None, None
 
 
+_DUAL_TAIL_USED = [0]
+
+
+def _bn_param_grad_dst(gamma_ref, beta_ref, need_g, need_b, out, C, dev):
+    tg = _leaf_grad(gamma_ref, C) if need_g else None
+    tb = _leaf_grad(beta_ref, C) if need_b else None
+    if tb is not None and (tg is not None or not need_g):
+        dg_buf = tg if tg is not None else torch.zeros(C, dtype=torch.float32, device=dev)
+        return dg_buf.data_ptr(), tb.data_ptr(), 1, True, dg_buf
+    return out[0].data_ptr(), out[1].data_ptr(), 0, False, None
+
+
+class BatchNormDualTailNHWC(torch.autograd.Function):
+
+    @staticmethod
+    def forward(ctx, x, z, gamma, beta, zgamma, zbeta, eps, training, moving_mean, moving_var, zmoving_mean,
+                zmoving_var, momentum=None):
+        lib = _K.lib()
+        assert z.shape == x.shape and z.dtype == x.dtype and z.is_contiguous()
+        dev = x.device
+        dt = _DT[x.dtype]
+        zg, zmean, zinvstd, _zvar, zscale, zshift, zargs, zhost = _bn_fwd_stats(
+            lib, z, zgamma, zbeta, zmoving_mean, zmoving_var, eps, training, momentum)
+        if training:
+            lib.bn_nhwc_forward(dt, z.data_ptr(), 0, 0, 0, *zargs(False))
+        g, mean, invstd, var, scale, shift, args, host = _bn_fwd_stats(
+            lib, x, gamma, beta, moving_mean, moving_var, eps, training, momentum)
+        y = torch.empty_like(x)
+        mask = torch.empty(x.numel() // 8, dtype=torch.uint8, device=dev)
+        lib.bn_nhwc_forward(dt, x.data_ptr(), z.data_ptr(), y.data_ptr(), mask.data_ptr(), *args(True),
+                            zscale.data_ptr(), zshift.data_ptr())
+        for h in (zhost, host):
+            if h is not None:
+                h()
+        _DUAL_TAIL_USED[0] += 1
+        ctx.save_for_backward(x, z, mask, g, mean, invstd, zg, zmean, zinvstd)
+        ctx.cfg = (bool(training), gamma.dtype, beta.dtype, zgamma.dtype, zbeta.dtype)
+        ctx.refs = (gamma, beta, zgamma, zbeta)
+        ctx.bn_token = None
+        if training and _BN_BWD_FUSE[0]:
+            ctx.bn_token = _BnToken()
+            y._mxamd_bn_src = (x, mean, None, None, mask, 3, ctx.bn_token)
+        ctx.mark_non_differentiable(mean, var)
+        ctx.set_materialize_grads(False)
+        return y, mean, var
+
+    @staticmethod
+    def backward(ctx, gy, _gm, _gv):
+        lib = _K.lib()
+        x, z, mask, g, mean, invstd, zg, zmean, zinvstd = ctx.saved_tensors
+        training, gdt, bdt, zgdt, zbdt = ctx.cfg
+        gamma_ref, beta_ref, zgamma_ref, zbeta_ref = ctx.refs
+        if gy is None:
+            return (None,) * 13
+        gy = gy.contiguous()
+        C = x.shape[-1]
+        R = x.numel() // C
+        dev = x.device
+        dt = _DT[x.dtype]
+        need = ctx.needs_input_grad
+        dx = torch.empty_like(x)
+        dzs = torch.empty_like(z)
+        ext = getattr(gy, '_mxamd_bn_bwd', None)
+        ext_nblk = 0
+        if ext is not None and ctx.bn_token is not None and ext[2] is ctx.bn_token and ext[3] == gy._version:
+            part, ext_nblk = ext[0], ext[1]
+        else:
+            part = torch.empty(2 * lib.bn_partials_rows(R, C) * C, dtype=torch.float32, device=dev)
+        out = torch.empty(5, C, dtype=torch.float32, device=dev)
+        zout = torch.empty(5, C, dtype=torch.float32, device=dev)
+        dg_ptr, db_ptr, accum, direct, _k1 = _bn_param_grad_dst(gamma_ref, beta_ref, need[2], need[3], out, C, dev)
+        zdg_ptr, zdb_ptr, zaccum, zdirect, _k2 = _bn_param_grad_dst(zgamma_ref, zbeta_ref, need[4], need[5], zout, C,
+                                                                    dev)
+        ride = training and _BN_TAIL_DS[0]
+        dkw, zpart, znblk = {}, None, 0
+        if ride:
+            znblk = lib.bn_tail_ds_rows(R, C)
+            zpart = torch.empty(2 * znblk * C, dtype=torch.float32, device=dev)
+            dkw = dict(ds_z=z.data_ptr(), ds_mean=zmean.data_ptr(), ds_part=zpart.data_ptr())
+        else:
+            zpart = torch.empty(2 * lib.bn_partials_rows(R, C) * C, dtype=torch.float32, device=dev)
+        lib.bn_nhwc_backward(dt, x.data_ptr(), gy.data_ptr(), 0, mask.data_ptr(), dx.data_ptr(), 0, g.data_ptr(),
+                             mean.data_ptr(), invstd.data_ptr(), 0, 0, part.data_ptr(), dg_ptr, db_ptr,
+                             out[2].data_ptr(), R, C, 3, 0, int(training), accum, _stream(), ext_nblk, **dkw)
+        lib.bn_nhwc_backward(dt, z.data_ptr(), gy.data_ptr(), 0, mask.data_ptr(), dzs.data_ptr(), 0, zg.data_ptr(),
+                             zmean.data_ptr(), zinvstd.data_ptr(), 0, 0, zpart.data_ptr(), zdg_ptr, zdb_ptr,
+                             zout[2].data_ptr(), R, C, 3, 0, int(training), zaccum, _stream(), znblk)
+        dgamma = None if direct or not need[2] else out[0].to(gdt)
+        dbeta = None if direct or not need[3] else out[1].to(bdt)
+        zdgamma = None if zdirect or not need[4] else zout[0].to(zgdt)
+        zdbeta = None if zdirect or not need[5] else zout[1].to(zbdt)
+        return dx, dzs, dgamma, dbeta, zdgamma, zdbeta, None, None, None, None, None, None, None
+
+
 def bnrelu_pool_ok(x, kernel, stride, pad):
     return (bn_ok(x) and tuple(kernel) == (3, 3) and pool_ok(x, kernel, stride, pad)
             and x.numel() + 256 * 32 * 256 * 8 < 2 ** 31 and hasattr(_K.lib(), 'pool_nhwc_forward_bnrelu'))
diff --git a/mxnet_maintenance_amd/ops/nn.py b/mxnet_maintenance_amd/ops/nn.py
--- a/mxnet_maintenance_amd/ops/nn.py
+++ b/mxnet_maintenance_amd/ops/nn.py
@@ -247,6 +247,28 @@
     training = _state.STATE.training and not use_global_stats
     return hip_ops.batch_norm(data, gamma, beta, moving_mean, moving_var, eps, momentum, fix_gamma,
                               training, axis, 'relu', addend=addend)
+
+
+def _bn_dual_infer(in_shapes, a):
+    d = in_shapes[0]
+    if d is None:
+        return {}
+    c = d[a.get('axis', 1) % len(d)]
+    return {i: (c,) for i in range(2, 10)}
+
+
+@register('_contrib_BatchNormBatchNormAddReLU', aliases=('BatchNormBatchNormAddReLU',),
+          arg_names=('data', 'shortcut_data', 'gamma', 'beta', 'shortcut_gamma', 'shortcut_beta'),
+          aux_names=('moving_mean', 'moving_var', 'shortcut_moving_mean', 'shortcut_moving_var'),
+          num_outputs=3, num_visible_outputs=_bn_nvis, infer_params=_bn_dual_infer, params=_BN_PARAMS)
+def batch_norm_batch_norm_add_relu(data, shortcut_data, gamma, beta, shortcut_gamma, shortcut_beta, moving_mean,
+                                   moving_var, shortcut_moving_mean, shortcut_moving_var, eps=1e-3, momentum=0.9,
+                                   fix_gamma=True, use_global_stats=False, output_mean_var=False, axis=1,
+                                   cudnn_off=False, act_type=None, min_calib_range=None, max_calib_range=None):
+    training = _state.STATE.training and not use_global_stats
+    return hip_ops.batch_norm_dual_add_relu(data, shortcut_data, gamma, beta, shortcut_gamma, shortcut_beta,
+                                            moving_mean, moving_var, shortcut_moving_mean, shortcut_moving_var,
+                                            eps, momentum, fix_gamma, training, axis)
 
 
 
diff --git a/src/kernels/bindings.cc b/src/kernels/bindings.cc
--- a/src/kernels/bindings.cc
+++ b/src/kernels/bindings.cc
@@ -13,7 +13,8 @@
                      const float* beta,
                      const float* center, float* part, float* mean, float* invstd, float* var, float* scale,
                      float* shift, int64_t R, int C, float eps, int training, int relu, int fix_gamma,
-                     float momentum, float* mm_upd, float* mv_upd, int ext_nblk, hipStream_t s);
+                     float momentum, float* mm_upd, float* mv_upd, int ext_nblk, hipStream_t s, const float* ascale,
+                     const float* ashift);
 void bn_nhwc_backward(int dtype, const void* x, const void* dy, const void* y, const uint8_t* mask, void* dx,
                       void* dz,
                       const float* gamma, const float* mean, const float* invstd, const float* fscale,
@@ -419,12 +420,17 @@
                               uintptr_t center, uintptr_t part, uintptr_t mean, uintptr_t inv, uintptr_t var,
                               uintptr_t scale, uintptr_t shift, int64_t R, int C, float eps, int training, int relu,
                               int fix_gamma, float momentum, uintptr_t mm_upd, uintptr_t mv_upd, int ext_nblk,
-                              uintptr_t s) {
+                              uintptr_t s, uintptr_t ascale, uintptr_t ashift) {
     bn_nhwc_forward(dt, P<void>(x), P<void>(add), P<void>(y), P<uint8_t>(mask), P<float>(g), P<float>(b), P<float>(center),
                     P<float>(part), P<float>(mean), P<float>(inv), P<float>(var), P<float>(scale), P<float>(shift), R,
-                    C, eps, training, relu, fix_gamma, momentum, P<float>(mm_upd), P<float>(mv_upd), ext_nblk, S(s));
+                    C, eps, training, relu, fix_gamma, momentum, P<float>(mm_upd), P<float>(mv_upd), ext_nblk, S(s),
+                    P<const float>(ascale), P<const float>(ashift));
     check_launch("bn_nhwc_forward");
-  });
+  }, py::arg("dt"), py::arg("x"), py::arg("add"), py::arg("y"), py::arg("mask"), py::arg("g"), py::arg("b"),
+     py::arg("center"), py::arg("part"), py::arg("mean"), py::arg("inv"), py::arg("var"), py::arg("scale"),
+     py::arg("shift"), py::arg("R"), py::arg("C"), py::arg("eps"), py::arg("training"), py::arg("relu"),
+     py::arg("fix_gamma"), py::arg("momentum"), py::arg("mm_upd"), py::arg("mv_upd"), py::arg("ext_nblk"),
+     py::arg("stream"), py::arg("ascale") = 0, py::arg("ashift") = 0);
   m.def("bn_nhwc_backward", [](int dt, uintptr_t x, uintptr_t dy, uintptr_t y, uintptr_t mask, uintptr_t dx,
                                uintptr_t dz,
                                uintptr_t g, uintptr_t mean, uintptr_t inv, uintptr_t fscale, uintptr_t fshift,
diff --git a/src/kernels/bn_nhwc.hip b/src/kernels/bn_nhwc.hip
--- a/src/kernels/bn_nhwc.hip
+++ b/src/kernels/bn_nhwc.hip
@@ -225,18 +225,32 @@
 }
 
 
-template <typename T, bool ADD, bool RELU, bool MASK>
+template <typename T, bool ADD, bool RELU, bool MASK, bool AFF = false>
 __global__ void __launch_bounds__(kBnThreads) bn_apply_kernel(
     const T* __restrict__ x, const T* __restrict__ addend, const float* __restrict__ scale,
-    const float* __restrict__ shift, T* __restrict__ y, uint8_t* __restrict__ mask, int64_t nvec, int C, int nt) {
+    const float* __restrict__ shift, T* __restrict__ y, uint8_t* __restrict__ mask, int64_t nvec, int C, int nt,
+    const float* __restrict__ ascale, const float* __restrict__ ashift) {
+  static_assert(ADD || !AFF, "an affine addend needs the add");
   const int64_t stride = static_cast<int64_t>(gridDim.x) * blockDim.x;
   int64_t v = static_cast<int64_t>(blockIdx.x) * blockDim.x + threadIdx.x;
   int c = static_cast<int>((v * 8) % C);
   const int cstep = static_cast<int>((stride * 8) % C);
-  float sc[8], sh[8];
-  auto compute = [&](const Vec8<T>& vx, const Vec8<T>& va, int64_t vv) {
+  float sc[8], sh[8], asc[8], ash[8];
+  auto coef = [&](int cc) {
+    load8f(scale + cc, sc);
+    load8f(shift + cc, sh);
+    if (AFF) {
+      load8f(ascale + cc, asc);
+      load8f(ashift + cc, ash);
+    }
+  };
+  auto compute = [&](const Vec8<T>& vx, Vec8<T> va, int64_t vv) {
     Vec8<T> out;
     uint32_t bits = 0;
+    if (AFF) {
+#pragma unroll
+      for (int i = 0; i < 8; ++i) va.set(i, va.get(i) * asc[i] + ash[i]);
+    }
 #pragma unroll
     for (int i = 0; i < 8; ++i) {
       float r = vx.get(i) * sc[i] + sh[i];
@@ -249,8 +263,7 @@
     if (MASK) mask[vv] = static_cast<uint8_t>(bits);
   };
   if (cstep == 0) {
-    load8f(scale + c, sc);
-    load8f(shift + c, sh);
+    coef(c);
     for (; v + stride < nvec; v += 2 * stride) {
       Vec8<T> vx0, vx1, va0, va1;
       vload(vx0, x + v * 8, nt);
@@ -274,8 +287,7 @@
     Vec8<T> vx, va;
     vload(vx, x + v * 8, nt);
     if (ADD) vload(va, addend + v * 8, nt);
-    load8f(scale + c, sc);
-    load8f(shift + c, sh);
+    coef(c);
     compute(vx, va, v);
   }
 }
@@ -472,7 +484,7 @@
                             const float* beta, const float* center, float* part, float* mean, float* invstd,
                             float* var, float* scale, float* shift, int64_t R, int C, float eps, int training,
                             int relu, int fix_gamma, float momentum, float* mm_upd, float* mv_upd, int ext_nblk,
-                            hipStream_t s) {
+                            hipStream_t s, const float* ascale, const float* ashift) {
   MXAMD_HOST_CHECK(C % 8 == 0, "bn_nhwc: channels must be a multiple of 8");
   BnGeom g = bn_geom(C);
   MXAMD_HOST_CHECK(C % g.cb == 0, "bn_nhwc: unsupported channel count");
@@ -501,11 +513,24 @@
   const T* xa = static_cast<const T*>(x);
   const T* aa = static_cast<const T*>(addend);
   T* ya = static_cast<T*>(y);
+  const float* no_coef = nullptr;
 #define APPLY(ADD, RELU, MASK)                                                                              \
   hipLaunchKernelGGL((bn_apply_kernel<T, ADD, RELU, MASK>), dim3(blocks), dim3(kBnThreads), 0, s, xa, aa, scale, \
-                     shift, ya, mask, nvec, C, bn_nt())
+                     shift, ya, mask, nvec, C, bn_nt(), no_coef, no_coef)
   MXAMD_HOST_CHECK(mask == nullptr || (addend && relu), "bn_nhwc_forward: mask output only for add+relu");
-  if (addend) {
+  MXAMD_HOST_CHECK((ascale == nullptr) == (ashift == nullptr) && (ascale == nullptr || addend),
+                   "bn_nhwc_forward: an affine addend needs the addend and both of its coefficient vectors");
+  if (ascale) {
+#define APPLY_AFF(RELU, MASK)                                                                                 \
+  hipLaunchKernelGGL((bn_apply_kernel<T, true, RELU, MASK, true>), dim3(blocks), dim3(kBnThreads), 0, s, xa, aa, \
+                     scale, shift, ya, mask, nvec, C, bn_nt(), ascale, ashift)
+    if (relu) {
+      if (mask) APPLY_AFF(true, true); else APPLY_AFF(true, false);
+    } else {
+      APPLY_AFF(false, false);
+    }
+#undef APPLY_AFF
+  } else if (addend) {
     if (relu) {
       if (mask) APPLY(true, true, true); else APPLY(true, true, false);
     } else {
@@ -709,19 +734,21 @@
                      const float* beta,
                      const float* center, float* part, float* mean, float* invstd, float* var, float* scale,
                      float* shift, int64_t R, int C, float eps, int training, int relu, int fix_gamma,
-                     float momentum, float* mm_upd, float* mv_upd, int ext_nblk, hipStream_t s) {
+                     float momentum, float* mm_upd, float* mv_upd, int ext_nblk, hipStream_t s, const float* ascale,
+                     const float* ashift) {
   switch (dtype) {
     case kF16:
       bn_forward_impl<__half>(x, addend, y, mask, gamma, beta, center, part, mean, invstd, var, scale, shift, R, C, eps,
-                              training, relu, fix_gamma, momentum, mm_upd, mv_upd, ext_nblk, s);
+                              training, relu, fix_gamma, momentum, mm_upd, mv_upd, ext_nblk, s, ascale, ashift);
       break;
     case kBF16:
       bn_forward_impl<__hip_bfloat16>(x, addend, y, mask, gamma, beta, center, part, mean, invstd, var, scale, shift, R,
-                                      C, eps, training, relu, fix_gamma, momentum, mm_upd, mv_upd, ext_nblk, s);
+                                      C, eps, training, relu, fix_gamma, momentum, mm_upd, mv_upd, ext_nblk, s, ascale,
+                                      ashift);
       break;
     default:
       bn_forward_impl<float>(x, addend, y, mask, gamma, beta, center, part, mean, invstd, var, scale, shift, R, C, eps,
-                             training, relu, fix_gamma, momentum, mm_upd, mv_upd, ext_nblk, s);
+                             training, relu, fix_gamma, momentum, mm_upd, mv_upd, ext_nblk, s, ascale, ashift);
   }
 }
 
diff --git a/src/kernels/conv_wgrad.hip b/src/kernels/conv_wgrad.hip
--- a/src/kernels/conv_wgrad.hip
+++ b/src/kernels/conv_wgrad.hip
@@ -549,48 +549,67 @@
               __uint_as_float(r.y & 0xffff0000u)};
 }
 
-template <typename OutT, bool FINAL>
-__global__ void __launch_bounds__(256) wgrad_reduce_kernel(float* __restrict__ slab, int nrows, int64_t row_stride,
-                                                           int rows_per_group, int64_t n, OutT* __restrict__ out,
-                                                           int accum) {
-  const int64_t i4 = ((int64_t)blockIdx.x * 256 + threadIdx.x) * 4;
-  if (i4 >= n) return;
-  const int r0 = blockIdx.y * rows_per_group;
-  const int r1 = min(nrows, r0 + rows_per_group);
-  float* base = slab + i4;
+__device__ __forceinline__ f4_t sum_rows4(const float* base, int64_t stride, int r0, int r1) {
   f4_t s0 = f4_t{0.f, 0.f, 0.f, 0.f}, s1 = s0, s2 = s0, s3 = s0;
   int r = r0;
   for (; r + 3 < r1; r += 4) {
-    s0 += *reinterpret_cast<const f4_t*>(base + (int64_t)r * row_stride);
-    s1 += *reinterpret_cast<const f4_t*>(base + (int64_t)(r + 1) * row_stride);
-    s2 += *reinterpret_cast<const f4_t*>(base + (int64_t)(r + 2) * row_stride);
-    s3 += *reinterpret_cast<const f4_t*>(base + (int64_t)(r + 3) * row_stride);
-  }
-  for (; r < r1; ++r) s0 += *reinterpret_cast<const f4_t*>(base + (int64_t)r * row_stride);
+    s0 += *reinterpret_cast<const f4_t*>(base + (int64_t)r * stride);
+    s1 += *reinterpret_cast<const f4_t*>(base + (int64_t)(r + 1) * stride);
+    s2 += *reinterpret_cast<const f4_t*>(base + (int64_t)(r + 2) * stride);
+    s3 += *reinterpret_cast<const f4_t*>(base + (int64_t)(r + 3) * stride);
+  }
+  for (; r < r1; ++r) s0 += *reinterpret_cast<const f4_t*>(base + (int64_t)r * stride);
   s0 += s1 + s2 + s3;
-  if (FINAL) {
-    if (accum) s0 += load4<OutT>(out + i4);
-    store4<OutT>(out + i4, s0);
-  } else {
-    *reinterpret_cast<f4_t*>(base + (int64_t)r0 * row_stride) = s0;
-  }
+  return s0;
+}
+
+template <typename OutT>
+__global__ void __launch_bounds__(256) wgrad_reduce_kernel(const float* __restrict__ slab, int nrows, int64_t n,
+                                                           OutT* __restrict__ out, int accum) {
+  const int64_t i4 = ((int64_t)blockIdx.x * 256 + threadIdx.x) * 4;
+  if (i4 >= n) return;
+  f4_t s0 = sum_rows4(slab + i4, n, 0, nrows);
+  if (accum) s0 += load4<OutT>(out + i4);
+  store4<OutT>(out + i4, s0);
+}
+
+constexpr int kReduceLdsQuads = 2048;
+
+template <typename OutT>
+__global__ void __launch_bounds__(256) wgrad_reduce_lanes_kernel(const float* __restrict__ slab, int nrows, int64_t n,
+                                                                 int groups, int rpg, int cq, OutT* __restrict__ out,
+                                                                 int accum) {
+  __shared__ f4_t red[kReduceLdsQuads];
+  const int lanes = 256 / cq;
+  const int q = threadIdx.x % cq, lane = threadIdx.x / cq;
+  const int64_t i4 = ((int64_t)blockIdx.x * cq + q) * 4;
+  const bool live = i4 < n;
+  if (live) {
+    for (int g = lane; g < groups; g += lanes)
+      red[g * cq + q] = sum_rows4(slab + i4, n, g * rpg, min(nrows, (g + 1) * rpg));
+  }
+  __syncthreads();
+  if (lane != 0 || !live) return;
+  f4_t s0 = sum_rows4(reinterpret_cast<const float*>(red + q), (int64_t)cq * 4, 0, groups);
+  if (accum) s0 += load4<OutT>(out + i4);
+  store4<OutT>(out + i4, s0);
 }
 
 template <typename OutT>
 void launch_reduce(float* slab, int splits, int64_t n, OutT* out, int accum, hipStream_t s) {
   const int64_t cols4 = n / 4;
-  const unsigned gx = (unsigned)((cols4 + 255) / 256);
   int groups = (int)std::min<int64_t>(splits, std::max<int64_t>(1, (256 * 256 * 2) / std::max<int64_t>(cols4, 1)));
   const int rpg = (splits + groups - 1) / groups;
   groups = (splits + rpg - 1) / rpg;
-  if (groups > 1) {
-    hipLaunchKernelGGL((wgrad_reduce_kernel<OutT, false>), dim3(gx, groups), dim3(256), 0, s, slab, splits, n, rpg, n,
-                       out, accum);
-    hipLaunchKernelGGL((wgrad_reduce_kernel<OutT, true>), dim3(gx, 1), dim3(256), 0, s, slab, groups,
-                       (int64_t)rpg * n, groups, n, out, accum);
+  if (groups > 1 && groups <= kReduceLdsQuads) {
+    int cq = cols4 / 64 >= 512 ? 64 : cols4 / 32 >= 512 ? 32 : cols4 / 16 >= 256 ? 16 : 8;
+    while (cq < 64 && 256 / cq >= 2 * groups) cq *= 2;
+    while (cq > 1 && groups * cq > kReduceLdsQuads) cq /= 2;
+    hipLaunchKernelGGL((wgrad_reduce_lanes_kernel<OutT>), dim3((unsigned)((cols4 + cq - 1) / cq)), dim3(256), 0, s,
+                       slab, splits, n, groups, rpg, cq, out, accum);
   } else {
-    hipLaunchKernelGGL((wgrad_reduce_kernel<OutT, true>), dim3(gx, 1), dim3(256), 0, s, slab, splits, n, splits, n,
-                       out, accum);
+    hipLaunchKernelGGL((wgrad_reduce_kernel<OutT>), dim3((unsigned)((cols4 + 255) / 256)), dim3(256), 0, s, slab,
+                       splits, n, out, accum);
   }
 }
 
```

New measurement: 12580 images/sec, median of 6. 1.02x the previous value.
